# fundwotsai2001/AP-adapter

Hardware: AMD Instinct MI355X
Metric: 10s-clips/sec @200 DDIM steps, AudioLDM2-large+AP (higher is better)
Workload: dtype bf16; 1 GPU; AudioLDM2-large geometry + 32 AP processors, style_transfer preset (ap_scale 0.55, La=32, CFG 9.5), batch 32/GPU, 10 s clips (latents 8x250x16), 200-step DDIM, hipGraph-captured step; one bench step = one DDIM step; global_batch=32, parallelism=dp1 (independent clips, no collective in the loop), weights=random-init N(0,0.02^2), real shapes (no checkpoint offline)

## Files before the change

ap-adapter_amd/_lib.py:

```python
import ctypes as C
import os
import subprocess
import threading

import torch

_HERE = os.path.dirname(os.path.abspath(__file__))
LIB_PATH = os.environ.get("APAD_LIB_PATH") or os.path.join(_HERE, "libapadapter_hip.so")
CSRC = os.path.join(_HERE, "csrc")

BF16, F16, F32, F32_BF16X3 = 0, 1, 2, 3
A_PLAIN, A_CONV3X3, A_PATCH16, A_CONV1D = 0, 1, 2, 4
EPI_NONE, EPI_SILU, EPI_GELU, EPI_GEGLU, EPI_TANH, EPI_RELU, EPI_GELU_TANH, EPI_GEGLU_TANH = 0, 1, 2, 3, 4, 5, 6, 7
OUT_ROWMAJOR, OUT_VT, OUT_QKV = 0, 1, 2

_vp, _i64, _i32, _f32 = C.c_void_p, C.c_int64, C.c_int32, C.c_float


class GemmDesc(C.Structure):
    _fields_ = [(n, _vp) for n in ("a", "w", "out", "bias", "residual", "rowgroup_bias", "step_ptr")] + \
               [(n, _i64) for n in ("M", "N", "K", "lda", "ldw", "ldo", "ldr", "ld_rg", "rows_per_group")] + \
               [(n, _i32) for n in ("a_mode", "epilogue", "out_mode", "dtype", "Hin", "Win", "Cin", "Hout", "Wout",
                                    "stride", "Hup", "Wup", "src_batch_mod", "residual_row_mod", "heads", "head_dim", "L", "Lpad")] + \
               [("out2", _vp), ("out3", _vp)] + \
               [(n, _i32) for n in ("taps", "dilation", "pad", "transposed", "a_pre_act")] + [("a_pre_slope", _f32)] + \
               [("conv_asym_pad", _i32), ("reserved_conv", _i32)] + \
               [(n, _vp) for n in ("rowstat_out", "rowstat_in", "ln_colsum", "ln_bias")] + [("rowstat_in_tiles", _i32), ("ln_eps", _f32)] + \
               [("a2", _vp), ("lda2", _i64), ("k_split", _i32), ("a_row_mod", _i32), ("a2_row_mod", _i32), ("reserved_a2", _i32), ("out4", _vp),
                ("w_halo", _vp), ("workspace", _vp), ("workspace_bytes", _i64)]


class AttnDesc(C.Structure):
    _fields_ = [(n, _vp) for n in ("q", "k", "vt", "k2", "vt2", "out", "key_bias", "lse")] + \
               [(n, _i64) for n in ("q_stride_b", "q_stride_n", "k_stride_b", "k_stride_l", "vt_stride_b",
                                    "k2_stride_b", "k2_stride_l", "vt2_stride_b", "o_stride_b", "o_stride_n")] + \
               [(n, _i32) for n in ("B", "N", "H", "D", "L", "Lpad", "L2", "Lpad2", "kv_batch_div", "kv2_batch_div",
                                    "dtype")] + \
               [("softmax_scale", _f32), ("scale2", _f32), ("q_prescaled", _i32)]


class RpSegment(C.Structure):
    _fields_ = [("out", _vp), ("bias", _vp), ("ldo", _i64), ("n_cols", _i32), ("mode", _i32)]


class RpDesc(C.Structure):
    _fields_ = [(n, _vp) for n in ("x", "w", "ln_gamma", "ln_beta", "residual")] + \
               [(n, _i64) for n in ("M", "lda", "ldw", "ldr")] + \
               [(n, _i32) for n in ("K", "epilogue", "dtype", "n_segments")] + [("ln_eps", _f32)] + \
               [(n, _i32) for n in ("heads", "head_dim", "L", "Lpad")] + [("seg", RpSegment * 3)]


class MlpDesc(C.Structure):
    _fields_ = [(n, _vp) for n in ("x", "ln_gamma", "ln_beta", "w1", "b1", "w2", "b2", "out")] + \
               [("M", _i64), ("C", _i32), ("dtype", _i32), ("ln_eps", _f32), ("reserved", _i32)]


class XattnDesc(C.Structure):
    _fields_ = [(n, _vp) for n in ("x", "ln_gamma", "ln_beta", "wq_packed", "wo_packed", "bo", "kv1_packed", "key_bias", "kv2_packed", "out", "q_fold")] + \
               [(n, _i32) for n in ("B", "N", "C", "heads", "L1", "L2", "dtype", "reserved")] + \
               [(n, _f32) for n in ("ln_eps", "softmax_scale", "scale2", "reserved_f")]


class XrowsDesc(C.Structure):
    _fields_ = [(n, _vp) for n in ("x", "ln_gamma", "ln_beta", "wq_packed", "wo_packed", "bo", "k1", "vt1", "key_bias", "k2", "vt2", "out")] + \
               [(n, _i32) for n in ("B", "N", "C", "heads", "L1", "Lpad1", "L2", "Lpad2", "dtype", "reserved")] + \
               [(n, _f32) for n in ("ln_eps", "softmax_scale", "scale2", "reserved_f")]


class HsAttnDesc(C.Structure):
    _fields_ = [(n, _vp) for n in ("x", "w_packed", "w_bias", "k1", "vt1", "key_bias", "k2", "vt2", "out")] + \
               [(n, _i32) for n in ("B", "N", "C", "heads", "L1", "Lpad1", "L2", "Lpad2", "self_attention", "q_prescaled", "dtype", "normalize")] + \
               [(n, _f32) for n in ("ln_eps", "softmax_scale", "scale2", "reserved_f")]


class HsOutDesc(C.Structure):
    _fields_ = [(n, _vp) for n in ("o", "w_packed", "bias", "residual", "out", "rowstat_out")] + [(n, _i32) for n in ("B", "N", "C", "dtype")]


class AttnBwdDesc(C.Structure):
    _fields_ = [(n, _vp) for n in ("q", "k", "v", "qt", "kt", "out", "dout", "doutt", "lse", "key_bias", "delta", "dq", "dk", "dv")] + \
               [(n, _i32) for n in ("B", "N", "H", "D", "L", "Npad", "Lpad", "dtype")] + \
               [("softmax_scale", _f32), ("dout_scale", _f32), ("accumulate_dq", _i32), ("ld_grad", _i32)]


SYMBOLS = {
    "apad_last_error": (C.c_char_p, []),
    "apad_abi_version": (C.c_int, []),
    "apad_set_gemm_ring": (C.c_int, [_i32]),
    "apad_sizeof_gemm_desc": (C.c_int, []),
    "apad_sizeof_attn_desc": (C.c_int, []),
    "apad_echo_gemm_desc": (C.c_int, [C.POINTER(GemmDesc), C.POINTER(C.c_double), C.c_int]),
    "apad_echo_attn_desc": (C.c_int, [C.POINTER(AttnDesc), C.POINTER(C.c_double), C.c_int]),
    "apad_sizeof_rp_desc": (C.c_int, []),
    "apad_echo_rp_desc": (C.c_int, [C.POINTER(RpDesc), C.POINTER(C.c_double), C.c_int]),
    "apad_rowpanel_gemm": (C.c_int, [C.POINTER(RpDesc), _vp]),
    "apad_sizeof_mlp_desc": (C.c_int, []),
    "apad_echo_mlp_desc": (C.c_int, [C.POINTER(MlpDesc), C.POINTER(C.c_double), C.c_int]),
    "apad_geglu_mlp": (C.c_int, [C.POINTER(MlpDesc), _vp]),
    "apad_mlp_packed_bytes": (_i64, [_i32]),
    "apad_mlp_packed_bias_floats": (_i64, [_i32]),
    "apad_mlp_pack": (C.c_int, [_vp, _vp, _vp, _vp, _vp, _i32, _i32, _vp]),
    "apad_geglu_mlp_packed": (C.c_int, [C.POINTER(MlpDesc), _vp, _vp, _vp]),
    "apad_geglu_packed_bytes": (_i64, [_i32]),
    "apad_geglu_packed_bias_floats": (_i64, [_i32]),
    "apad_geglu_pack": (C.c_int, [_vp, _vp, _vp, _vp, _i32, _i32, _vp]),
    "apad_layernorm_geglu_packed": (C.c_int, [_vp, _vp, _vp, _vp, _vp, _vp, _i64, _i32, _f32, _i32, _vp]),
    "apad_sizeof_xattn_desc": (C.c_int, []),
    "apad_echo_xattn_desc": (C.c_int, [C.POINTER(XattnDesc), C.POINTER(C.c_double), C.c_int]),
    "apad_fused_cross_attention": (C.c_int, [C.POINTER(XattnDesc), _vp]),
    "apad_sizeof_xrows_desc": (C.c_int, []),
    "apad_cross_attention_rows": (C.c_int, [C.POINTER(XrowsDesc), _vp]),
    "apad_sizeof_hs_attn_desc": (C.c_int, []),
    "apad_hs_attention": (C.c_int, [C.POINTER(HsAttnDesc), _vp]),
    "apad_self_attention_fused": (C.c_int, [_vp, _vp, _vp, _vp, _i32, _i32, _i32, _i32, _f32, _i32, _vp]),
    "apad_hs_geglu": (C.c_int, [_vp, _vp, _vp, _vp, _i32, _i32, _i32, _i32, _f32, _i32, _vp]),
    "apad_sizeof_hs_out_desc": (C.c_int, []),
    "apad_hs_out": (C.c_int, [C.POINTER(HsOutDesc), _vp]),
    "apad_hs_ff2": (C.c_int, [C.POINTER(HsOutDesc), _vp]),
    "apad_xattn_pack_weight": (C.c_int, [_vp, _vp, _i64, _i32, _vp]),
    "apad_xattn_packed_kv_bytes": (_i64, [_i32, _i32]),
    "apad_xattn_pack_kv": (C.c_int, [_vp, _vp, _vp, _i32, _i32, _i32, _i64, _i64, _i64, _i32, _vp]),
    "apad_rows_packed_kv_bytes": (_i64, [_i32, _i32, _i32, _i32]),
    "apad_rows_pack_kv": (C.c_int, [_vp, _vp, _vp, _i32, _i32, _i32, _i32, _i32, _i32, _vp]),
    "apad_gemm": (C.c_int, [C.POINTER(GemmDesc), _vp]),
    "apad_conv_halo_pack": (C.c_int, [_vp, _vp, _i64, _i64, _i32, _vp]),
    "apad_hconv_launch_count": (_i64, []),
    "apad_f32_split_weight": (C.c_int, [_vp, _vp, _i64, _i64, _i64, _vp]),
    "apad_f32x3_launch_count": (_i64, []),
    "apad_probe_mfma": (C.c_int, [_vp, _i32, _i32, C.POINTER(C.c_double), _vp]),
    "apad_conv_halo_packed_bytes": (_i64, [_i64, _i64]),
    "apad_conv_halo_workspace_bytes": (_i64, [_i64, _i64, _i64, _i32]),
    "apad_attention": (C.c_int, [C.POINTER(AttnDesc), _vp]),
    "apad_layernorm": (C.c_int, [_vp, _vp, _vp, _vp, _i64, _i32, _i64, _i64, _f32, _i32, _vp]),
    "apad_groupnorm_workspace_bytes": (_i64, [_i32, _i32, _i32]),
    "apad_groupnorm": (C.c_int, [_vp, _vp, _vp, _vp, _vp, _i32, _i32, _i32, _i32, _f32, _i32, _i32, _vp]),
    "apad_groupnorm2": (C.c_int, [_vp, _vp, _vp, _vp, _vp, _vp, _i32, _i32, _i32, _i32, _i32, _i32, _i32, _f32, _i32, _i32, _vp]),
    "apad_audiomae_pool": (C.c_int, [_vp, _vp, _i32, _i32, _i32, _i32, _i32, _vp]),
    "apad_timestep_embedding": (C.c_int, [_vp, _vp, _i32, _i32, _i32, _f32, _i32, _vp]),
    "apad_cfg_ddim_step": (C.c_int, [_vp, _vp, _vp, _vp, _vp, _vp, _f32, _i32, _i64, _i32, _vp]),
    "apad_step_advance": (C.c_int, [_vp, _vp]),
    "apad_cfg_sampler_step": (C.c_int, [_vp, _vp, _vp, _vp, _vp, _vp, _vp, _vp, _i32, _f32, _i32, _i64, _i32, _vp]),
    "apad_cfg_edit_step": (C.c_int, [_vp, _vp, _vp, _vp, _vp, _vp, _vp, _vp, _vp, _vp, _vp, _i32, _i32, _vp, _i32, _f32, _i32, _i64, _i32, _vp]),
    "apad_cfg_dual_step": (C.c_int, [_vp, _vp, _vp, _vp, _vp, _vp, _vp, _vp, _vp, _vp, _vp, _vp, _i32, _i32, _vp, _i32, _i32, _i64, _i32, _vp]),
    "apad_cfg_shaped_step": (C.c_int, [_vp] * 15 + [_i32, _i32, _vp, _i32, _f32, _i32, _i32, _i64, _i32, _vp]),
    "apad_cfg_invert_step": (C.c_int, [_vp, _vp, _vp, _vp, _vp, _vp, _vp, _vp, _vp, _vp, _i32, _f32, _i32, _i32, _i64, _i32, _vp]),
    "apad_edit_start": (C.c_int, [_vp, _vp, _vp, _vp, _vp, _vp, _f32, _f32, _f32, _i64, _i32, _i32, _vp]),
    "apad_mix3": (C.c_int, [_vp, _vp, _vp, _vp, _i64, _f32, _i32, _vp]),
    "apad_softmax_rows": (C.c_int, [_vp, _vp, _vp, _i64, _i32, _i64, _i64, _i64, _f32, _i32, _vp]),
    "apad_rmsnorm": (C.c_int, [_vp, _vp, _vp, _i64, _i32, _i64, _i64, _f32, _i32, _i32, _vp]),
    "apad_gather_rows": (C.c_int, [_vp, _vp, _vp, _i64, _i64, _i32, _i32, _vp]),
    "apad_gaussian_sample": (C.c_int, [_vp, _vp, _vp, _i64, _i32, _f32, _i32, _vp]),
    "apad_sizeof_attn_bwd_desc": (C.c_int, []),
    "apad_echo_attn_bwd_desc": (C.c_int, [C.POINTER(AttnBwdDesc), C.POINTER(C.c_double), C.c_int]),
    "apad_attention_bwd": (C.c_int, [C.POINTER(AttnBwdDesc), _vp]),
    "apad_head_transpose": (C.c_int, [_vp, _vp, _i32, _i32, _i32, _i32, _i32, _i32, _vp]),
    "apad_head_transpose3": (C.c_int, [_vp, _vp, _vp, _vp, _vp, _vp, _i32, _i32, _i32, _i32, _i32, _i32, _vp]),
    "apad_layernorm_bwd": (C.c_int, [_vp, _vp, _vp, _vp, _i64, _i32, _f32, _i32, _vp]),
    "apad_layernorm_bwd_add": (C.c_int, [_vp, _vp, _vp, _vp, _vp, _i64, _i32, _f32, _i32, _vp]),
    "apad_groupnorm_bwd": (C.c_int, [_vp, _vp, _vp, _vp, _vp, _i32, _i32, _i32, _i32, _f32, _i32, _i32, _vp]),
    "apad_geglu": (C.c_int, [_vp, _vp, _i64, _i32, _i32, _vp]),
    "apad_geglu_bwd": (C.c_int, [_vp, _vp, _vp, _i64, _i32, _i32, _vp]),
    "apad_upsample_nearest_bwd": (C.c_int, [_vp, _vp, _i32, _i32, _i32, _i32, _i32, _i32, _i32, _vp]),
    "apad_zero_stuff2": (C.c_int, [_vp, _vp, _i32, _i32, _i32, _i32, _i32, _i32, _i32, _vp]),
    "apad_transpose_pad": (C.c_int, [_vp, _vp, _i32, _i32, _i32, _i32, _vp]),
    "apad_transpose_pad2": (C.c_int, [_vp, _vp, _i32, _vp, _vp, _i32, _i32, _i32, _i32, _i32, _vp]),
    "apad_reduce_workspace_bytes": (_i64, []),
    "apad_mse_loss_grad": (C.c_int, [_vp, _vp, _vp, _vp, _vp, _i64, _f32, _i32, _vp]),
    "apad_step_advance_if_finite": (C.c_int, [_vp, _vp, _vp]),
    "apad_grad_norm": (C.c_int, [_vp, _vp, _vp, _i64, _vp]),
    "apad_resample_fir": (C.c_int, [_vp, _vp, _vp, _i64, _i64, _i32, _i32, _i32, _vp]),
    "apad_kaldi_fbank": (C.c_int, [_vp, _i64, _f32, _vp, _vp, _vp, _vp, _i32, _i32, _f32, _f32, _f32, _vp]),
    "apad_wav_stats": (C.c_int, [_vp, _vp, _vp, _vp, _i32, _vp]),
    "apad_stft_logmel": (C.c_int, [_vp, _vp, _vp, _vp, _vp, _vp, _vp, _vp, _vp, _i32, _i64, _i32, _vp]),
    "apad_adamw_step": (C.c_int, [_vp, _vp, _vp, _vp, _vp, _vp, _vp, _i64, _f32, _f32, _f32, _f32, _f32, _f32, _i32, _vp]),
    "apad_window_attention": (C.c_int, [_vp, _vp, _vp, _i32, _i32, _i32, _i32, _i32, _i32, _i32, _i32, _vp]),
    "apad_clap_mel2img": (C.c_int, [_vp, _vp, _vp, _vp, _vp, _f32, _vp, _i32, _i32, _i32, _i32, _vp]),
    "apad_clap_logmel": (C.c_int, [_vp, _vp, _vp, _vp, _vp, _vp, _i32, _i32, _i32, _vp, _vp, _vp, _vp, _vp, _i32, _i64, _i32, _i32, _i32, _vp]),
    "apad_chroma": (C.c_int, [_vp, _vp, _vp, _vp, _vp, _vp, _vp, _i32, _i32, _vp]),
    "apad_chroma_similarity": (C.c_int, [_vp, _vp, _vp, _vp, _vp, _vp, _vp, _vp, _i32, _i32, _i32, _vp]),
    "apad_loudness": (C.c_int, [_vp, _vp, _vp, _vp, _vp, _vp, _vp, _i32, _i32, _i32, _vp]),
    "apad_loudness_gain": (C.c_int, [_vp, _vp, _vp, _vp, _vp, _vp, _vp, _vp, _vp, _vp, _i32, _i32, _f32, _vp]),
}

_lock = threading.Lock()
_lib = None


def build(verbose=False):
    r = subprocess.run(["make", "-C", CSRC, "-j4"], capture_output=True, text=True)
    if verbose or r.returncode != 0:
        print(r.stdout[-4000:])
        print(r.stderr[-4000:])
    if r.returncode != 0:
        raise RuntimeError("building libapadapter_hip.so failed:\n" + r.stderr[-2000:])
    return LIB_PATH


def lib():
    global _lib
    if _lib is not None:
        return _lib
    with _lock:
        if _lib is None:
            if not os.path.exists(LIB_PATH):
                raise RuntimeError(
                    f"{LIB_PATH} is missing: the HIP extension is the product path and has no fallback; "
                    "run `python -c 'import __graft_entry__ as g; g.build()'` (or `make -C ap-adapter_amd/csrc`).")
            h = C.CDLL(LIB_PATH)
            for name, (res, args) in SYMBOLS.items():
                fn = getattr(h, name)
                fn.restype = res
                fn.argtypes = args
            if h.apad_abi_version() != 12:
                raise RuntimeError("libapadapter_hip.so ABI version mismatch")
            if h.apad_sizeof_gemm_desc() != C.sizeof(GemmDesc) or h.apad_sizeof_attn_desc() != C.sizeof(AttnDesc) \
                    or h.apad_sizeof_rp_desc() != C.sizeof(RpDesc) \
                    or h.apad_sizeof_mlp_desc() != C.sizeof(MlpDesc) \
                    or h.apad_sizeof_attn_bwd_desc() != C.sizeof(AttnBwdDesc) \
                    or h.apad_sizeof_xattn_desc() != C.sizeof(XattnDesc) or h.apad_sizeof_xrows_desc() != C.sizeof(XrowsDesc) \
                    or h.apad_sizeof_hs_attn_desc() != C.sizeof(HsAttnDesc) or h.apad_sizeof_hs_out_desc() != C.sizeof(HsOutDesc):
                raise RuntimeError("descriptor layout mismatch between include/apadapter_hip.h and _lib.py")
            _lib = h
    return _lib


def check(rc, what):
    if rc != 0:
        raise RuntimeError(f"{what} failed (rc={rc}): {lib().apad_last_error().decode()}")
```

ap-adapter_amd/autograd.py:

```python
import os as _os

import torch

from . import ops
from .derived import derived


def on(*tensors):
    return torch.is_grad_enabled() and any(t is not None and t.requires_grad for t in tensors)


def _derived(w, tag, make, deps=()):
    return make() if w.requires_grad else derived(w, tag, make, deps)


def _wt(w):
    return _derived(w, "T", lambda: w.detach().reshape(w.shape[0], -1).t().contiguous())


def _conv_dgrad_w(w):
    return _derived(w, "dgrad", lambda: w.detach().flip(2, 3).permute(1, 2, 3, 0).reshape(w.shape[1], -1).contiguous())


def _conv_fwd_w(w):
    return ops.conv3x3_pack(w) if w.requires_grad else ops.conv3x3_weight(w)


def _c(t):
    return t if t.is_contiguous() else t.contiguous()


def _exact(backward):
    def run(ctx, *grads):
        with ops.exact_f32():
            return backward(ctx, *grads)
    return run


class _Linear(torch.autograd.Function):

    @staticmethod
    def forward(ctx, x, w, b, residual):
        ctx.save_for_backward(x if w.requires_grad else None, w)
        ctx.has_res = residual is not None
        ctx.sink = getattr(w, "_apad_grad_sink", None)
        w2 = w.reshape(w.shape[0], -1)
        with ops.recorded_forward():
            return ops.linear(_c(x), w2, b, residual=None if residual is None else _c(residual))

    @staticmethod
    @_exact
    def backward(ctx, dy):
        x, w = ctx.saved_tensors
        dy = _c(dy)
        dx = dw = None
        if ctx.needs_input_grad[0]:
            dx = ops.linear(dy, _wt(w))
        if ctx.needs_input_grad[1]:
            if ctx.sink is not None:
                acc, inv_scale = ctx.sink
                if inv_scale == 1.0 and acc.is_contiguous() and acc.dim() == 2:
                    ops.weight_grad(dy.reshape(-1, dy.shape[-1]), x.reshape(-1, x.shape[-1]), fp32=True, acc=acc)
                else:
                    acc.add_(ops.weight_grad(dy.reshape(-1, dy.shape[-1]), x.reshape(-1, x.shape[-1]), fp32=True).reshape(acc.shape),
                             alpha=inv_scale)
            else:
                dw = ops.weight_grad(dy.reshape(-1, dy.shape[-1]), x.reshape(-1, x.shape[-1])).reshape(w.shape)
        return dx, dw, None, (dy if ctx.has_res and ctx.needs_input_grad[3] else None)


def linear(x, w, b=None, residual=None):
    return _Linear.apply(x, w, b, residual)


_BWD_PACKED = True


def _packed_grads(dq, dk, dv):
    base = dq._base
    C_ = dq.shape[-1]
    if (base is not None and dk._base is base and dv._base is base and base.is_contiguous() and base.shape[-1] == 3 * C_
            and base.shape[:-1] == dq.shape[:-1] and dq.stride() == dk.stride() == dv.stride() == base.stride()
            and dq.storage_offset() == base.storage_offset() and dk.storage_offset() == base.storage_offset() + C_
            and dv.storage_offset() == base.storage_offset() + 2 * C_):
        return base
    return torch.cat([_c(dq), _c(dk), _c(dv)], dim=-1)


class _QKV(torch.autograd.Function):

    @staticmethod
    def forward(ctx, x, wq, wk, wv):
        x = _c(x)
        ctx.save_for_backward(wq, wk, wv)
        with ops.recorded_forward():
            return ops.linear(x, wq), ops.linear(x, wk), ops.linear(x, wv)

    @staticmethod
    @_exact
    def backward(ctx, dq, dk, dv):
        wq, wk, wv = ctx.saved_tensors
        wst = _derived(wq, "qkvT", lambda: torch.cat([wq.detach(), wk.detach(), wv.detach()], 0).t().contiguous(), (wk, wv))
        return ops.linear(_packed_grads(dq, dk, dv), wst), None, None, None


class _QKVT(_QKV):

    @staticmethod
    def forward(ctx, x, wq, wk, wv, heads):
        from .processors import vt_buffer
        x = _c(x)
        B, N, Cc = x.shape
        ctx.save_for_backward(wq, wk, wv)
        w = _derived(wq, "qkv_train", lambda: torch.cat([wq.detach(), wk.detach(), wv.detach()], 0).contiguous(), (wk, wv))
        q, k, v = torch.empty_like(x), torch.empty_like(x), torch.empty_like(x)
        vt = vt_buffer("train_self", B, heads, Cc // heads, N, x.dtype, x.device)
        ops.linear_qkv(x, w, B, N, heads, q, k, vt, v=v)
        ctx.mark_non_differentiable(vt)
        return q, k, v, vt

    @staticmethod
    @_exact
    def backward(ctx, dq, dk, dv, _dvt):
        return _QKV.backward(ctx, dq, dk, dv) + (None,)


_QKV_FUSED = True


def qkv(x, wq, wk, wv, heads=None):
    if wq.requires_grad or wk.requires_grad or wv.requires_grad:
        return linear(x, wq), linear(x, wk), linear(x, wv), None
    C_ = x.shape[-1]
    if (_QKV_FUSED and heads is not None and x.dtype in ops.FUSED_DTYPES and x.dim() == 3 and C_ % 128 == 0
            and tuple(wq.shape) == tuple(wk.shape) == tuple(wv.shape) == (C_, C_)):
        return _QKVT.apply(x, wq, wk, wv, heads)
    return _QKV.apply(x, wq, wk, wv) + (None,)


class _LayerNorm(torch.autograd.Function):
    @staticmethod
    def forward(ctx, x, g, b, eps):
        x = _c(x)
        ctx.save_for_backward(x, g)
        ctx.eps = eps
        return ops.layer_norm(x, g, b, eps)

    @staticmethod
    @_exact
    def backward(ctx, dy):
        x, g = ctx.saved_tensors
        return ops.layer_norm_bwd(x, g, _c(dy), ctx.eps), None, None, None


def layer_norm(x, g, b, eps):
    return _LayerNorm.apply(x, g, b, eps)


class _LayerNormRes(torch.autograd.Function):

    @staticmethod
    def forward(ctx, x, g, b, eps):
        x = _c(x)
        ctx.save_for_backward(x, g)
        ctx.eps = eps
        return ops.layer_norm(x, g, b, eps), x.view_as(x)

    @staticmethod
    @_exact
    def backward(ctx, dy, dres):
        x, g = ctx.saved_tensors
        if dy is None:
            return dres, None, None, None
        return ops.layer_norm_bwd(x, g, _c(dy), ctx.eps, dres=None if dres is None else _c(dres)), None, None, None


_LN_RES = True


def layer_norm_res(x, g, b, eps):
    if not _LN_RES:
        return _LayerNorm.apply(x, g, b, eps), x
    return _LayerNormRes.apply(x, g, b, eps)


class _GroupNorm(torch.autograd.Function):
    @staticmethod
    def forward(ctx, x, g, b, groups, eps, silu):
        x = _c(x)
        ctx.save_for_backward(x, g, b)
        ctx.cfg = (groups, eps, silu)
        return ops.group_norm(x, g, b, groups, eps, silu=silu)

    @staticmethod
    @_exact
    def backward(ctx, dy):
        x, g, b = ctx.saved_tensors
        groups, eps, silu = ctx.cfg
        return ops.group_norm_bwd(x, g, b, _c(dy), groups, eps, silu), None, None, None, None, None


def group_norm(x, g, b, groups, eps, silu):
    return _GroupNorm.apply(x, g, b, groups, eps, silu)


class _Conv3x3(torch.autograd.Function):

    @staticmethod
    def forward(ctx, x, w, b, residual, rowgroup_bias, geom):
        B, H, W, stride, up, rows_per_group = geom
        ctx.save_for_backward(w)
        ctx.geom = geom
        ctx.has_res = residual is not None
        out, Ho, Wo = ops.conv3x3(_c(x), _conv_fwd_w(w), b, B, H, W, stride=stride, up=up,
                                  residual=None if residual is None else _c(residual), rowgroup_bias=rowgroup_bias,
                                  rows_per_group=rows_per_group)
        ctx.out_hw = (Ho, Wo)
        return out

    @staticmethod
    @_exact
    def backward(ctx, dy):
        (w,) = ctx.saved_tensors
        B, H, W, stride, up, _ = ctx.geom
        Ho, Wo = ctx.out_hw
        dy = _c(dy)
        dx = None
        if ctx.needs_input_grad[0]:
            wd = _conv_dgrad_w(w)
            if stride == 2:
                z = ops.zero_stuff2(dy, B, H, W, Ho, Wo)
                dx, _, _ = ops.conv3x3(z, wd, None, B, H, W)
            elif up is not None:
                dup, _, _ = ops.conv3x3(dy, wd, None, B, up[0], up[1])
                dx = ops.upsample_nearest_bwd(dup, B, H, W, up[0], up[1])
            else:
                dx, _, _ = ops.conv3x3(dy, wd, None, B, H, W)
        return dx, None, None, (dy if ctx.has_res and ctx.needs_input_grad[3] else None), None, None


def conv3x3(x, w, b, B, H, W, stride=1, up=None, residual=None, rowgroup_bias=None, rows_per_group=0):
    Hs, Ws = up if up is not None else (H, W)
    Ho, Wo = (Hs + 2 - 3) // stride + 1, (Ws + 2 - 3) // stride + 1
    out = _Conv3x3.apply(x, w, b, residual, rowgroup_bias, (B, H, W, stride, up, rows_per_group))
    return out, Ho, Wo


class _Geglu(torch.autograd.Function):
    @staticmethod
    def forward(ctx, proj):
        proj = _c(proj)
        ctx.save_for_backward(proj)
        return ops.geglu(proj)

    @staticmethod
    @_exact
    def backward(ctx, dh):
        (proj,) = ctx.saved_tensors
        return ops.geglu_bwd(proj, _c(dh))


def geglu(proj):
    return _Geglu.apply(proj)


class _Attention(torch.autograd.Function):

    @staticmethod
    def forward(ctx, q, k, v, heads, key_bias, vt=None):
        q, k, v = _c(q), _c(k), _c(v)
        if vt is None:
            vt = ops.head_transpose(v, heads)
        o, lse = ops.attention_lse(q, k, vt, k.shape[1], heads, key_bias=key_bias)
        ctx.save_for_backward(q, k, v, o, lse, key_bias)
        ctx.heads = heads
        return o

    @staticmethod
    @_exact
    def backward(ctx, do):
        q, k, v, o, lse, key_bias = ctx.saved_tensors
        need_kv = ctx.needs_input_grad[1] or ctx.needs_input_grad[2]
        packed = _BWD_PACKED and all(ctx.needs_input_grad[:3]) and q.shape == k.shape
        dq, dk, dv = ops.attention_bwd(q, k, v, o, _c(do), lse, ctx.heads, key_bias=key_bias, need_dkv=need_kv, packed=packed)
        return dq, dk, dv, None, None, None


def attention(q, k, v, heads, key_bias=None, vt=None):
    return _Attention.apply(q, k, v, heads, key_bias, vt)


class _IPAttention(torch.autograd.Function):

    @staticmethod
    def forward(ctx, q, k_t, v_t, k_a, v_a, heads, key_bias, scale):
        q, k_t, v_t, k_a, v_a = _c(q), _c(k_t), _c(v_t), _c(k_a), _c(v_a)
        vt_t, vt_a = ops.head_transpose(v_t, heads), ops.head_transpose(v_a, heads)
        o_t, lse_t = ops.attention_lse(q, k_t, vt_t, k_t.shape[1], heads, key_bias=key_bias)
        o_a, lse_a = ops.attention_lse(q, k_a, vt_a, k_a.shape[1], heads)
        o = ops.attention(q, k_t, vt_t, k_t.shape[1], heads, key_bias=key_bias, k2=k_a, vt2=vt_a, L2=k_a.shape[1], scale2=scale)
        ctx.save_for_backward(q, k_t, v_t, k_a, v_a, o_t, o_a, lse_t, lse_a, key_bias)
        ctx.heads, ctx.scale = heads, scale
        return o

    @staticmethod
    @_exact
    def backward(ctx, do):
        q, k_t, v_t, k_a, v_a, o_t, o_a, lse_t, lse_a, key_bias = ctx.saved_tensors
        do = _c(do)
        need_t = ctx.needs_input_grad[1] or ctx.needs_input_grad[2]
        need_a = ctx.needs_input_grad[3] or ctx.needs_input_grad[4]
        dq, dk_t, dv_t = ops.attention_bwd(q, k_t, v_t, o_t, do, lse_t, ctx.heads, key_bias=key_bias, need_dkv=need_t)
        _, dk_a, dv_a = ops.attention_bwd(q, k_a, v_a, o_a, do, lse_a, ctx.heads, dout_scale=ctx.scale, need_dkv=need_a, dq=dq)
        return dq, dk_t, dv_t, dk_a, dv_a, None, None, None


def ip_attention(q, k_t, v_t, k_a, v_a, heads, key_bias, scale):
    return _IPAttention.apply(q, k_t, v_t, k_a, v_a, heads, key_bias, scale)


class _MSE(torch.autograd.Function):

    @staticmethod
    def forward(ctx, pred, target, grad_scale):
        loss, dpred = ops.mse_loss_grad(_c(pred), _c(target.float()), grad_scale)
        ctx.save_for_backward(dpred)
        return loss.reshape(())

    @staticmethod
    @_exact
    def backward(ctx, g):
        (dpred,) = ctx.saved_tensors
        return dpred * g.to(dpred.dtype), None, None


def mse_loss(pred, target, grad_scale=1.0):
    return _MSE.apply(pred, target, float(grad_scale))
```

ap-adapter_amd/csrc/capi.cpp:

```cpp
#include <hip/hip_runtime.h>
#include <stdarg.h>
#include <stdio.h>
#include <mutex>
#include "common.h"

static thread_local char g_err[512] = "";

void apad_set_error(const char* fmt, ...) {
    va_list ap;
    va_start(ap, fmt);
    vsnprintf(g_err, sizeof(g_err), fmt, ap);
    va_end(ap);
}

int apad_check_launch(const char* what) {
    hipError_t e = hipGetLastError();
    if (e != hipSuccess) {
        apad_set_error("%s: launch failed: %s", what, hipGetErrorString(e));
        return -2;
    }
    return 0;
}

extern "C" const char* apad_last_error(void) { return g_err; }
int apad_ensure_dyn_lds(const void* kern, int bytes, unsigned* devmask) {
    static std::mutex mu;
    int dev = 0;
    if (hipGetDevice(&dev) != hipSuccess || dev < 0 || dev > 31) dev = 0;
    std::lock_guard<std::mutex> g(mu);
    if (!((*devmask >> dev) & 1u)) {
        const hipError_t e = hipFuncSetAttribute(kern, hipFuncAttributeMaxDynamicSharedMemorySize, bytes);
        if (e != hipSuccess) {
            apad_set_error("hipFuncSetAttribute(MaxDynamicSharedMemorySize = %d) failed on device %d: %s", bytes, dev, hipGetErrorString(e));
            return -1;
        }
        *devmask |= 1u << dev;
    }
    return 0;
}

extern "C" int apad_abi_version(void) { return APAD_ABI_VERSION; }
extern "C" int apad_sizeof_gemm_desc(void) { return (int)sizeof(apad_gemm_desc); }
extern "C" int apad_sizeof_attn_desc(void) { return (int)sizeof(apad_attn_desc); }

#define PUT(x)                          \
    do {                                \
        if (n < cap) out[n] = (double)(x); \
        ++n;                            \
    } while (0)
#define PUTP(x) PUT((uintptr_t)(x))

extern "C" int apad_echo_gemm_desc(const apad_gemm_desc* d, double* out, int cap) {
    int n = 0;
    PUTP(d->a); PUTP(d->w); PUTP(d->out); PUTP(d->bias); PUTP(d->residual); PUTP(d->rowgroup_bias); PUTP(d->step_ptr);
    PUT(d->M); PUT(d->N); PUT(d->K); PUT(d->lda); PUT(d->ldw); PUT(d->ldo); PUT(d->ldr); PUT(d->ld_rg);
    PUT(d->rows_per_group);
    PUT(d->a_mode); PUT(d->epilogue); PUT(d->out_mode); PUT(d->dtype);
    PUT(d->Hin); PUT(d->Win); PUT(d->Cin); PUT(d->Hout); PUT(d->Wout); PUT(d->stride); PUT(d->Hup); PUT(d->Wup);
    PUT(d->src_batch_mod); PUT(d->residual_row_mod); PUT(d->heads); PUT(d->head_dim); PUT(d->L); PUT(d->Lpad);
    PUTP(d->out2); PUTP(d->out3);
    PUT(d->taps); PUT(d->dilation); PUT(d->pad); PUT(d->transposed); PUT(d->a_pre_act); PUT(d->a_pre_slope);
    PUT(d->conv_asym_pad); PUT(d->reserved_conv);
    PUTP(d->rowstat_out); PUTP(d->rowstat_in); PUTP(d->ln_colsum); PUTP(d->ln_bias); PUT(d->rowstat_in_tiles); PUT(d->ln_eps);
    PUTP(d->a2); PUT(d->lda2); PUT(d->k_split); PUT(d->a_row_mod); PUT(d->a2_row_mod); PUT(d->reserved_a2);
    PUTP(d->out4); PUTP(d->w_halo); PUTP(d->workspace); PUT(d->workspace_bytes);
    return n;
}

extern "C" int apad_echo_attn_desc(const apad_attn_desc* d, double* out, int cap) {
    int n = 0;
    PUTP(d->q); PUTP(d->k); PUTP(d->vt); PUTP(d->k2); PUTP(d->vt2); PUTP(d->out); PUTP(d->key_bias); PUTP(d->lse);
    PUT(d->q_stride_b); PUT(d->q_stride_n); PUT(d->k_stride_b); PUT(d->k_stride_l); PUT(d->vt_stride_b);
    PUT(d->k2_stride_b); PUT(d->k2_stride_l); PUT(d->vt2_stride_b); PUT(d->o_stride_b); PUT(d->o_stride_n);
    PUT(d->B); PUT(d->N); PUT(d->H); PUT(d->D); PUT(d->L); PUT(d->Lpad); PUT(d->L2); PUT(d->Lpad2);
    PUT(d->kv_batch_div); PUT(d->kv2_batch_div); PUT(d->dtype); PUT(d->softmax_scale); PUT(d->scale2); PUT(d->q_prescaled);
    return n;
}

extern "C" int apad_sizeof_rp_desc(void) { return (int)sizeof(apad_rp_desc); }
extern "C" int apad_echo_rp_desc(const apad_rp_desc* d, double* out, int cap) {
    int n = 0;
    PUTP(d->x); PUTP(d->w); PUTP(d->ln_gamma); PUTP(d->ln_beta); PUTP(d->residual);
    PUT(d->M); PUT(d->lda); PUT(d->ldw); PUT(d->ldr);
    PUT(d->K); PUT(d->epilogue); PUT(d->dtype); PUT(d->n_segments); PUT(d->ln_eps);
    PUT(d->heads); PUT(d->head_dim); PUT(d->L); PUT(d->Lpad);
    for (int i = 0; i < 3; ++i) {
        PUTP(d->seg[i].out); PUTP(d->seg[i].bias); PUT(d->seg[i].ldo); PUT(d->seg[i].n_cols); PUT(d->seg[i].mode);
    }
    return n;
}

extern "C" int apad_sizeof_mlp_desc(void) { return (int)sizeof(apad_mlp_desc); }
extern "C" int apad_echo_mlp_desc(const apad_mlp_desc* d, double* out, int cap) {
    int n = 0;
    PUTP(d->x); PUTP(d->ln_gamma); PUTP(d->ln_beta); PUTP(d->w1); PUTP(d->b1); PUTP(d->w2); PUTP(d->b2); PUTP(d->out);
    PUT(d->M); PUT(d->C); PUT(d->dtype); PUT(d->ln_eps); PUT(d->reserved);
    return n;
}

extern "C" int apad_sizeof_attn_bwd_desc(void) { return (int)sizeof(apad_attn_bwd_desc); }
extern "C" int apad_echo_attn_bwd_desc(const apad_attn_bwd_desc* d, double* out, int cap) {
    int n = 0;
    PUTP(d->q); PUTP(d->k); PUTP(d->v); PUTP(d->qt); PUTP(d->kt); PUTP(d->out); PUTP(d->dout); PUTP(d->doutt); PUTP(d->lse);
    PUTP(d->key_bias); PUTP(d->delta); PUTP(d->dq); PUTP(d->dk); PUTP(d->dv);
    PUT(d->B); PUT(d->N); PUT(d->H); PUT(d->D); PUT(d->L); PUT(d->Npad); PUT(d->Lpad); PUT(d->dtype);
    PUT(d->softmax_scale); PUT(d->dout_scale); PUT(d->accumulate_dq); PUT(d->ld_grad);
    return n;
}

extern "C" int apad_sizeof_xattn_desc(void) { return (int)sizeof(apad_xattn_desc); }
extern "C" int apad_sizeof_xrows_desc(void) { return (int)sizeof(apad_xrows_desc); }
extern "C" int apad_echo_xattn_desc(const apad_xattn_desc* d, double* out, int cap) {
    int n = 0;
    PUTP(d->x); PUTP(d->ln_gamma); PUTP(d->ln_beta); PUTP(d->wq_packed); PUTP(d->wo_packed); PUTP(d->bo); PUTP(d->kv1_packed);
    PUTP(d->key_bias); PUTP(d->kv2_packed); PUTP(d->out); PUTP(d->q_fold);
    PUT(d->B); PUT(d->N); PUT(d->C); PUT(d->heads); PUT(d->L1); PUT(d->L2);
    PUT(d->dtype); PUT(d->reserved); PUT(d->ln_eps); PUT(d->softmax_scale); PUT(d->scale2); PUT(d->reserved_f);
    return n;
}
```

ap-adapter_amd/csrc/hconv.hip:

```cpp
#include <type_traits>
#include <utility>
#include "gfx950_prims.h"
#include "gemm_shared.h"

namespace {

constexpr uint32_t H_OOB = 0x80000000u;

struct HcP {
    const uint8_t* a;
    const uint8_t* wp;
    uint8_t* out;
    const uint8_t* bias;
    const uint8_t* residual;
    const uint8_t* rg;
    const int32_t* step_ptr;
    int64_t ldo, ldr, ld_rg, rows_per_group;
    int32_t M, N, Cin;
    int32_t H, W, Wlog;
    int32_t Hs, Ws;
    int32_t Btot;
    int32_t m_tiles, n_tiles, nchunks;
    int32_t ksplit;
    float* partial;
    uint32_t a_bytes, w_bytes;
};

template <int... S, class F> __device__ __forceinline__ void h_for_each(std::integer_sequence<int, S...>, F&& f) {
    (f(std::integral_constant<int, S>{}), ...);
}

template <int WAVES_M_, int WAVES_N_, int MI_, int NJ_, int KS_> struct HcT {
    static constexpr int WAVES_M = WAVES_M_, WAVES_N = WAVES_N_, MI = MI_, NJ = NJ_, KS = KS_;
    static constexpr int NW = WAVES_M * WAVES_N, NT = NW * 64;
    static constexpr int BM = WAVES_M * MI * 32, BN = WAVES_N * NJ * 32;
    static constexpr int NLD = 5;
    static constexpr int NPX = NLD * NW * 8;
    static constexpr int ABUF = NPX * 128;
    static constexpr int SUBB = BN * 64;
    static constexpr int STAGE_B = SUBB * (KS / 2);
    static constexpr int NSTG = 4;
    static constexpr int PBW = STAGE_B / 1024 / NW;
    static constexpr int SPT = 4 / KS;
    static constexpr int SPC = 9 * SPT;
    static constexpr int OFF_B = ABUF, OFF_A1 = OFF_B + NSTG * STAGE_B, OFF_Z = OFF_A1 + ABUF, SMEM = OFF_Z + 256;
    static constexpr int OFF_STG = OFF_B + (NSTG - 1) * STAGE_B, STG_BYTES = STAGE_B + ABUF;
    static_assert(STAGE_B % (1024 * NW) == 0 && (KS == 2 || KS == 4) && SMEM <= 160 * 1024, "tile shape");
    static_assert(NJ * 2048 + SUBB < 65536, "immediate offsets of the weight fragment reads");
};

template <int DT, class T>
__global__ __launch_bounds__(T::NT) void hconv_kernel(HcP p) {
    constexpr int MI = T::MI, NJ = T::NJ, KS = T::KS, NW = T::NW, BM = T::BM, BN = T::BN, NLD = T::NLD, PBW = T::PBW, SPT = T::SPT, SPC = T::SPC;
    extern __shared__ __attribute__((aligned(16))) uint8_t smem[];
    using E = ET<DT>;
    const int tid = threadIdx.x, lane = tid & 63;
    const int wave = __builtin_amdgcn_readfirstlane(tid >> 6);
    const int wm = wave / T::WAVES_N, wn = wave % T::WAVES_N;
    const int half = lane >> 5, l31 = lane & 31;

    const int W = p.W, H = p.H, Wlog = p.Wlog;
    const int R = BM >> Wlog;
    const __amdgpu_buffer_rsrc_t ra = buf_rsrc(p.a, p.a_bytes), rw = buf_rsrc(p.wp, p.w_bytes);
    const uint32_t lds0 = (uint32_t)(size_t)(lds_ptr)smem;

    int m0 = 0, n0 = 0, c_begin = 0, c_end = 0, kslice = 0;
    uint32_t aoff[5];
    uint32_t pbase[4];
    auto setup_tile = [&](int tl_ks) {
        const int tl = tl_ks / p.ksplit;
        kslice = tl_ks - tl * p.ksplit;
        c_begin = kslice * p.nchunks / p.ksplit;
        c_end = (kslice + 1) * p.nchunks / p.ksplit;
        int mt, nt;
        xcd_tile_order(tl, p.m_tiles, p.n_tiles, mt, nt);
        m0 = mt * BM;
        n0 = nt * BN;
        const int g0 = mt * R;
        const int b0 = g0 / H, y0 = g0 - b0 * H;
#pragma unroll
        for (int l = 0; l < NLD; ++l) {
            const int pp = (l * NW + wave) * 8 + (lane >> 3);
            const int slot = lane & 7;
            const int j = pp >> Wlog, x = pp & (W - 1);
            const int v = y0 - 1 + j;
            const int q = v >= 0 ? v / (H + 1) : 0, r = v - q * (H + 1);
            const bool valid = v >= 0 && r != H && b0 + q < p.Btot;
            const int sy = p.Hs == H ? r : (r * p.Hs) / H, sx = p.Ws == W ? x : (x * p.Ws) / W;
            const uint32_t src = (uint32_t)(((b0 + q) * p.Hs + sy) * p.Ws + sx) * (uint32_t)(p.Cin * 2) + (uint32_t)((slot ^ ((pp >> 1) & 7)) << 4);
            aoff[l] = valid ? src : H_OOB;
        }
#pragma unroll
        for (int i = 0; i < MI; ++i) {
            const int ml = (wm * MI + i) * 32 + l31;
            const int ir = ml >> Wlog, x = ml & (W - 1);
            const int nsep = (y0 + ir) / H;
            pbase[i] = (uint32_t)(((1 + ir + nsep) << Wlog) + x);
        }
    };
    auto issue_a = [&](int l, int buf, int chunk) {
        __builtin_amdgcn_raw_ptr_buffer_load_lds(ra, (lds_ptr)(smem + buf * T::OFF_A1 + (l * NW + wave) * 1024), 16, aoff[l], chunk * 128, 0, 0);
    };
    const uint32_t lane16 = (uint32_t)(lane * 16);
    auto issue_b = [&](int c, int s, int slot, int i) {
        const int sub0 = (c * 9 + s / SPT) * 2 + (s % SPT) * (KS / 2);
        const int q = wave * PBW + i;
        const int sb = q / (T::SUBB / 1024), qq = q - sb * (T::SUBB / 1024);
        const int soff = ((sub0 + sb) * p.N + n0) * 64 + qq * 1024;
        __builtin_amdgcn_raw_ptr_buffer_load_lds(rw, (lds_ptr)(smem + T::OFF_B + slot * T::STAGE_B + q * 1024), 16, lane16, soff, 0, 0);
    };

    const bool x_first = (l31 & (W - 1)) == 0, x_last = (l31 & (W - 1)) == W - 1;
    const uint32_t zbase = lds0 + (uint32_t)T::OFF_Z;
    uint32_t bfo[2];
    {
        const int nl = wn * NJ * 32 + l31;
#pragma unroll
        for (int k2 = 0; k2 < 2; ++k2) bfo[k2] = lds0 + (uint32_t)T::OFF_B + (uint32_t)(nl * 64 + (((k2 * 2 + half) ^ ((nl >> 2) & 3)) << 4));
    }

    f32x16 acc[4][4];
    u32x4 fa[2][4] = {}, fb[2][4] = {};
    uint32_t a0[4], a0n[4];
    auto tap_address = [&](int i, int tap, int buf) -> uint32_t {
        const int dy = tap / 3 - 1, dx = tap - (tap / 3) * 3 - 1;
        const uint32_t ps = pbase[i] + (uint32_t)(dy * W + dx);
        uint32_t a = lds0 + (uint32_t)(buf * T::OFF_A1) + (ps << 7) + ((((ps >> 1) & 7) ^ (uint32_t)half) << 4);
        if (dx < 0) a = x_first ? (zbase | (a & 0xF0u)) : a;
        if (dx > 0) a = x_last ? (zbase | (a & 0xF0u)) : a;
        return a;
    };
    auto read_one = [&](auto set_tag, auto ks_tag, auto idx_tag, auto next_tag, uint32_t bb) {
        constexpr int SET = decltype(set_tag)::value, KSI = decltype(ks_tag)::value, IDX = decltype(idx_tag)::value;
        constexpr bool NEXT = decltype(next_tag)::value != 0;
        if constexpr (IDX < MI) {
            lds_read16<0, 'i'>(fa[SET][IDX], (NEXT ? a0n[IDX] : a0[IDX]) ^ (uint32_t)(KSI << 5));
        } else if constexpr (IDX < MI + NJ) {
            constexpr int J = IDX - MI, SB = (KSI % KS) >> 1;
            lds_read16<SB * T::SUBB + J * 2048, 'i'>(fb[SET][J], bb);
        }
    };
    using I0 = std::integral_constant<int, 0>;
    constexpr int NMF = MI * NJ, NRD = MI + NJ;
    constexpr int RSLOTS = (NRD + 1) / 2;
    constexpr int DSLOT0 = RSLOTS < NMF - 1 ? RSLOTS : NMF - 2;
    const int grp = wave >> 2;

    auto issue_prologue = [&]() {
#pragma unroll
        for (int l = 0; l < NLD; ++l) issue_a(l, 0, c_begin);
#pragma unroll
        for (int s = 0; s < 3; ++s)
#pragma unroll
            for (int i = 0; i < PBW; ++i) issue_b(c_begin, s, s, i);
    };
    if (tid < 16) *reinterpret_cast<uint4*>(smem + T::OFF_Z + tid * 16) = make_uint4(0, 0, 0, 0);
    const int ntiles = p.m_tiles * p.n_tiles * p.ksplit;
    setup_tile(blockIdx.x);
    issue_prologue();
#pragma unroll 1
    for (int tl = blockIdx.x; tl < ntiles; tl += gridDim.x) {
    const int cm0 = m0, cn0 = n0, cks = kslice, cb = c_begin, ce = c_end;
#pragma unroll
    for (int j = 0; j < NJ; ++j)
#pragma unroll
        for (int i = 0; i < MI; ++i)
#pragma unroll
            for (int r = 0; r < 16; ++r) acc[j][i][r] = 0.f;
    wait_vm<2 * PBW>();
    wait_lgkm<0>();
    RAW_BARRIER();
#pragma unroll
    for (int i = 0; i < MI; ++i) a0[i] = a0n[i] = tap_address(i, 0, 0);
    h_for_each(std::make_integer_sequence<int, NRD>{}, [&](auto idx_tag) { read_one(I0{}, I0{}, idx_tag, I0{}, bfo[0]); });

    int slot = 0;
#pragma unroll 1
    for (int c = cb; c < ce; ++c) {
        const bool last = c + 1 == ce;
        const int buf = (c - cb) & 1;
        auto stage = [&](auto s_tag) {
            constexpr int S = decltype(s_tag)::value;
            constexpr int TAP = S / SPT, KS0 = (S % SPT) * KS;
            constexpr bool prevA = S >= 1 && S - 1 < NLD;
            if (!last) wait_vm<PBW + (prevA ? 1 : 0)>();
            else if (S == 0 || S - 1 + 3 < SPC) wait_vm<PBW>();
            else wait_vm<0>();
            wait_lgkm<0>();
            RAW_BARRIER();
            const int nslot = (slot + 1) & 3;
            const bool dma_a = S < NLD && !last, dma_b = S + 3 < SPC || !last;
            h_for_each(std::make_integer_sequence<int, KS>{}, [&](auto kk_tag) {
                constexpr int KK = decltype(kk_tag)::value, SET = KK & 1;
                constexpr bool SAME = KK + 1 < KS;
                constexpr int NS = (S + 1) % SPC;
                constexpr bool NEWTAP = !SAME && NS % SPT == 0;
                constexpr int PKSI = SAME ? KS0 + KK + 1 : (NS % SPT) * KS;
                constexpr bool TAPCALC = S % SPT == SPT - 1 && KK == 0;
                constexpr int NTAP = (TAP + 1) % 9;
                const bool pf = SAME || S + 1 < SPC || !last;
                const uint32_t bb = bfo[PKSI & 1] + (uint32_t)((SAME ? slot : nslot) * T::STAGE_B);
                const bool dma_here = grp == (KK == 0 ? 0 : (KK == KS / 2 ? 1 : 2));
                h_for_each(std::make_integer_sequence<int, NMF>{}, [&](auto idx_tag) {
                    constexpr int IDX = decltype(idx_tag)::value;
                    acc[IDX / MI][IDX % MI] = E::mfma32(__builtin_bit_cast(typename E::v8, fb[SET][IDX / MI]),
                                                        __builtin_bit_cast(typename E::v8, fa[SET][IDX % MI]), acc[IDX / MI][IDX % MI]);
                    __builtin_amdgcn_sched_barrier(0);
                    if constexpr (IDX < RSLOTS) if (pf) {
                        read_one(std::integral_constant<int, SET ^ 1>{}, std::integral_constant<int, PKSI>{}, std::integral_constant<int, 2 * IDX>{},
                                 std::integral_constant<int, NEWTAP>{}, bb);
                        read_one(std::integral_constant<int, SET ^ 1>{}, std::integral_constant<int, PKSI>{}, std::integral_constant<int, 2 * IDX + 1>{},
                                 std::integral_constant<int, NEWTAP>{}, bb);
                    }
                    if constexpr (TAPCALC && IDX < MI) a0n[IDX] = tap_address(IDX, NTAP, TAP + 1 < 9 ? buf : buf ^ 1);
                    if (dma_here) {
                        if (IDX == DSLOT0 && dma_a) issue_a(S, buf ^ 1, c + 1);
                        if (IDX >= DSLOT0 && IDX - DSLOT0 < PBW && dma_b) {
                            if (S + 3 < SPC) issue_b(c, S + 3, (slot + 3) & 3, IDX - DSLOT0);
                            else issue_b(c + 1, S + 3 - SPC, (slot + 3) & 3, IDX - DSLOT0);
                        }
                    }
                    __builtin_amdgcn_sched_barrier(0);
                });
                if constexpr (SAME) {
                    wait_lgkm<0>(); SCHED_PIN();
                }
                if constexpr (NEWTAP) {
#pragma unroll
                    for (int i = 0; i < MI; ++i) a0[i] = a0n[i];
                }
            });
            slot = nslot;
        };
        h_for_each(std::make_integer_sequence<int, SPC>{}, stage);
    }

    const int64_t step = p.step_ptr ? (int64_t)*p.step_ptr : 0;
    using elem = typename E::elem;
    const bool rg_table = p.rg && p.rows_per_group >= p.M;
    const bool rg_rows = p.rg && !rg_table;
    constexpr int EROW = NJ * 64 + 16;
    constexpr int LPR = NJ * 4;
    constexpr int RPI = 64 / LPR;
    static_assert(32 * EROW * NW <= T::STG_BYTES, "the epilogue tiles of all waves fit ring slot 3 + halo buffer 1");
    const uint32_t stg = lds0 + (uint32_t)(T::OFF_STG + wave * (32 * EROW));
    const uint32_t stg_w = stg + (uint32_t)(l31 * EROW + 8 * half), stg_r = stg + (uint32_t)((lane / LPR) * EROW + (lane % LPR) * 16);
    const int cn_w = cn0 + wn * NJ * 32;
    uint2 braw[4][4], traw[4][4];
#pragma unroll
    for (int j = 0; j < NJ; ++j)
#pragma unroll
        for (int g = 0; g < 4; ++g) {
            const int n = cn_w + j * 32 + 8 * g + 4 * half;
            braw[j][g] = traw[j][g] = make_uint2(0, 0);
            if (p.bias && p.ksplit == 1) braw[j][g] = *reinterpret_cast<const uint2*>(p.bias + (int64_t)n * 2);
            if (rg_table && p.ksplit == 1) traw[j][g] = *reinterpret_cast<const uint2*>(p.rg + (step * p.ld_rg + n) * 2);
        }
    RAW_BARRIER();
    if (tl + (int)gridDim.x < ntiles) {
        setup_tile(tl + (int)gridDim.x);
        issue_prologue();
    }
    if (p.ksplit > 1) {
        float* slab = p.partial + (int64_t)cks * p.M * p.N;
#pragma unroll
        for (int i = 0; i < MI; ++i) {
            const int m = cm0 + (wm * MI + i) * 32 + l31;
            if (m < p.M) {
#pragma unroll
                for (int j = 0; j < NJ; ++j)
#pragma unroll
                    for (int g = 0; g < 4; ++g) {
                        const f32x4 v = {acc[j][i][4 * g], acc[j][i][4 * g + 1], acc[j][i][4 * g + 2], acc[j][i][4 * g + 3]};
                        *reinterpret_cast<f32x4*>(slab + (int64_t)m * p.N + cn_w + j * 32 + 8 * g + 4 * half) = v;
                    }
            }
        }
    } else {
#pragma unroll
    for (int i = 0; i < MI; ++i) {
        const int mrow0 = cm0 + (wm * MI + i) * 32;
        uint4 rres[32 / RPI] = {};
        if (p.residual) {
#pragma unroll
            for (int k = 0; k < 32 / RPI; ++k) {
                int m = mrow0 + lane / LPR + RPI * k;
                m = m < p.M ? m : p.M - 1;
                rres[k] = *reinterpret_cast<const uint4*>(p.residual + ((int64_t)m * p.ldr + cn_w + (lane % LPR) * 8) * 2);
            }
        }
        const int mp = mrow0 + l31 < p.M ? mrow0 + l31 : p.M - 1;
        const int64_t grp = rg_rows ? mp / p.rows_per_group + step : 0;
#pragma unroll
        for (int j = 0; j < NJ; ++j)
#pragma unroll
            for (int g = 0; g < 4; ++g) {
                uint2 tr = traw[j][g];
                if (rg_rows) tr = *reinterpret_cast<const uint2*>(p.rg + (grp * p.ld_rg + cn_w + j * 32 + 8 * g + 4 * half) * 2);
                const typename E::v4 b4 = __builtin_bit_cast(typename E::v4, braw[j][g]), t4 = __builtin_bit_cast(typename E::v4, tr);
                typename E::v4 h4;
#pragma unroll
                for (int e = 0; e < 4; ++e) h4[e] = (elem)((acc[j][i][4 * g + e] + (float)b4[e]) + (float)t4[e]);
                const uint2 u2 = __builtin_bit_cast(uint2, h4);
                asm volatile("ds_write_b64 %0, %1" ::"v"(stg_w + (uint32_t)((j * 32 + 8 * g) * 2)), "v"(u2) : "memory");
            }
        u32x4 orow[32 / RPI];
#pragma unroll
        for (int k = 0; k < 32 / RPI; ++k) asm volatile("ds_read_b128 %0, %1" : "=v"(orow[k]) : "v"(stg_r + (uint32_t)(RPI * k * EROW)));
        wait_lgkm<0>(); SCHED_PIN();
#pragma unroll
        for (int k = 0; k < 32 / RPI; ++k) {
            const int rl = lane / LPR + RPI * k, m = mrow0 + rl;
            uint4 o = __builtin_bit_cast(uint4, orow[k]);
            if (p.residual) {
                float f[8], rr[8];
                unpack8<DT>(o, f);
                unpack8<DT>(rres[k], rr);
#pragma unroll
                for (int e = 0; e < 8; ++e) f[e] += rr[e];
                o = pack8<DT>(f);
            }
            if (m < p.M)
                *reinterpret_cast<uint4*>(p.out + ((int64_t)m * p.ldo + cn_w + (lane % LPR) * 8) * 2) = o;
        }
    }
    }
    }
}

template <typename TE>
__global__ void hconv_pack_kernel(const TE* __restrict__ w, TE* __restrict__ out, int N, int Cin, int64_t total) {
    const int64_t idx = (int64_t)blockIdx.x * blockDim.x + threadIdx.x;
    if (idx >= total) return;
    const int s = (int)(idx & 3);
    int64_t r = idx >> 2;
    const int n = (int)(r % N);
    r /= N;
    const int h = (int)(r & 1);
    r >>= 1;
    const int tap = (int)(r % 9), c = (int)(r / 9);
    const int ch = c * 64 + h * 32 + ((s ^ ((n >> 2) & 3)) << 3);
    const uint4 v = *reinterpret_cast<const uint4*>(w + ((int64_t)n * 9 + tap) * Cin + ch);
    *reinterpret_cast<uint4*>(out + idx * 8) = v;
}

int64_t g_hconv_launches = 0;

struct HnP {
    const uint8_t* a;
    const uint8_t* wp;
    uint8_t* out;
    const uint8_t* bias;
    int64_t ldo;
    int32_t M, N, Cin, H, W, Wlog, Hs, Ws, Btot, m_tiles, nchunks;
    uint32_t a_bytes;
};

template <int DT> __device__ __forceinline__ f32x4 hn_mfma(u32x4 a, u32x4 b, f32x4 c) {
    if constexpr (DT == APAD_BF16) return __builtin_amdgcn_mfma_f32_16x16x32_bf16(__builtin_bit_cast(bf16x8_t, a), __builtin_bit_cast(bf16x8_t, b), c, 0, 0, 0);
    else return __builtin_amdgcn_mfma_f32_16x16x32_f16(__builtin_bit_cast(f16x8_t, a), __builtin_bit_cast(f16x8_t, b), c, 0, 0, 0);
}

template <int DT, int NCH>
__global__ __launch_bounds__(512) void hnarrow_kernel(HnP p) {
    constexpr int NW = 8, NLD = 5, NPX = NLD * NW * 8, ABUF = NPX * 128, NBUF = 3, OFF_Z = NBUF * ABUF, BM = 256;
    extern __shared__ __attribute__((aligned(16))) uint8_t smem[];
    using E = ET<DT>;
    const int tid = threadIdx.x, lane = tid & 63;
    const int wave = __builtin_amdgcn_readfirstlane(tid >> 6);
    const int l15 = lane & 15, kg = lane >> 4;
    const int W = p.W, H = p.H, Wlog = p.Wlog, R = BM >> Wlog;
    const __amdgpu_buffer_rsrc_t ra = buf_rsrc(p.a, p.a_bytes);
    const uint32_t lds0 = (uint32_t)(size_t)(lds_ptr)smem;

    u32x4 wf[NCH * 18];
#pragma unroll
    for (int i = 0; i < NCH * 18; ++i) wf[i] = *reinterpret_cast<const u32x4*>(p.wp + ((int64_t)i * 64 + lane) * 16);

    auto tile_sources = [&](int mt, uint32_t (&ao)[5]) {
        const int g0 = mt * R, b0 = g0 / H, y0 = g0 - b0 * H;
#pragma unroll
        for (int l = 0; l < NLD; ++l) {
            const int pp = (l * NW + wave) * 8 + (lane >> 3), slot = lane & 7;
            const int j = pp >> Wlog, x = pp & (W - 1), v = y0 - 1 + j;
            const int q = v >= 0 ? v / (H + 1) : 0, r = v - q * (H + 1);
            const bool valid = v >= 0 && r != H && b0 + q < p.Btot;
            const int sy = p.Hs == H ? r : (r * p.Hs) / H, sx = p.Ws == W ? x : (x * p.Ws) / W;
            const uint32_t src = (uint32_t)(((b0 + q) * p.Hs + sy) * p.Ws + sx) * (uint32_t)(p.Cin * 2) + (uint32_t)((slot ^ ((pp >> 1) & 7)) << 4);
            ao[l] = valid ? src : H_OOB;
        }
    };
    auto pixel_records = [&](int mt, uint32_t (&pb)[2]) {
        const int g0 = mt * R, b0 = g0 / H, y0 = g0 - b0 * H;
#pragma unroll
        for (int b = 0; b < 2; ++b) {
            const int ml = wave * 32 + b * 16 + l15, ir = ml >> Wlog, x = ml & (W - 1);
            pb[b] = (uint32_t)(((1 + ir + (y0 + ir) / H) << Wlog) + x);
        }
    };
    const bool x_first = (l15 & (W - 1)) == 0, x_last = (l15 & (W - 1)) == W - 1;
    const uint32_t zbase = lds0 + (uint32_t)OFF_Z;
    if (tid < 16) *reinterpret_cast<uint4*>(smem + OFF_Z + tid * 16) = make_uint4(0, 0, 0, 0);

    const int ntiles = p.m_tiles, tstride = (int)gridDim.x;
    uint32_t ao_cur[5], ao_next[5];
    auto request = [&](const uint32_t (&ao)[5], int chunk, int buf) {
#pragma unroll
        for (int l = 0; l < NLD; ++l)
            __builtin_amdgcn_raw_ptr_buffer_load_lds(ra, (lds_ptr)(smem + buf * ABUF + (l * NW + wave) * 1024), 16, ao[l], chunk * 128, 0, 0);
    };
    int tl = blockIdx.x;
    tile_sources(tl, ao_cur);
    if (tl + tstride < ntiles) tile_sources(tl + tstride, ao_next);
    int gc = 0;
    request(ao_cur, 0, 0);
    if (NCH == 2) request(ao_cur, 1, 1);
    else if (tl + tstride < ntiles) request(ao_next, 0, 1);
#pragma unroll 1
    for (; tl < ntiles; tl += tstride) {
        uint32_t pb[2];
        pixel_records(tl, pb);
        f32x4 acc[2] = {{0.f, 0.f, 0.f, 0.f}, {0.f, 0.f, 0.f, 0.f}};
        const bool more = tl + tstride < ntiles, more2 = tl + 2 * tstride < ntiles;
#pragma unroll
        for (int c = 0; c < NCH; ++c, ++gc) {
            const int buf = gc % NBUF;
            const bool has_next = c + 1 < NCH || more;
            if (has_next) wait_vm<NLD>();
            else wait_vm<0>();
            wait_lgkm<0>();
            RAW_BARRIER();
            {
                const int c2 = c + 2;
                const int nbuf = (gc + 2) % NBUF;
                if (c2 < NCH) request(ao_cur, c2, nbuf);
                else if (c2 - NCH < NCH) { if (more) request(ao_next, c2 - NCH, nbuf); }
                else if (more2) {
                    uint32_t ao2[5];
                    tile_sources(tl + 2 * tstride, ao2);
                    request(ao2, 0, nbuf);
                }
            }
#pragma unroll
            for (int tap = 0; tap < 9; ++tap) {
                const int dy = tap / 3 - 1, dx = tap - (tap / 3) * 3 - 1;
                uint32_t a0[2];
#pragma unroll
                for (int b = 0; b < 2; ++b) {
                    const uint32_t ps = pb[b] + (uint32_t)(dy * W + dx);
                    uint32_t a = lds0 + (uint32_t)(buf * ABUF) + (ps << 7) + ((((ps >> 1) & 7) ^ (uint32_t)kg) << 4);
                    if (dx < 0) a = x_first ? (zbase | (a & 0xF0u)) : a;
                    if (dx > 0) a = x_last ? (zbase | (a & 0xF0u)) : a;
                    a0[b] = a;
                }
                u32x4 fb[2][2];
#pragma unroll
                for (int kk = 0; kk < 2; ++kk)
#pragma unroll
                    for (int b = 0; b < 2; ++b) asm volatile("ds_read_b128 %0, %1" : "=v"(fb[kk][b]) : "v"(a0[b] ^ (uint32_t)(kk << 6)));
                wait_lgkm<0>(); SCHED_PIN();
#pragma unroll
                for (int kk = 0; kk < 2; ++kk)
#pragma unroll
                    for (int b = 0; b < 2; ++b) acc[b] = hn_mfma<DT>(wf[(c * 9 + tap) * 2 + kk], fb[kk][b], acc[b]);
            }
        }
        if (4 * kg < p.N) {
            float bv[4] = {0.f, 0.f, 0.f, 0.f};
            if (p.bias) {
#pragma unroll
                for (int e = 0; e < 4; ++e) bv[e] = ld_elem<DT>(p.bias, 4 * kg + e);
            }
#pragma unroll
            for (int b = 0; b < 2; ++b) {
                const int m = tl * BM + wave * 32 + b * 16 + l15;
                typename E::v4 h4;
#pragma unroll
                for (int e = 0; e < 4; ++e) h4[e] = (typename E::elem)(acc[b][e] + bv[e]);
                if (m < p.M) *reinterpret_cast<uint2*>(p.out + ((int64_t)m * p.ldo + 4 * kg) * 2) = __builtin_bit_cast(uint2, h4);
            }
        }
        if (more) {
#pragma unroll
            for (int l = 0; l < NLD; ++l) ao_cur[l] = ao_next[l];
            if (more2) tile_sources(tl + 2 * tstride, ao_next);
        }
    }
}

template <typename TE>
__global__ void hnarrow_pack_kernel(const TE* __restrict__ w, TE* __restrict__ out, int N, int Cin, int64_t total) {
    const int64_t idx = (int64_t)blockIdx.x * blockDim.x + threadIdx.x;
    if (idx >= total) return;
    const int lane = (int)(idx & 63);
    const int f = (int)(idx >> 6), kk = f & 1, tap = (f >> 1) % 9, c = (f >> 1) / 9;
    const int n = lane & 15, ch = c * 64 + kk * 32 + 8 * (lane >> 4);
    uint4 v = make_uint4(0, 0, 0, 0);
    if (n < N) v = *reinterpret_cast<const uint4*>(w + ((int64_t)n * 9 + tap) * Cin + ch);
    *reinterpret_cast<uint4*>(out + idx * 8) = v;
}

template <int DT, int NCH> int hn_launch(const HnP& p, hipStream_t s) {
    auto kern = hnarrow_kernel<DT, NCH>;
    constexpr int SMEM = 3 * 5 * 8 * 8 * 128 + 256;
    static unsigned devs = 0;
    if (apad_ensure_dyn_lds(reinterpret_cast<const void*>(kern), SMEM, &devs) != 0) return -1;
    ++g_hconv_launches;
    int dev = 0, cus = 256;
    if (hipGetDevice(&dev) == hipSuccess) (void)hipDeviceGetAttribute(&cus, hipDeviceAttributeMultiprocessorCount, dev);
    if (cus <= 0) cus = 256;
    hipLaunchKernelGGL(kern, dim3((unsigned)(p.m_tiles < cus ? p.m_tiles : cus)), dim3(512), SMEM, s, p);
    return apad_check_launch("apad_gemm(halo convolution, narrow form)");
}

template <int DT>
__global__ __launch_bounds__(256) void hconv_reduce_kernel(HcP p) {
    const int vpr = p.N >> 3;
    const int64_t idx = (int64_t)blockIdx.x * 256 + threadIdx.x;
    if (idx >= (int64_t)p.M * vpr) return;
    const int m = (int)(idx / vpr), n = (int)(idx - (int64_t)m * vpr) * 8;
    float a[8];
#pragma unroll
    for (int e = 0; e < 8; ++e) a[e] = 0.f;
    for (int ks = 0; ks < p.ksplit; ++ks) {
        const float* src = p.partial + ((int64_t)ks * p.M + m) * p.N + n;
        const f32x4 v0 = *reinterpret_cast<const f32x4*>(src), v1 = *reinterpret_cast<const f32x4*>(src + 4);
#pragma unroll
        for (int e = 0; e < 4; ++e) {
            a[e] += v0[e];
            a[e + 4] += v1[e];
        }
    }
    if (p.bias) {
        float b[8];
        unpack8<DT>(*reinterpret_cast<const uint4*>(p.bias + n * 2), b);
#pragma unroll
        for (int e = 0; e < 8; ++e) a[e] += b[e];
    }
    if (p.rg) {
        const int64_t step = p.step_ptr ? (int64_t)*p.step_ptr : 0;
        const int64_t grp = (p.rows_per_group >= p.M ? 0 : m / p.rows_per_group) + step;
        float t[8];
        unpack8<DT>(*reinterpret_cast<const uint4*>(p.rg + (grp * p.ld_rg + n) * 2), t);
#pragma unroll
        for (int e = 0; e < 8; ++e) a[e] += t[e];
    }
    uint4 o = pack8<DT>(a);
    if (p.residual) {
        float f[8], rr[8];
        unpack8<DT>(o, f);
        unpack8<DT>(*reinterpret_cast<const uint4*>(p.residual + ((int64_t)m * p.ldr + n) * 2), rr);
#pragma unroll
        for (int e = 0; e < 8; ++e) f[e] += rr[e];
        o = pack8<DT>(f);
    }
    *reinterpret_cast<uint4*>(p.out + ((int64_t)m * p.ldo + n) * 2) = o;
}

template <int DT, class T> int hc_launch(const HcP& p, hipStream_t s) {
    auto kern = hconv_kernel<DT, T>;
    ++g_hconv_launches;
    static unsigned devs = 0;
    if (apad_ensure_dyn_lds(reinterpret_cast<const void*>(kern), T::SMEM, &devs) != 0) return -1;
    static int cus[32] = {};
    int dev = 0;
    if (hipGetDevice(&dev) != hipSuccess || dev < 0 || dev > 31) dev = 0;
    if (cus[dev] == 0) {
        int n = 0;
        if (hipDeviceGetAttribute(&n, hipDeviceAttributeMultiprocessorCount, dev) != hipSuccess || n <= 0) n = 256;
        cus[dev] = n;
    }
    const int tiles = p.m_tiles * p.n_tiles * p.ksplit, cap = cus[dev];
    hipLaunchKernelGGL(kern, dim3((unsigned)(tiles < cap ? tiles : cap)), dim3(T::NT), T::SMEM, s, p);
    int rc = apad_check_launch("apad_gemm(halo convolution)");
    if (rc || p.ksplit == 1) return rc;
    const int64_t vecs = (int64_t)p.M * (p.N / 8);
    hipLaunchKernelGGL(hconv_reduce_kernel<DT>, dim3((unsigned)((vecs + 255) / 256)), dim3(256), 0, s, p);
    return apad_check_launch("apad_gemm(halo convolution, slice sum)");
}

using HcA = HcT<2, 4, 4, 2, 2>;
using HcB = HcT<4, 2, 2, 2, 4>;

}

static int hconv_ksplit(int W, int Cin) { return W == 2 && Cin / 64 >= 3 ? 3 : 1; }

extern "C" int64_t apad_conv_halo_workspace_bytes(int64_t M, int64_t N, int64_t Cin, int32_t Wout) {
    const int ks = hconv_ksplit(Wout, (int)Cin);
    return ks > 1 ? ks * M * N * (int64_t)sizeof(float) : 0;
}

extern "C" int64_t apad_hconv_launch_count(void) { return g_hconv_launches; }

extern "C" int64_t apad_conv_halo_packed_bytes(int64_t N, int64_t Cin) { return N <= 16 ? (Cin / 64) * 18 * 1024 : N * 9 * Cin * 2; }

extern "C" int apad_conv_halo_pack(const void* w, void* out, int64_t N, int64_t Cin, int32_t dtype, void* stream) {
    APAD_CHECK(w && out && N > 0 && Cin > 0 && Cin % 64 == 0, "apad_conv_halo_pack: needs Cin %% 64 == 0");
    APAD_CHECK(dtype == APAD_BF16 || dtype == APAD_F16, "apad_conv_halo_pack: 16-bit weights only");
    if (N <= 16) {
        const int64_t total = (Cin / 64) * 18 * 64;
        hipLaunchKernelGGL(hnarrow_pack_kernel<uint16_t>, dim3((unsigned)((total + 255) / 256)), dim3(256), 0, (hipStream_t)stream,
                           (const uint16_t*)w, (uint16_t*)out, (int)N, (int)Cin, total);
        return apad_check_launch("apad_conv_halo_pack(narrow)");
    }
    const int64_t total = N * 9 * Cin / 8;
    hipLaunchKernelGGL(hconv_pack_kernel<uint16_t>, dim3((unsigned)((total + 255) / 256)), dim3(256), 0, (hipStream_t)stream,
                       (const uint16_t*)w, (uint16_t*)out, (int)N, (int)Cin, total);
    return apad_check_launch("apad_conv_halo_pack");
}

int apad_hconv_try(const apad_gemm_desc* d, hipStream_t s) {
    if (!d->w_halo || d->a_mode != APAD_A_CONV3X3) return 1;
    if (d->dtype != APAD_BF16 && d->dtype != APAD_F16) return 1;
    if (d->epilogue != APAD_EPI_NONE || d->out_mode != APAD_OUT_ROWMAJOR || d->rowstat_out || d->rowstat_in) return 1;
    if (d->stride != 1 || d->src_batch_mod != 0 || d->conv_asym_pad || d->residual_row_mod != 0 || d->Cin % 64 != 0 || d->K != 9 * (int64_t)d->Cin) return 1;
    const int H = d->Hout, W = d->Wout;
    if (W < 2 || W > 16 || (W & (W - 1)) != 0 || H < 1) return 1;
    const int ksplit = hconv_ksplit(W, d->Cin);
    if (ksplit > 1 && (!d->workspace || d->workspace_bytes < ksplit * d->M * d->N * (int64_t)sizeof(float))) return 1;
    if (d->Hup == 0 && (d->Hin != H || d->Win != W)) return 1;
    if (d->Hup != 0 && (d->Hup != H || d->Wup != W)) return 1;
    if (d->M % ((int64_t)H * W) != 0 || d->M >= (1LL << 30)) return 1;
    if (d->N <= 16) {
        if (d->N % 8 != 0 || (d->Cin != 64 && d->Cin != 128) || W < 4 || d->residual || d->rowgroup_bias || d->ldo % 8 != 0) return 1;
        const int R = 256 / W, S = (R - 1) / H + 1;
        if ((R + 2 + S) * W > 320) return 1;
        const int64_t Btot = d->M / ((int64_t)H * W);
        const int64_t a_bytes = Btot * d->Hin * d->Win * (int64_t)d->Cin * 2;
        if (a_bytes >= (1LL << 31)) return 1;
        HnP q;
        q.a = (const uint8_t*)d->a; q.wp = (const uint8_t*)d->w_halo; q.out = (uint8_t*)d->out; q.bias = (const uint8_t*)d->bias; q.ldo = d->ldo;
        q.M = (int32_t)d->M; q.N = (int32_t)d->N; q.Cin = d->Cin; q.H = H; q.W = W; q.Wlog = __builtin_ctz((unsigned)W); q.Hs = d->Hin; q.Ws = d->Win;
        q.Btot = (int32_t)Btot; q.m_tiles = (int32_t)((d->M + 255) / 256); q.nchunks = d->Cin / 64; q.a_bytes = (uint32_t)a_bytes;
        if (d->dtype == APAD_BF16) return d->Cin == 64 ? hn_launch<APAD_BF16, 1>(q, s) : hn_launch<APAD_BF16, 2>(q, s);
        return d->Cin == 64 ? hn_launch<APAD_F16, 1>(q, s) : hn_launch<APAD_F16, 2>(q, s);
    }
    if (d->N % 128 != 0) return 1;
    if (d->ldo % 8 != 0 || (d->residual && d->ldr % 8 != 0)) return 1;
    const int cfg = d->N % 256 == 0 ? 0 : 1;
    constexpr int BM = 256;
    const int BNc = cfg == 0 ? HcA::BN : HcB::BN;
    const int R = BM / W, S = (R - 1) / H + 1;
    if ((R + 2 + S) * W > HcA::NPX) return 1;
    const int64_t Btot = d->M / ((int64_t)H * W);
    const int64_t a_bytes = Btot * d->Hin * d->Win * (int64_t)d->Cin * 2, w_bytes = d->N * 9 * (int64_t)d->Cin * 2;
    if (a_bytes >= (1LL << 31) || w_bytes >= (1LL << 31)) return 1;
    if (d->rowgroup_bias && d->rows_per_group <= 0) return 1;
    HcP p;
    p.a = (const uint8_t*)d->a; p.wp = (const uint8_t*)d->w_halo; p.out = (uint8_t*)d->out; p.bias = (const uint8_t*)d->bias;
    p.residual = (const uint8_t*)d->residual; p.rg = (const uint8_t*)d->rowgroup_bias; p.step_ptr = d->step_ptr;
    p.ldo = d->ldo; p.ldr = d->ldr; p.ld_rg = d->ld_rg; p.rows_per_group = d->rows_per_group;
    p.M = (int32_t)d->M; p.N = (int32_t)d->N; p.Cin = d->Cin;
    p.H = H; p.W = W; p.Wlog = __builtin_ctz((unsigned)W); p.Hs = d->Hin; p.Ws = d->Win; p.Btot = (int32_t)Btot;
    p.m_tiles = (int32_t)((d->M + BM - 1) / BM); p.n_tiles = (int32_t)(d->N / BNc); p.nchunks = d->Cin / 64;
    p.ksplit = ksplit; p.partial = (float*)d->workspace;
    p.a_bytes = (uint32_t)a_bytes; p.w_bytes = (uint32_t)w_bytes;
    if (d->dtype == APAD_BF16) return cfg == 0 ? hc_launch<APAD_BF16, HcA>(p, s) : hc_launch<APAD_BF16, HcB>(p, s);
    return cfg == 0 ? hc_launch<APAD_F16, HcA>(p, s) : hc_launch<APAD_F16, HcB>(p, s);
}
```

ap-adapter_amd/ops.py:

```python
import ctypes as C
import math

import torch

from . import _lib as L
from .derived import derived, is_derived

_DT = {torch.bfloat16: L.BF16, torch.float16: L.F16, torch.float32: L.F32}
_EPI = {None: L.EPI_NONE, "none": L.EPI_NONE, "silu": L.EPI_SILU, "gelu": L.EPI_GELU, "geglu": L.EPI_GEGLU, "tanh": L.EPI_TANH,
        "relu": L.EPI_RELU, "gelu_tanh": L.EPI_GELU_TANH, "geglu_tanh": L.EPI_GEGLU_TANH}


def _stream():
    return torch.cuda.current_stream().cuda_stream


def _ptr(t):
    return None if t is None else t.data_ptr()


def _req(t, name, dtype=None):
    if not t.is_cuda:
        raise RuntimeError(f"{name}: expected a GPU tensor; the HIP path has no CPU fallback")
    if dtype is not None and t.dtype != dtype:
        raise RuntimeError(f"{name}: dtype {t.dtype} != {dtype}")
    if t.stride(-1) != 1:
        raise RuntimeError(f"{name}: last dim must be contiguous")
    return t


def round_up(x, m):
    return (x + m - 1) // m * m


def set_gemm_ring(mode):
    return int(L.lib().apad_set_gemm_ring(int(mode)))


_F32_PRECISIONS = ("highest", "high")
_f32_precision = ["highest"]
_exact_depth = [0]


def set_float32_matmul_precision(precision):
    if precision not in _F32_PRECISIONS:
        raise ValueError(f"set_float32_matmul_precision: {precision!r} is not one of {_F32_PRECISIONS}")
    _f32_precision[0] = precision


def get_float32_matmul_precision():
    return _f32_precision[0]


class exact_f32:
    def __enter__(self):
        _exact_depth[0] += 1

    def __exit__(self, *exc):
        _exact_depth[0] -= 1


def _f32_dtype(dtype, exact=False):
    if dtype == torch.float32 and not exact and _exact_depth[0] == 0 and _f32_precision[0] == "high":
        return L.F32_BF16X3
    return _DT[dtype]


def f32_split_weight(w, rows, K, ldw):
    def make():
        wv = w.detach()
        out = torch.empty(2, rows, K, dtype=torch.bfloat16, device=w.device)
        L.check(L.lib().apad_f32_split_weight(wv.data_ptr(), out.data_ptr(), rows, K, ldw, _stream()), "apad_f32_split_weight")
        return out
    if not split_cacheable(w):
        return make()
    base = w if w._base is None else w._base
    off = w.storage_offset() - base.storage_offset()
    return derived(base, ("bf16x3", off, rows, K, ldw), make)


_in_recorded_forward = [0]


class recorded_forward:
    def __enter__(self):
        _in_recorded_forward[0] += 1

    def __exit__(self, *exc):
        _in_recorded_forward[0] -= 1


def split_cacheable(w):
    base = w if w._base is None else w._base
    recording = torch.is_grad_enabled() or _in_recorded_forward[0] > 0
    if recording and (w.requires_grad or base.requires_grad):
        return False
    return isinstance(base, torch.nn.Parameter) or is_derived(base)


def _set_w(d, w, rows, K, ldw, exact=False):
    d.dtype = _f32_dtype(w.dtype, exact)
    if d.dtype == L.F32_BF16X3:
        d.w, d.ldw = f32_split_weight(w, rows, K, ldw).data_ptr(), K
    else:
        d.w, d.ldw = w.data_ptr(), ldw


def gemm(a, w, *, M, N, K, lda, out, ldo, bias=None, residual=None, ldr=0, act=None, rowgroup_bias=None, ld_rg=0,
         rows_per_group=0, step_ptr=None, a_mode=L.A_PLAIN, out_mode=L.OUT_ROWMAJOR, conv=None, vt=None, ldw=None,
         residual_row_mod=0, asym_pad=False, rowstat_out=None, ln_fold=None, a2=None, lda2=0, k_split=0, a_row_mod=0, a2_row_mod=0,
         w_halo=None, workspace=None, exact=False):
    d = L.GemmDesc()
    if rowstat_out is not None:
        d.rowstat_out = rowstat_out.data_ptr()
    if ln_fold is not None:
        rs, cs, bb, eps = ln_fold
        d.rowstat_in, d.ln_colsum, d.ln_bias, d.rowstat_in_tiles, d.ln_eps = rs.data_ptr(), cs.data_ptr(), bb.data_ptr(), rs.shape[-2], float(eps)
    d.a, d.out = a.data_ptr(), out.data_ptr()
    d.bias, d.residual, d.rowgroup_bias, d.step_ptr = _ptr(bias), _ptr(residual), _ptr(rowgroup_bias), _ptr(step_ptr)
    d.M, d.N, d.K, d.lda, d.ldo, d.ldr, d.ld_rg = M, N, K, lda, ldo, ldr, ld_rg
    _set_w(d, w, 2 * N if act in ("geglu", "geglu_tanh") else N, K, K if ldw is None else ldw, exact)
    d.rows_per_group = rows_per_group
    d.residual_row_mod = residual_row_mod
    d.a_mode, d.epilogue, d.out_mode = a_mode, _EPI[act], out_mode
    if conv is not None:
        (d.Hin, d.Win, d.Cin, d.Hout, d.Wout, d.stride, d.Hup, d.Wup, d.src_batch_mod) = conv
    if vt is not None:
        d.heads, d.head_dim, d.L, d.Lpad = vt
    d.conv_asym_pad = 1 if asym_pad else 0
    if a2 is not None:
        d.a2, d.lda2, d.k_split = a2.data_ptr(), lda2, k_split
    d.a_row_mod, d.a2_row_mod = a_row_mod, a2_row_mod
    d.w_halo = _ptr(w_halo)
    if workspace is not None:
        d.workspace, d.workspace_bytes = workspace.data_ptr(), workspace.numel() * workspace.element_size()
    L.check(L.lib().apad_gemm(C.byref(d), _stream()), "apad_gemm")
    return out




def rowstat_of(x):
    return getattr(x, "_apad_rowstat", None)


def _ln_folded(w, bias, gamma, beta):
    def make():
        wf = w.detach().float()
        wg = (wf * gamma.detach().float()).to(w.dtype).contiguous()
        cs = wg.float().sum(1).contiguous()
        bb = wf @ beta.detach().float()
        if bias is not None:
            bb = bb + bias.detach().float()
        return wg, cs, bb.contiguous()
    return derived(w, "ln_fold", make, (bias, gamma, beta))


def linear(x, w, bias=None, residual=None, act=None, out=None, rowgroup_bias=None, rows_per_group=0, step_ptr=None,
           residual_row_mod=0, rowstat=False, ln=None):
    _req(x, "linear.x", w.dtype)
    _req(w, "linear.w")
    K = x.shape[-1]
    M = x.numel() // K
    N = w.shape[0] // 2 if act in ("geglu", "geglu_tanh") else w.shape[0]
    x2 = x.reshape(M, K)
    if out is None:
        out = torch.empty(*x.shape[:-1], N, dtype=w.dtype, device=x.device)
    r2 = None if residual is None else _req(residual, "linear.residual", w.dtype).reshape(-1, N)
    fold = rs_out = None
    if ln is not None:
        rs = rowstat_of(x)
        if rs is None:
            raise RuntimeError("linear(ln=...): no row statistics for x (use fused_linear, which falls back to apad_layernorm)")
        w, cs, bb = _ln_folded(w, bias, ln[0], ln[1])
        bias, fold = None, (rs, cs, bb, ln[2])
    if rowstat and N % 64 == 0 and N not in RP_K and act in (None, "none") and w.dtype in FUSED_DTYPES:
        rs_out = torch.empty(M, N // 64, 2, dtype=torch.float32, device=x.device)
    gemm(x2, w, M=M, N=N, K=K, lda=x2.stride(0), out=out, ldo=N, bias=bias, residual=r2, ldr=N, act=act,
         rowgroup_bias=rowgroup_bias, ld_rg=(rowgroup_bias.stride(0) if rowgroup_bias is not None else 0),
         rows_per_group=rows_per_group, step_ptr=step_ptr, ldw=w.stride(0), residual_row_mod=residual_row_mod,
         rowstat_out=rs_out, ln_fold=fold)
    if rs_out is not None:
        out._apad_rowstat = rs_out
    elif hasattr(out, "_apad_rowstat"):
        del out._apad_rowstat
    return out


def linear2(xa, xb, w, bias=None, out=None):
    _req(xa, "linear2.xa", w.dtype)
    _req(xb, "linear2.xb", w.dtype)
    Ba, T, Ca = xa.shape
    Bb, Tb, Cb = xb.shape
    B = max(Ba, Bb)
    if Tb != T or B % Ba or B % Bb or Ca % 64 or w.shape[1] != Ca + Cb or not (xa.is_contiguous() and xb.is_contiguous()):
        raise ValueError(f"linear2: xa {tuple(xa.shape)}, xb {tuple(xb.shape)}, w {tuple(w.shape)}")
    N = w.shape[0]
    if out is None:
        out = torch.empty(B, T, N, dtype=w.dtype, device=xa.device)
    gemm(xa, w, M=B * T, N=N, K=Ca + Cb, lda=Ca, out=out, ldo=N, bias=bias, ldw=w.stride(0), a2=xb, lda2=Cb, k_split=Ca,
         a_row_mod=(Ba * T if Ba != B else 0), a2_row_mod=(Bb * T if Bb != B else 0))
    return out


def ln_foldable(x, w):
    return x.dtype in FUSED_DTYPES and not rp_ok(x) and rowstat_of(x) is not None and w.shape[1] == x.shape[-1]


RP_K = (256, 384)
FUSED_DTYPES = (torch.bfloat16, torch.float16)


def rp_ok(x, K=None):
    return (x.shape[-1] if K is None else K) in RP_K and x.dtype in FUSED_DTYPES


def rowpanel(x, w, segs, ln=None, residual=None, act=None, vt_geom=None):
    _req(x, "rowpanel.x", w.dtype)
    K = x.shape[-1]
    M = x.numel() // K
    d = L.RpDesc()
    d.x, d.w = x.data_ptr(), w.data_ptr()
    if ln is not None:
        d.ln_gamma, d.ln_beta, d.ln_eps = ln[0].data_ptr(), ln[1].data_ptr(), float(ln[2])
    d.residual = _ptr(residual)
    d.M, d.lda, d.ldw, d.ldr = M, x.reshape(M, K).stride(0), w.stride(0), (residual.shape[-1] if residual is not None else 0)
    d.K, d.epilogue, d.dtype, d.n_segments = K, _EPI[act], _DT[w.dtype], len(segs)
    if vt_geom is not None:
        d.heads, d.head_dim, d.L, d.Lpad = vt_geom
    for i, (out, bias, n_cols, mode) in enumerate(segs):
        d.seg[i].out, d.seg[i].bias = out.data_ptr(), _ptr(bias)
        d.seg[i].ldo = out.shape[-1] if mode == "row" else 0
        d.seg[i].n_cols, d.seg[i].mode = n_cols, (L.OUT_ROWMAJOR if mode == "row" else L.OUT_VT)
    L.check(L.lib().apad_rowpanel_gemm(C.byref(d), _stream()), "apad_rowpanel_gemm")
    return [s[0] for s in segs]


def fused_linear(x, w, bias=None, ln=None, residual=None, act=None, out=None, rowstat=False):
    K = x.shape[-1]
    N = w.shape[0] // 2 if act == "geglu" else w.shape[0]
    if rp_ok(x, K) and N % 64 == 0:
        if out is None:
            out = torch.empty(*x.shape[:-1], N, dtype=w.dtype, device=x.device)
        rowpanel(x, w, [(out, bias, N, "row")], ln=ln, residual=residual, act=act)
        return out
    if ln is not None and ln_foldable(x, w):
        return linear(x, w, bias, residual=residual, act=act, out=out, rowstat=rowstat, ln=ln)
    if ln is not None:
        x = layer_norm(x, ln[0], ln[1], ln[2])
    return linear(x, w, bias, residual=residual, act=act, out=out, rowstat=rowstat)


XATTN_C, XATTN_HEADS, XATTN_MAXL = 256, 8, 64
XATTN_MAXL2 = 128
XATTN_LONG2 = 512


def xattn_lengths_ok(L1, L2=0, masked=False):
    return L1 <= XATTN_MAXL and (L2 <= XATTN_MAXL or (L1 == 8 and not masked and (L2 == XATTN_MAXL2 or (XATTN_MAXL2 < L2 <= XATTN_LONG2 and L2 % 64 == 0))))


def xattn_pack_weight(w, ln=None):
    _req(w, "xattn_pack_weight.w")
    if ln is not None:
        wf = w.detach().float()
        wg = (wf * ln[0].detach().float()).to(w.dtype).contiguous()
        q_fold = torch.stack([wg.float().sum(1), wf @ ln[1].detach().float()], 0).contiguous()
        return xattn_pack_weight(wg), q_fold
    if tuple(w.shape) != (XATTN_C, XATTN_C) or w.dtype not in FUSED_DTYPES:
        raise ValueError(f"xattn_pack_weight: weight {tuple(w.shape)} {w.dtype} outside the kernel envelope")
    out = torch.empty(XATTN_C * XATTN_C, dtype=w.dtype, device=w.device)
    L.check(L.lib().apad_xattn_pack_weight(w.data_ptr(), out.data_ptr(), w.stride(0), _DT[w.dtype], _stream()), "apad_xattn_pack_weight")
    return out


def xattn_pack_kv(k, vt, Lk):
    _req(k, "xattn_pack_kv.k")
    _req(vt, "xattn_pack_kv.vt", k.dtype)
    B = k.shape[0]
    if k.shape[-1] != XATTN_C or Lk > XATTN_LONG2 or tuple(vt.shape[:3]) != (B, XATTN_HEADS, XATTN_C // XATTN_HEADS) or not vt.is_contiguous():
        raise ValueError(f"xattn_pack_kv: k {tuple(k.shape)}, vt {tuple(vt.shape)}, Lk={Lk} outside the kernel envelope")
    nbytes = L.lib().apad_xattn_packed_kv_bytes(B, Lk)
    out = torch.empty(nbytes // k.element_size(), dtype=k.dtype, device=k.device)
    L.check(L.lib().apad_xattn_pack_kv(k.data_ptr(), vt.data_ptr(), out.data_ptr(), B, Lk, vt.shape[-1], k.stride(0), k.stride(1),
                                       vt.stride(0), _DT[k.dtype], _stream()), "apad_xattn_pack_kv")
    return out


def fused_cross_attention(x, wq_packed, wo_packed, bo, kv1_packed, L1, heads, ln=None, key_bias=None, kv2_packed=None, L2=0,
                          scale2=0.0, out=None, q_fold=None):
    _req(x, "fused_cross_attention.x", wq_packed.dtype)
    B, N, Cc = x.shape
    if Cc != XATTN_C or heads != XATTN_HEADS or not xattn_lengths_ok(L1, L2, key_bias is not None) or x.dtype not in FUSED_DTYPES:
        raise ValueError(f"fused_cross_attention: C={Cc} heads={heads} L1={L1} L2={L2} outside the kernel envelope")
    if not x.is_contiguous():
        raise ValueError("fused_cross_attention.x: must be contiguous")
    if out is None:
        out = torch.empty_like(x)
    d = L.XattnDesc()
    d.x, d.wq_packed, d.wo_packed, d.bo, d.kv1_packed, d.out = (x.data_ptr(), wq_packed.data_ptr(), wo_packed.data_ptr(), _ptr(bo),
                                                                 kv1_packed.data_ptr(), out.data_ptr())
    if ln is not None:
        if q_fold is None or q_fold.dtype != torch.float32 or tuple(q_fold.shape) != (2, Cc) or not q_fold.is_contiguous():
            raise ValueError("fused_cross_attention(ln=...): needs q_fold = the second result of xattn_pack_weight(to_q.weight, ln)")
        d.ln_gamma, d.ln_beta, d.ln_eps, d.q_fold = ln[0].data_ptr(), ln[1].data_ptr(), float(ln[2]), q_fold.data_ptr()
    d.key_bias = _ptr(key_bias)
    d.B, d.N, d.C, d.heads, d.L1 = B, N, Cc, heads, L1
    if L2 > 0:
        d.kv2_packed, d.L2 = kv2_packed.data_ptr(), L2
    d.dtype, d.softmax_scale, d.scale2 = _DT[x.dtype], 1.0 / math.sqrt(Cc // heads), float(scale2)
    L.check(L.lib().apad_fused_cross_attention(C.byref(d), _stream()), "apad_fused_cross_attention")
    return out


XROWS_C, XROWS_MAXL = (384,), 64
XROWS_MAXL2 = 512


def xrows_ok(C_, heads, L1, L2=0):
    return (C_ in XROWS_C and heads == XATTN_HEADS and 1 <= L1 <= XROWS_MAXL
            and (0 <= L2 <= XROWS_MAXL or (L2 <= XROWS_MAXL2 and L1 <= 32)))


def xrows_pack_weight(w):
    N, K = w.shape
    if N % 32 or K % 16:
        raise ValueError(f"xrows_pack_weight: {tuple(w.shape)}")
    return w.detach().reshape(N // 32, 32, K // 16, 2, 8).permute(0, 2, 3, 1, 4).contiguous().reshape(-1)


class RowsKV:
    __slots__ = ("data", "B", "L", "heads", "head_dim")

    def __init__(self, data, B, L, heads, head_dim):
        self.data, self.B, self.L, self.heads, self.head_dim = data, B, L, heads, head_dim

    @property
    def dtype(self):
        return self.data.dtype

    @property
    def shape(self):
        return (self.B, self.L, self.heads * self.head_dim)


def rows_pack_kv(k, vt):
    _req(k, "rows_pack_kv.k")
    _req(vt, "rows_pack_kv.vt", k.dtype)
    B, Lk, Cc = k.shape
    heads, hd = vt.shape[1], vt.shape[2]
    if k.dtype not in FUSED_DTYPES or not k.is_contiguous() or not vt.is_contiguous() or vt.shape[0] != B or heads * hd != Cc or hd % 16 or Lk < 1 \
            or vt.shape[3] < Lk or vt.shape[3] % 32:
        raise ValueError(f"rows_pack_kv: k {tuple(k.shape)} {k.dtype}, vt {tuple(vt.shape)} outside the packing's envelope")
    nbytes = L.lib().apad_rows_packed_kv_bytes(B, heads, hd, Lk)
    out = torch.empty(nbytes // k.element_size(), dtype=k.dtype, device=k.device)
    L.check(L.lib().apad_rows_pack_kv(k.data_ptr(), vt.data_ptr(), out.data_ptr(), B, heads, hd, Lk, vt.shape[3], _DT[k.dtype], _stream()), "apad_rows_pack_kv")
    return RowsKV(out, B, Lk, heads, hd)


def _rows_kv_args(k, vt, B, heads, hd, dtype, what):
    if isinstance(k, RowsKV):
        if vt is not None or (k.B, k.heads, k.head_dim) != (B, heads, hd) or k.dtype != dtype:
            raise ValueError(f"{what}: a RowsKV stands for the (k, vt) pair and must have the batch / heads / type of x")
        return k.data.data_ptr(), 0, k.L, 0
    for t in (k, vt):
        if t is None or not t.is_contiguous() or t.dtype != dtype:
            raise ValueError(f"{what}: must be contiguous {dtype}")
    if k.shape[0] != B or tuple(vt.shape[:3]) != (B, heads, hd):
        raise ValueError(f"{what}: key / value sets must have the batch of x")
    return k.data_ptr(), vt.data_ptr(), k.shape[1], vt.shape[-1]


def cross_attention_rows(x, wq_packed, wo_packed, bo, k1, vt1, heads, ln=None, key_bias=None, k2=None, vt2=None, scale2=0.0, out=None):
    _req(x, "cross_attention_rows.x", wq_packed.dtype)
    B, N, Cc = x.shape
    L1, L2 = k1.shape[1], (0 if k2 is None else k2.shape[1])
    if not xrows_ok(Cc, heads, L1, L2) or x.dtype not in FUSED_DTYPES:
        raise ValueError(f"cross_attention_rows: C={Cc} heads={heads} L1={L1} L2={L2} {x.dtype} outside the kernel envelope")
    if not x.is_contiguous():
        raise ValueError(f"cross_attention_rows.x: must be contiguous {x.dtype}")
    if out is None:
        out = torch.empty_like(x)
    d = L.XrowsDesc()
    d.x, d.wq_packed, d.wo_packed, d.bo, d.out = x.data_ptr(), wq_packed.data_ptr(), wo_packed.data_ptr(), _ptr(bo), out.data_ptr()
    d.k1, d.vt1, d.L1, d.Lpad1 = _rows_kv_args(k1, vt1, B, heads, Cc // heads, x.dtype, "cross_attention_rows.k1 / vt1")
    if ln is not None:
        d.ln_gamma, d.ln_beta, d.ln_eps = ln[0].data_ptr(), ln[1].data_ptr(), float(ln[2])
    d.key_bias = _ptr(key_bias)
    d.B, d.N, d.C, d.heads = B, N, Cc, heads
    if L2 > 0:
        d.k2, d.vt2, d.L2, d.Lpad2 = _rows_kv_args(k2, vt2, B, heads, Cc // heads, x.dtype, "cross_attention_rows.k2 / vt2")
    d.dtype, d.softmax_scale, d.scale2 = _DT[x.dtype], 1.0 / math.sqrt(Cc // heads), float(scale2)
    L.check(L.lib().apad_cross_attention_rows(C.byref(d), _stream()), "apad_cross_attention_rows")
    return out


SATTN_FUSED = True
SATTN_ENVELOPE = {256: (513, 1024), 384: (129, 256)}


def sattn_ok(x, heads):
    if not (SATTN_FUSED and x.dim() == 3 and x.dtype in FUSED_DTYPES and x.is_contiguous() and heads == 8):
        return False
    lo_hi = SATTN_ENVELOPE.get(x.shape[-1])
    return lo_hi is not None and lo_hi[0] <= x.shape[1] <= lo_hi[1]


def sattn_pack(wq, wk, wv, ln, heads):
    Cc = wq.shape[0]
    d = Cc // heads
    T3 = (3 * d + 31) // 32
    qs = LOG2E / math.sqrt(d)
    gamma, beta = ln[0].detach().float(), ln[1].detach().float()
    wf = torch.stack([wq.detach().float() * qs, wk.detach().float(), wv.detach().float()], 0)
    bb = wf @ beta
    wg = (wf * gamma).to(wq.dtype)
    cs = wg.float().sum(-1)
    per_head = lambda t: t.reshape(3, heads, d, *t.shape[2:]).transpose(0, 1).reshape(heads, 3 * d, *t.shape[2:])
    pad = T3 * 32 - 3 * d
    wh = torch.nn.functional.pad(per_head(wg), (0, 0, 0, pad))
    w = wh.reshape(heads, T3, 32, Cc // 16, 2, 8).permute(0, 1, 3, 4, 2, 5).contiguous().reshape(-1)
    csbb = torch.stack([torch.nn.functional.pad(per_head(cs), (0, pad)), torch.nn.functional.pad(per_head(bb), (0, pad))], 1).contiguous().reshape(-1)
    return w, csbb


def self_attention_fused(x, w_packed, csbb, heads, ln_eps, out=None):
    _req(x, "self_attention_fused.x", w_packed.dtype)
    B, N, Cc = x.shape
    if x.dtype not in FUSED_DTYPES or not x.is_contiguous() or csbb.dtype != torch.float32:
        raise ValueError("self_attention_fused: x must be contiguous 16-bit, colsum / bias fp32")
    if out is None:
        out = torch.empty_like(x)
    L.check(L.lib().apad_self_attention_fused(x.data_ptr(), w_packed.data_ptr(), csbb.data_ptr(), out.data_ptr(), B, N, Cc, heads, float(ln_eps),
                                              _DT[x.dtype], _stream()), "apad_self_attention_fused")
    return out


HS_C, HS_HEADS, HS_MAXN = 640, 8, 64
HS_ATTN = True


def hs_ok(x, heads, n_q_rows):
    return (HS_ATTN and x.dim() == 3 and x.shape[-1] == HS_C and x.shape[1] <= HS_MAXN and heads == HS_HEADS and n_q_rows == HS_C
            and x.dtype in FUSED_DTYPES and x.is_contiguous())


def hs_rows_ok(x):
    return x.dim() == 3 and x.shape[-1] == HS_C and x.shape[1] <= HS_MAXN and x.dtype in FUSED_DTYPES and x.is_contiguous()


def hs_cross_lengths_ok(L1, L2=0):
    return 1 <= L1 <= 64 and (0 <= L2 <= 64 or (L2 <= XROWS_MAXL2 and L1 <= 32))


def _hs_frag(w):
    lead = w.shape[:-2]
    n = len(lead)
    w = w.reshape(*lead, 5, 32, 40, 2, 8)
    return w.permute(*range(n), n, n + 2, n + 3, n + 1, n + 4)


def hs_pack_rows(w, ln=None, bias=None, scale=1.0):
    wf = w.detach().float()
    bb = None if bias is None else bias.detach().float()
    if ln is not None:
        bb = wf @ ln[1].detach().float() + (0.0 if bb is None else bb)
        wf = wf * ln[0].detach().float()
    if scale != 1.0:
        wf = wf * scale
        bb = None if bb is None else bb * scale
    pk = _hs_frag(wf.to(w.dtype).reshape(4, 160, HS_C)).contiguous().reshape(-1)
    return pk, (None if bb is None else bb.contiguous())


def hs_pack_qkv(wq, wk, wv, ln=None, q_scale=1.0):
    ws = [w.detach().float() for w in (wq, wk, wv)]
    bb = None
    if ln is not None:
        beta, gamma = ln[1].detach().float(), ln[0].detach().float()
        bb = [w @ beta for w in ws]
        ws = [w * gamma for w in ws]
    if q_scale != 1.0:
        ws[0] = ws[0] * q_scale
        if bb is not None:
            bb[0] = bb[0] * q_scale
    w = torch.stack(ws, 0).to(wq.dtype).reshape(3, 4, 160, HS_C).permute(1, 0, 2, 3)
    pk = _hs_frag(w).contiguous().reshape(-1)
    if bb is not None:
        bb = torch.stack(bb, 0).reshape(3, 4, 160).permute(1, 0, 2).contiguous().reshape(-1)
    return pk, bb


def hs_pack_geglu(w1, b1, ln=None):
    wf = w1.detach().float()
    bb = torch.zeros(wf.shape[0], device=wf.device) if b1 is None else b1.detach().float()
    if ln is not None:
        bb = wf @ ln[1].detach().float() + bb
        wf = wf * ln[0].detach().float()
    w = wf.to(w1.dtype).reshape(2, 4, 20, 32, 40, 2, 8).permute(1, 2, 0, 4, 5, 3, 6)
    return w.contiguous().reshape(-1), bb.reshape(2, 4, 20, 32).permute(1, 2, 0, 3).contiguous().reshape(-1)


def hs_geglu(x, w_packed, w_bias, normalize=True, ln_eps=1e-5, out=None):
    _req(x, "hs_geglu.x", w_packed.dtype)
    B, N, Cc = x.shape
    if Cc != HS_C or N > HS_MAXN or x.dtype not in FUSED_DTYPES or not x.is_contiguous():
        raise ValueError(f"hs_geglu: x {tuple(x.shape)} {x.dtype} outside the kernel envelope")
    if out is None:
        out = torch.empty(B, N, 4 * Cc, dtype=x.dtype, device=x.device)
    L.check(L.lib().apad_hs_geglu(x.data_ptr(), w_packed.data_ptr(), _ptr(w_bias), out.data_ptr(), B, N, Cc, int(bool(normalize)), float(ln_eps),
                                  _DT[x.dtype], _stream()), "apad_hs_geglu")
    return out


def hs_pack_ff2(w2):
    return w2.detach().reshape(4, 5, 32, 160, 2, 8).permute(0, 1, 3, 4, 2, 5).contiguous().reshape(-1)


def hs_ff2(h, w2_packed, bias, residual, rowstat=False, out=None):
    _req(h, "hs_ff2.h", w2_packed.dtype)
    B, N, K = h.shape
    if K != 4 * HS_C or N > HS_MAXN or h.dtype not in FUSED_DTYPES or not h.is_contiguous():
        raise ValueError(f"hs_ff2: h {tuple(h.shape)} outside the kernel envelope")
    if residual is not None:
        _req(residual, "hs_ff2.residual", h.dtype)
        if not residual.is_contiguous() or tuple(residual.shape) != (B, N, HS_C):
            raise ValueError(f"hs_ff2: residual {tuple(residual.shape)} must be contiguous [B, N, 640]")
    if out is None:
        out = torch.empty(B, N, HS_C, dtype=h.dtype, device=h.device)
    rs = torch.empty(B * N, 20, 2, dtype=torch.float32, device=h.device) if rowstat else None
    d = L.HsOutDesc()
    d.o, d.w_packed, d.bias, d.residual, d.out, d.rowstat_out = h.data_ptr(), w2_packed.data_ptr(), _ptr(bias), _ptr(residual), out.data_ptr(), _ptr(rs)
    d.B, d.N, d.C, d.dtype = B, N, HS_C, _DT[h.dtype]
    L.check(L.lib().apad_hs_ff2(C.byref(d), _stream()), "apad_hs_ff2")
    if rs is not None:
        out._apad_rowstat = rs
    elif hasattr(out, "_apad_rowstat"):
        del out._apad_rowstat
    return out


def hs_attention(x, w_packed, w_bias, *, self_attention, normalize=True, ln_eps=1e-5, k1=None, vt1=None, key_bias=None, k2=None, vt2=None,
                 scale2=0.0, q_prescaled=False, out=None):
    _req(x, "hs_attention.x", w_packed.dtype)
    B, N, Cc = x.shape
    if Cc != HS_C or N > HS_MAXN or x.dtype not in FUSED_DTYPES or not x.is_contiguous():
        raise ValueError(f"hs_attention: x {tuple(x.shape)} {x.dtype} outside the kernel envelope")
    d = L.HsAttnDesc()
    d.x, d.w_packed, d.w_bias = x.data_ptr(), w_packed.data_ptr(), _ptr(w_bias)
    if w_bias is not None and w_bias.dtype != torch.float32:
        raise ValueError("hs_attention.w_bias: must be fp32")
    if not self_attention:
        L1, L2 = k1.shape[1], (0 if k2 is None else k2.shape[1])
        if not hs_cross_lengths_ok(L1, L2):
            raise ValueError(f"hs_attention: segment lengths {L1} / {L2} outside the kernel envelope")
        d.k1, d.vt1, d.L1, d.Lpad1 = _rows_kv_args(k1, vt1, B, HS_HEADS, 80, x.dtype, "hs_attention.k1 / vt1")
        d.key_bias = _ptr(key_bias)
        if L2 > 0:
            d.k2, d.vt2, d.L2, d.Lpad2 = _rows_kv_args(k2, vt2, B, HS_HEADS, 80, x.dtype, "hs_attention.k2 / vt2")
    if out is None:
        out = torch.empty_like(x)
    d.out = out.data_ptr()
    d.B, d.N, d.C, d.heads = B, N, Cc, HS_HEADS
    d.self_attention, d.q_prescaled, d.dtype, d.normalize = int(bool(self_attention)), int(bool(q_prescaled)), _DT[x.dtype], int(bool(normalize))
    d.ln_eps, d.softmax_scale, d.scale2 = float(ln_eps), 1.0 / math.sqrt(80.0), float(scale2)
    L.check(L.lib().apad_hs_attention(C.byref(d), _stream()), "apad_hs_attention")
    return out


def hs_out(o, wo_packed, bias, residual, rowstat=False, out=None):
    _req(o, "hs_out.o", wo_packed.dtype)
    B, N, Cc = o.shape
    if Cc != HS_C or N > HS_MAXN or o.dtype not in FUSED_DTYPES or not o.is_contiguous():
        raise ValueError(f"hs_out: o {tuple(o.shape)} outside the kernel envelope")
    if residual is not None:
        _req(residual, "hs_out.residual", o.dtype)
        if not residual.is_contiguous() or residual.shape != o.shape:
            raise ValueError(f"hs_out: residual {tuple(residual.shape)} must be contiguous with the shape of o")
    if out is None:
        out = torch.empty_like(o)
    rs = torch.empty(B * N, 20, 2, dtype=torch.float32, device=o.device) if rowstat else None
    d = L.HsOutDesc()
    d.o, d.w_packed, d.bias, d.residual, d.out, d.rowstat_out = o.data_ptr(), wo_packed.data_ptr(), _ptr(bias), _ptr(residual), out.data_ptr(), _ptr(rs)
    d.B, d.N, d.C, d.dtype = B, N, Cc, _DT[o.dtype]
    L.check(L.lib().apad_hs_out(C.byref(d), _stream()), "apad_hs_out")
    if rs is not None:
        out._apad_rowstat = rs
    elif hasattr(out, "_apad_rowstat"):
        del out._apad_rowstat
    return out


MLP_C = (256,)
MLP_PACKED = True
MLP_PACKED_MIN_M = 48000


def mlp_pack(w1, b1, w2):
    _req(w1, "mlp_pack.w1")
    _req(w2, "mlp_pack.w2", w1.dtype)
    Cc = w2.shape[0]
    if Cc not in MLP_C or tuple(w1.shape) != (8 * Cc, Cc) or tuple(w2.shape) != (Cc, 4 * Cc) or w1.dtype not in FUSED_DTYPES or not (w1.is_contiguous() and w2.is_contiguous()):
        raise ValueError(f"mlp_pack: w1 {tuple(w1.shape)}, w2 {tuple(w2.shape)} {w1.dtype} outside the kernel envelope")
    if b1 is not None and (b1.dtype != w1.dtype or not b1.is_contiguous()):
        raise ValueError("mlp_pack.b1: must be contiguous and of the weights' dtype")
    wp = torch.empty(L.lib().apad_mlp_packed_bytes(Cc) // w1.element_size(), dtype=w1.dtype, device=w1.device)
    bp = torch.empty(L.lib().apad_mlp_packed_bias_floats(Cc), dtype=torch.float32, device=w1.device)
    L.check(L.lib().apad_mlp_pack(w1.data_ptr(), _ptr(b1), w2.data_ptr(), wp.data_ptr(), bp.data_ptr(), Cc, _DT[w1.dtype], _stream()), "apad_mlp_pack")
    return wp, bp


def geglu_mlp_packed(x, w_packed, b1_packed, b2, ln=None, out=None):
    _req(x, "geglu_mlp_packed.x", w_packed.dtype)
    Cc = x.shape[-1]
    if Cc not in MLP_C or x.dtype not in FUSED_DTYPES or not x.is_contiguous() or b1_packed.dtype != torch.float32:
        raise ValueError(f"geglu_mlp_packed: x {tuple(x.shape)} {x.dtype} outside the kernel envelope")
    if out is None:
        out = torch.empty_like(x)
    d = L.MlpDesc()
    d.x, d.b2, d.out = x.data_ptr(), _ptr(b2), out.data_ptr()
    if ln is not None:
        d.ln_gamma, d.ln_beta, d.ln_eps = ln[0].data_ptr(), ln[1].data_ptr(), float(ln[2])
    d.M, d.C, d.dtype = x.numel() // Cc, Cc, _DT[x.dtype]
    L.check(L.lib().apad_geglu_mlp_packed(C.byref(d), w_packed.data_ptr(), b1_packed.data_ptr(), _stream()), "apad_geglu_mlp_packed")
    return out


def geglu_mlp(x, w1, b1, w2, b2, ln=None, out=None):
    _req(x, "geglu_mlp.x", w1.dtype)
    Cc = x.shape[-1]
    if Cc not in MLP_C or w1.shape != (8 * Cc, Cc) or w2.shape != (Cc, 4 * Cc) or x.dtype not in FUSED_DTYPES:
        raise ValueError(f"geglu_mlp: C={Cc}, w1 {tuple(w1.shape)}, w2 {tuple(w2.shape)} outside the kernel envelope")
    if not (x.is_contiguous() and w1.is_contiguous() and w2.is_contiguous()):
        raise ValueError("geglu_mlp: operands must be contiguous")
    if out is None:
        out = torch.empty_like(x)
    d = L.MlpDesc()
    d.x, d.w1, d.b1, d.w2, d.b2, d.out = x.data_ptr(), w1.data_ptr(), _ptr(b1), w2.data_ptr(), _ptr(b2), out.data_ptr()
    if ln is not None:
        d.ln_gamma, d.ln_beta, d.ln_eps = ln[0].data_ptr(), ln[1].data_ptr(), float(ln[2])
    d.M, d.C, d.dtype = x.numel() // Cc, Cc, _DT[x.dtype]
    L.check(L.lib().apad_geglu_mlp(C.byref(d), _stream()), "apad_geglu_mlp")
    return out


GEGLU_PACKED_C = (384,)
GEGLU_PACKED_MIN_M = 12000


def geglu_pack(w1, b1):
    _req(w1, "geglu_pack.w1")
    Cc = w1.shape[1]
    if Cc not in GEGLU_PACKED_C or w1.shape[0] != 8 * Cc or w1.dtype not in FUSED_DTYPES or not w1.is_contiguous():
        raise ValueError(f"geglu_pack: w1 {tuple(w1.shape)} {w1.dtype} outside the kernel envelope")
    if b1 is not None and (b1.dtype != w1.dtype or not b1.is_contiguous()):
        raise ValueError("geglu_pack.b1: must be contiguous and of the weights' dtype")
    wp = torch.empty(L.lib().apad_geglu_packed_bytes(Cc) // w1.element_size(), dtype=w1.dtype, device=w1.device)
    bp = torch.empty(L.lib().apad_geglu_packed_bias_floats(Cc), dtype=torch.float32, device=w1.device)
    L.check(L.lib().apad_geglu_pack(w1.data_ptr(), _ptr(b1), wp.data_ptr(), bp.data_ptr(), Cc, _DT[w1.dtype], _stream()), "apad_geglu_pack")
    return wp, bp


def layernorm_geglu_packed(x, w_packed, b1_packed, ln=None, out=None):
    _req(x, "layernorm_geglu_packed.x", w_packed.dtype)
    Cc = x.shape[-1]
    if Cc not in GEGLU_PACKED_C or x.dtype not in FUSED_DTYPES or not x.is_contiguous() or b1_packed.dtype != torch.float32:
        raise ValueError(f"layernorm_geglu_packed: x {tuple(x.shape)} {x.dtype} outside the kernel envelope")
    if out is None:
        out = torch.empty(*x.shape[:-1], 4 * Cc, dtype=x.dtype, device=x.device)
    g, b, eps = (ln[0].data_ptr(), ln[1].data_ptr(), float(ln[2])) if ln is not None else (None, None, 0.0)
    L.check(L.lib().apad_layernorm_geglu_packed(x.data_ptr(), g, b, w_packed.data_ptr(), b1_packed.data_ptr(), out.data_ptr(), x.numel() // Cc, Cc, eps,
                                                _DT[x.dtype], _stream()), "apad_layernorm_geglu_packed")
    return out


def linear_vt(x, w, B, Lk, heads, out_vt, bias=None):
    _req(x, "linear_vt.x", w.dtype)
    K = x.shape[-1]
    Cc = w.shape[0]
    x2 = x.reshape(B * Lk, K)
    gemm(x2, w, M=B * Lk, N=Cc, K=K, lda=x2.stride(0), out=out_vt, ldo=0, out_mode=L.OUT_VT, bias=bias,
         vt=(heads, Cc // heads, Lk, out_vt.shape[-1]), ldw=w.stride(0))
    return out_vt


def linear_qkv(x, w_qkv, B, Lk, heads, q, k, vt, bias=None, ln=None, v=None):
    _req(x, "linear_qkv.x", w_qkv.dtype)
    fold = None
    if ln is not None:
        rs = rowstat_of(x)
        w_qkv, cs, bb = _ln_folded(w_qkv, bias, ln[0], ln[1])
        bias, fold = None, (rs, cs, bb, ln[2])
    K = x.shape[-1]
    C3 = w_qkv.shape[0]
    Cc = C3 // 3
    x2 = x.reshape(B * Lk, K)
    d = L.GemmDesc()
    d.a, d.out, d.out2, d.out3 = x2.data_ptr(), q.data_ptr(), k.data_ptr(), vt.data_ptr()
    d.out4 = _ptr(v)
    d.bias = _ptr(bias)
    d.M, d.N, d.K, d.lda, d.ldo = B * Lk, C3, K, x2.stride(0), Cc
    _set_w(d, w_qkv, C3, K, w_qkv.stride(0))
    d.a_mode, d.epilogue, d.out_mode = L.A_PLAIN, L.EPI_NONE, L.OUT_QKV
    d.heads, d.head_dim, d.L, d.Lpad = heads, Cc // heads, Lk, vt.shape[-1]
    if fold is not None:
        rs, cs, bb, eps = fold
        d.rowstat_in, d.ln_colsum, d.ln_bias, d.rowstat_in_tiles, d.ln_eps = rs.data_ptr(), cs.data_ptr(), bb.data_ptr(), rs.shape[-2], float(eps)
    L.check(L.lib().apad_gemm(C.byref(d), _stream()), "apad_gemm(qkv)")
    return q, k, vt


HCONV = True


def conv_halo_eligible(Cin, Cout, Wout, stride, dtype, src_batch_mod=0, asym_pad=False):
    wide = Cout % 128 == 0 and Wout in (2, 4, 8, 16)
    narrow = Cout in (8, 16) and Cin in (64, 128) and Wout in (4, 8, 16)
    return HCONV and stride == 1 and not asym_pad and src_batch_mod == 0 and dtype in FUSED_DTYPES and Cin % 64 == 0 and (wide or narrow)


def conv_halo_weight(w_packed):
    def make():
        wc = w_packed.detach().contiguous()
        Cout, K = wc.shape
        out = torch.empty(L.lib().apad_conv_halo_packed_bytes(Cout, K // 9) // 2, dtype=wc.dtype, device=wc.device)
        L.check(L.lib().apad_conv_halo_pack(wc.data_ptr(), out.data_ptr(), Cout, K // 9, _DT[wc.dtype], _stream()), "apad_conv_halo_pack")
        return out
    return derived(w_packed, "halo", make)


def conv3x3_pack(w):
    return w.detach().permute(0, 2, 3, 1).reshape(w.shape[0], -1).contiguous()


def conv3x3_weight(w):
    return derived(w, "conv3x3", lambda: conv3x3_pack(w))


def conv3x3(x, w_packed, bias, B, Hin, Win, stride=1, up=None, residual=None, rowgroup_bias=None, rows_per_group=0,
            step_ptr=None, src_batch_mod=0, out=None, asym_pad=False):
    _req(x, "conv3x3.x", w_packed.dtype)
    Cin = x.shape[-1]
    Cout = w_packed.shape[0]
    Hs, Ws = (up if up is not None else (Hin, Win))
    Hout = (Hs + (1 if asym_pad else 2) - 3) // stride + 1
    Wout = (Ws + (1 if asym_pad else 2) - 3) // stride + 1
    M = B * Hout * Wout
    if out is None:
        out = torch.empty(B, Hout * Wout, Cout, dtype=x.dtype, device=x.device)
    wh = ws = None
    if conv_halo_eligible(Cin, Cout, Wout, stride, w_packed.dtype, src_batch_mod, asym_pad):
        wh = conv_halo_weight(w_packed)
        nws = L.lib().apad_conv_halo_workspace_bytes(M, Cout, Cin, Wout)
        if nws:
            ws = torch.empty(nws // 4, dtype=torch.float32, device=x.device)
    gemm(x, w_packed, M=M, N=Cout, K=9 * Cin, lda=0, out=out, ldo=Cout, bias=bias, w_halo=wh, workspace=ws,
         residual=residual, ldr=Cout, rowgroup_bias=rowgroup_bias,
         ld_rg=(rowgroup_bias.stride(0) if rowgroup_bias is not None else 0), rows_per_group=rows_per_group,
         step_ptr=step_ptr, a_mode=L.A_CONV3X3, asym_pad=asym_pad,
         conv=(Hin, Win, Cin, Hout, Wout, stride, (up[0] if up else 0), (up[1] if up else 0), src_batch_mod))
    return out, Hout, Wout


def conv1d(x, w_packed, bias, taps, dilation=1, transposed_stride=0, pad=None, pre_slope=None, residual=None, act=None, out=None):
    _req(x, "conv1d.x", w_packed.dtype)
    B, T, Cin = x.shape
    Cout = w_packed.shape[0]
    s_ = int(transposed_stride)
    if pad is None:
        pad = (taps - s_) // 2 if s_ else (taps * dilation - dilation) // 2
    Tout = (T - 1) * s_ - 2 * pad + taps if s_ else T + 2 * pad - dilation * (taps - 1)
    if out is None:
        out = torch.empty(B, Tout, Cout, dtype=x.dtype, device=x.device)
    d = L.GemmDesc()
    d.a, d.out, d.bias, d.residual = x.data_ptr(), out.data_ptr(), _ptr(bias), _ptr(residual)
    d.M, d.N, d.K, d.lda, d.ldo, d.ldr = B * Tout, Cout, taps * Cin, 0, Cout, Cout
    _set_w(d, w_packed, Cout, taps * Cin, w_packed.stride(0))
    d.a_mode, d.epilogue, d.out_mode = L.A_CONV1D, _EPI[act], L.OUT_ROWMAJOR
    d.Hin, d.Hout, d.Cin, d.stride = T, Tout, Cin, max(s_, 1)
    d.taps, d.dilation, d.pad, d.transposed = taps, dilation, pad, 1 if s_ else 0
    if pre_slope is not None:
        d.a_pre_act, d.a_pre_slope = 1, float(pre_slope)
    d.rows_per_group = 1
    L.check(L.lib().apad_gemm(C.byref(d), _stream()), "apad_gemm(conv1d)")
    return out


def mix3(a, b, c, scale, out=None):
    _req(a, "mix3.a")
    if out is None:
        out = torch.empty_like(a)
    L.check(L.lib().apad_mix3(a.data_ptr(), b.data_ptr(), c.data_ptr(), out.data_ptr(), a.numel(), float(scale), _DT[a.dtype], _stream()),
            "apad_mix3")
    return out


def softmax_rows(x, scale=1.0, out=None, bias=None):
    _req(x, "softmax_rows.x")
    N = x.shape[-1]
    x2 = x.reshape(-1, N)
    if out is None:
        out = torch.empty_like(x2)
    b2 = None
    if bias is not None:
        b2 = _req(bias, "softmax_rows.bias", torch.float32).reshape(-1, N)
        if b2.shape[0] != x2.shape[0]:
            raise ValueError(f"softmax_rows: bias {tuple(bias.shape)} does not match x {tuple(x.shape)}")
    L.check(L.lib().apad_softmax_rows(x2.data_ptr(), _ptr(b2), out.data_ptr(), x2.shape[0], N, x2.stride(0), b2.stride(0) if b2 is not None else 0,
                                      out.stride(0), float(scale), _DT[x.dtype], _stream()), "apad_softmax_rows")
    return out.view(x.shape)


def rms_norm(x, gamma, eps):
    _req(x, "rms_norm.x", gamma.dtype)
    Cc = x.shape[-1]
    x2 = x.reshape(-1, Cc)
    out = torch.empty_like(x2)
    L.check(L.lib().apad_rmsnorm(x2.data_ptr(), gamma.data_ptr(), out.data_ptr(), x2.shape[0], Cc, x2.stride(0), Cc, float(eps), 0, _DT[x.dtype],
                                 _stream()), "apad_rmsnorm")
    return out.view(x.shape)


def l2_normalize(x, eps=1e-12):
    _req(x, "l2_normalize.x")
    Cc = x.shape[-1]
    x2 = x.reshape(-1, Cc)
    out = torch.empty_like(x2)
    L.check(L.lib().apad_rmsnorm(x2.data_ptr(), None, out.data_ptr(), x2.shape[0], Cc, x2.stride(0), Cc, float(eps), 1, _DT[x.dtype], _stream()),
            "apad_rmsnorm")
    return out.view(x.shape)


def embedding(table, ids):
    _req(table, "embedding.table")
    if ids.dtype != torch.int64 or not ids.is_cuda:
        raise RuntimeError("embedding.ids: expected an int64 GPU tensor")
    ids = ids.contiguous()
    out = torch.empty(*ids.shape, table.shape[1], dtype=table.dtype, device=table.device)
    L.check(L.lib().apad_gather_rows(table.data_ptr(), ids.data_ptr(), out.data_ptr(), ids.numel(), table.shape[0], table.shape[1],
                                     _DT[table.dtype], _stream()), "apad_gather_rows")
    return out


def gather_rows(table, ids):
    return embedding(table, ids)


def window_attention(qkv, bias, B, H, W, heads, shift, out=None):
    _req(qkv, "window_attention.qkv", torch.float32)
    _req(bias, "window_attention.bias", torch.float32)
    C3 = qkv.shape[-1]
    if C3 % (3 * heads) != 0:
        raise ValueError(f"window_attention: qkv width {C3} is not 3 * heads ({heads}) * head size")
    if not (qkv.is_contiguous() and bias.is_contiguous()) or qkv.numel() != B * H * W * C3 or tuple(bias.shape) != (heads, 64, 64):
        raise ValueError(f"window_attention: qkv {tuple(qkv.shape)} / bias {tuple(bias.shape)} do not match B={B} H={H} W={W} heads={heads}")
    if out is None:
        out = torch.empty(B * H * W, C3 // 3, dtype=torch.float32, device=qkv.device)
    L.check(L.lib().apad_window_attention(qkv.data_ptr(), bias.data_ptr(), out.data_ptr(), B, H, W, heads, C3 // (3 * heads), 8, int(shift),
                                          L.F32, _stream()), "apad_window_attention")
    return out


def clap_mel2img(x, bn_weight, bn_bias, bn_mean, bn_var, bn_eps, spec_size):
    _req(x, "clap_mel2img.x", torch.float32)
    if x.dim() != 4 or x.shape[1] != 1 or not x.is_contiguous():
        raise ValueError(f"clap_mel2img: input_features {tuple(x.shape)}: expected contiguous [B, 1, T, F]")
    B, _, T, F = x.shape
    for n, t in (("weight", bn_weight), ("bias", bn_bias), ("running_mean", bn_mean), ("running_var", bn_var)):
        if tuple(_req(t, f"clap_mel2img.{n}", torch.float32).shape) != (F,):
            raise ValueError(f"clap_mel2img: batch_norm {n} {tuple(t.shape)} does not match {F} mel bins")
    if spec_size % 4 or spec_size % F or T > spec_size * (spec_size // F):
        raise ValueError("the wav size should be less than or equal to the swin input size")
    out = torch.empty(B * (spec_size // 4) ** 2, 16, dtype=torch.float32, device=x.device)
    L.check(L.lib().apad_clap_mel2img(x.data_ptr(), bn_weight.data_ptr(), bn_bias.data_ptr(), bn_mean.data_ptr(), bn_var.data_ptr(),
                                      float(bn_eps), out.data_ptr(), B, T, F, spec_size, _stream()), "apad_clap_mel2img")
    return out


def chroma(x, offsets, offsets_host, window, twiddle, fb, out):
    for t, name in ((x, "x"), (window, "window"), (twiddle, "twiddle"), (fb, "fb"), (out, "out")):
        if not _req(t, "chroma." + name, torch.float32).is_contiguous():
            raise RuntimeError(f"chroma.{name}: must be contiguous")
    _req(offsets, "chroma.offsets", torch.int64)
    if offsets_host.is_cuda or offsets_host.dtype != torch.int64 or not offsets_host.is_contiguous():
        raise RuntimeError("chroma.offsets_host: expected a contiguous int64 host tensor")
    B = offsets_host.numel() - 1
    if offsets.numel() != B + 1 or out.dim() != 3 or out.shape[0] != B or out.shape[2] != 12:
        raise RuntimeError(f"chroma: offsets {tuple(offsets.shape)} / out {tuple(out.shape)} do not describe {B} clips as [B + 1] / [B, frames, 12]")
    if tuple(window.shape) != (2048,) or tuple(twiddle.shape) != (1024, 2) or tuple(fb.shape) != (12, 1025):
        raise RuntimeError("chroma: expected window [2048], twiddle [1024, 2] and fb [12, 1025]")
    if B and x.numel() < int(offsets_host[-1]):
        raise RuntimeError(f"chroma.x: {x.numel()} samples, the offsets end at {int(offsets_host[-1])}")
    L.check(L.lib().apad_chroma(x.data_ptr(), offsets.data_ptr(), offsets_host.data_ptr(), window.data_ptr(), twiddle.data_ptr(), fb.data_ptr(),
                                out.data_ptr(), B, out.shape[1], _stream()), "apad_chroma")
    return out


def chroma_similarity(a, b, ref_index, ref_index_host, frames, frames_host, out=None, per_frame=None):
    for t, name in ((a, "a"), (b, "b")):
        if not _req(t, "chroma_similarity." + name, torch.float32).is_contiguous() or t.dim() != 3 or t.shape[2] != 12:
            raise RuntimeError(f"chroma_similarity.{name}: expected a contiguous fp32 [clips, frames, 12] tensor, got {tuple(t.shape)}")
    n, T = a.shape[0], a.shape[1]
    if b.shape[1] != T:
        raise RuntimeError(f"chroma_similarity: a has {T} frames per clip, b has {b.shape[1]}")
    for d, h, name in ((ref_index, ref_index_host, "ref_index"), (frames, frames_host, "frames")):
        if _req(d, "chroma_similarity." + name, torch.int32).numel() != n or not d.is_contiguous():
            raise RuntimeError(f"chroma_similarity.{name}: expected {n} contiguous int32 values")
        if h.is_cuda or h.dtype != torch.int32 or h.numel() != n or not h.is_contiguous():
            raise RuntimeError(f"chroma_similarity.{name}_host: expected {n} contiguous int32 values on the host")
    if out is None:
        out = torch.empty(n, dtype=torch.float32, device=a.device)
    if _req(out, "chroma_similarity.out", torch.float32).numel() != n or not out.is_contiguous():
        raise RuntimeError(f"chroma_similarity.out: expected {n} contiguous fp32 values")
    if per_frame is not None and (tuple(_req(per_frame, "chroma_similarity.per_frame", torch.float32).shape) != (n, T) or not per_frame.is_contiguous()):
        raise RuntimeError(f"chroma_similarity.per_frame: expected a contiguous fp32 [{n}, {T}] tensor")
    L.check(L.lib().apad_chroma_similarity(a.data_ptr(), b.data_ptr(), ref_index.data_ptr(), ref_index_host.data_ptr(), frames.data_ptr(),
                                           frames_host.data_ptr(), out.data_ptr(), _ptr(per_frame), n, b.shape[0], T, _stream()),
            "apad_chroma_similarity")
    return out


def _host_table(t, name, dtype, n):
    if t.is_cuda or t.dtype != dtype or t.numel() != n or not t.is_contiguous():
        raise RuntimeError(f"{name}: expected {n} contiguous {dtype} values on the host")
    return t


def loudness(x, offsets, offsets_host, coef, powers, stats, hop, hop_energy=None):
    for t, name in ((x, "x"), (coef, "coef"), (powers, "powers"), (stats, "stats")) + (((hop_energy, "hop_energy"),) if hop_energy is not None else ()):
        if not _req(t, "loudness." + name, torch.float32).is_contiguous():
            raise RuntimeError(f"loudness.{name}: must be contiguous")
    _req(offsets, "loudness.offsets", torch.int64)
    B = offsets_host.numel() - 1
    _host_table(offsets_host, "loudness.offsets_host", torch.int64, B + 1)
    if B < 1 or offsets.numel() != B + 1 or not offsets.is_contiguous() or tuple(stats.shape) != (B, 4):
        raise RuntimeError(f"loudness: offsets {tuple(offsets.shape)} / stats {tuple(stats.shape)} do not describe {B} clips as [B + 1] / [B, 4]")
    if coef.numel() != 10 or tuple(powers.shape) != (2, 65, 2, 2, 2):
        raise RuntimeError("loudness: expected coef [10] and powers [2, 65, 2, 2, 2]")
    if hop_energy is not None and (hop_energy.dim() != 2 or hop_energy.shape[0] != B or hop_energy.shape[1] < 1):
        raise RuntimeError(f"loudness.hop_energy: expected [{B}, target_hops], got {tuple(hop_energy.shape)}")
    if x.numel() < int(offsets_host[-1]):
        raise RuntimeError(f"loudness.x: {x.numel()} samples, the offsets end at {int(offsets_host[-1])}")
    L.check(L.lib().apad_loudness(x.data_ptr(), offsets.data_ptr(), offsets_host.data_ptr(), coef.data_ptr(), powers.data_ptr(), stats.data_ptr(),
                                  _ptr(hop_energy), B, int(hop), 0 if hop_energy is None else hop_energy.shape[1], _stream()), "apad_loudness")
    return stats


def loudness_gain(x, offsets, offsets_host, stats, out, gains, peak_limit, target=None, ref_stats=None, ref_index=None, ref_index_host=None):
    by_ref = ref_stats is not None or ref_index is not None or ref_index_host is not None
    if by_ref == (target is not None) or (by_ref and (ref_stats is None or ref_index is None or ref_index_host is None)):
        raise RuntimeError("loudness_gain: give either target, or ref_stats with ref_index and ref_index_host")
    for t, name in ((x, "x"), (stats, "stats"), (out, "out"), (gains, "gains")) + (((ref_stats, "ref_stats"),) if by_ref else ((target, "target"),)):
        if not _req(t, "loudness_gain." + name, torch.float32).is_contiguous():
            raise RuntimeError(f"loudness_gain.{name}: must be contiguous")
    _req(offsets, "loudness_gain.offsets", torch.int64)
    B = offsets_host.numel() - 1
    _host_table(offsets_host, "loudness_gain.offsets_host", torch.int64, B + 1)
    if B < 1 or offsets.numel() != B + 1 or not offsets.is_contiguous() or tuple(stats.shape) != (B, 4) or gains.numel() != B:
        raise RuntimeError(f"loudness_gain: offsets {tuple(offsets.shape)} / stats {tuple(stats.shape)} / gains {tuple(gains.shape)} do not describe "
                           f"{B} clips")
    if x.numel() < int(offsets_host[-1]) or out.numel() < int(offsets_host[-1]):
        raise RuntimeError(f"loudness_gain: x {x.numel()} / out {out.numel()} samples, the offsets end at {int(offsets_host[-1])}")
    m = 0
    if by_ref:
        if ref_stats.dim() != 2 or ref_stats.shape[1] != 4 or ref_stats.shape[0] < 1:
            raise RuntimeError(f"loudness_gain.ref_stats: expected [m, 4], got {tuple(ref_stats.shape)}")
        m = ref_stats.shape[0]
        if _req(ref_index, "loudness_gain.ref_index", torch.int32).numel() != B or not ref_index.is_contiguous():
            raise RuntimeError(f"loudness_gain.ref_index: expected {B} contiguous int32 values")
        _host_table(ref_index_host, "loudness_gain.ref_index_host", torch.int32, B)
    elif target.numel() != B:
        raise RuntimeError(f"loudness_gain.target: expected {B} values")
    L.check(L.lib().apad_loudness_gain(x.data_ptr(), offsets.data_ptr(), offsets_host.data_ptr(), stats.data_ptr(), _ptr(target), _ptr(ref_stats),
                                       _ptr(ref_index), _ptr(ref_index_host), out.data_ptr(), gains.data_ptr(), B, m, float(peak_limit), _stream()),
            "apad_loudness_gain")
    return out


def gaussian_sample(moments, noise, scale=1.0):
    _req(moments, "gaussian_sample.moments")
    _req(noise, "gaussian_sample.noise", moments.dtype)
    rows, L2 = moments.shape
    if not (moments.is_contiguous() and noise.is_contiguous() and tuple(noise.shape) == (rows, L2 // 2)):
        raise ValueError(f"gaussian_sample: moments {tuple(moments.shape)} / noise {tuple(noise.shape)} must be contiguous [rows, 2L] / [rows, L]")
    out = torch.empty_like(noise)
    L.check(L.lib().apad_gaussian_sample(moments.data_ptr(), noise.data_ptr(), out.data_ptr(), rows, L2 // 2, float(scale), _DT[moments.dtype],
                                         _stream()), "apad_gaussian_sample")
    return out


def patch_embed(mel, w, bias, dtype):
    _req(mel, "patch_embed.mel", torch.float32)
    B, H, W = mel.shape
    n_tok = (H // 16) * (W // 16)
    out = torch.empty(B, n_tok, w.shape[0], dtype=dtype, device=mel.device)
    gemm(mel, w, M=B * n_tok, N=w.shape[0], K=256, lda=0, out=out, ldo=w.shape[0], bias=bias, a_mode=L.A_PATCH16,
         conv=(H, W, 1, H // 16, W // 16, 1, 0, 0, 0))
    return out


LOG2E = 1.4426950408889634


def attention(q, k, vt, Lk, heads, key_bias=None, k2=None, vt2=None, L2=0, scale2=0.0, kv_batch_div=1,
              kv2_batch_div=1, out=None, q_prescaled=False):
    _req(q, "attention.q")
    _req(k, "attention.k", q.dtype)
    _req(vt, "attention.vt", q.dtype)
    B, N, Cc = q.shape
    d_head = Cc // heads
    if out is None:
        out = torch.empty(B, N, Cc, dtype=q.dtype, device=q.device)
    d = L.AttnDesc()
    d.q, d.k, d.vt, d.out = q.data_ptr(), k.data_ptr(), vt.data_ptr(), out.data_ptr()
    d.key_bias = _ptr(key_bias)
    d.q_stride_b, d.q_stride_n = q.stride(0), q.stride(1)
    d.k_stride_b, d.k_stride_l, d.vt_stride_b = k.stride(0), k.stride(1), vt.stride(0)
    d.o_stride_b, d.o_stride_n = out.stride(0), out.stride(1)
    d.B, d.N, d.H, d.D, d.L, d.Lpad = B, N, heads, d_head, Lk, vt.shape[-1]
    d.kv_batch_div, d.kv2_batch_div = kv_batch_div, kv2_batch_div
    d.dtype = _f32_dtype(q.dtype)
    d.softmax_scale = 1.0 / math.sqrt(d_head)
    d.scale2 = float(scale2)
    d.q_prescaled = 1 if q_prescaled else 0
    if L2 > 0:
        d.k2, d.vt2 = k2.data_ptr(), vt2.data_ptr()
        d.k2_stride_b, d.k2_stride_l, d.vt2_stride_b = k2.stride(0), k2.stride(1), vt2.stride(0)
        d.L2, d.Lpad2 = L2, vt2.shape[-1]
    L.check(L.lib().apad_attention(C.byref(d), _stream()), "apad_attention")
    return out


def layer_norm(x, gamma, beta, eps, out=None):
    _req(x, "layer_norm.x", gamma.dtype)
    Cc = x.shape[-1]
    M = x.numel() // Cc
    if out is None:
        out = torch.empty_like(x)
    L.check(L.lib().apad_layernorm(x.data_ptr(), gamma.data_ptr(), beta.data_ptr(), out.data_ptr(), M, Cc, Cc, Cc,
                                   eps, _DT[x.dtype], _stream()), "apad_layernorm")
    return out


_gn_ws = {}


def _gn_workspace(dev, B, HW, groups):
    key = (dev, B, HW, groups, torch.cuda.current_stream().cuda_stream)
    ws = _gn_ws.get(key)
    if ws is None:
        ws = torch.empty(L.lib().apad_groupnorm_workspace_bytes(B, HW, groups) // 4, dtype=torch.float32, device=dev)
        _gn_ws[key] = ws
    return ws


def group_norm(x, gamma, beta, groups, eps, silu=False, out=None):
    _req(x, "group_norm.x", gamma.dtype)
    B, HW, Cc = x.shape
    ws = _gn_workspace(x.device, B, HW, groups)
    if out is None:
        out = torch.empty_like(x)
    L.check(L.lib().apad_groupnorm(x.data_ptr(), gamma.data_ptr(), beta.data_ptr(), out.data_ptr(), ws.data_ptr(), B, HW,
                                   Cc, groups, eps, 1 if silu else 0, _DT[x.dtype], _stream()), "apad_groupnorm")
    return out


def group_norm2(xa, xb, gamma, beta, groups, eps, silu=False):
    _req(xa, "group_norm2.xa", gamma.dtype)
    _req(xb, "group_norm2.xb", gamma.dtype)
    Ba, HW, Ca = xa.shape
    Bb, HWb, Cb = xb.shape
    B = max(Ba, Bb)
    if HWb != HW or B % Ba or B % Bb or not (xa.is_contiguous() and xb.is_contiguous()) or xa.dtype not in FUSED_DTYPES:
        raise ValueError(f"group_norm2: xa {tuple(xa.shape)}, xb {tuple(xb.shape)} {xa.dtype}")
    ws = _gn_workspace(xa.device, B, HW, groups)
    out = torch.empty(B, HW, Ca + Cb, dtype=xa.dtype, device=xa.device)
    L.check(L.lib().apad_groupnorm2(xa.data_ptr(), xb.data_ptr(), gamma.data_ptr(), beta.data_ptr(), out.data_ptr(), ws.data_ptr(), B, Ba, Bb,
                                    HW, Ca, Cb, groups, eps, 1 if silu else 0, _DT[xa.dtype], _stream()), "apad_groupnorm2")
    return out


def audiomae_pool(rep, tp, fp, out_dtype=None):
    _req(rep, "audiomae_pool.rep")
    B = rep.shape[0]
    out_dtype = out_dtype or rep.dtype
    out = torch.empty(B, (64 // tp) * (8 // fp), 768, dtype=out_dtype, device=rep.device)
    L.check(L.lib().apad_audiomae_pool(rep.data_ptr(), out.data_ptr(), B, tp, fp, _DT[rep.dtype], _DT[out_dtype],
                                       _stream()), "apad_audiomae_pool")
    return out


def timestep_embedding(t, dim, flip_sin_to_cos, freq_shift, dtype):
    _req(t, "timestep_embedding.t", torch.float32)
    out = torch.empty(t.numel(), dim, dtype=dtype, device=t.device)
    L.check(L.lib().apad_timestep_embedding(t.data_ptr(), out.data_ptr(), t.numel(), dim, 1 if flip_sin_to_cos else 0,
                                            float(freq_shift), _DT[dtype], _stream()), "apad_timestep_embedding")
    return out


def cfg_ddim_step(eps2, latents, unet_in, coef, step_ptr, guidance_scale, eps_out=None):
    _req(latents, "cfg_ddim_step.latents", torch.float32)
    B = latents.shape[0]
    n = latents.numel() // B
    L.check(L.lib().apad_cfg_ddim_step(eps2.data_ptr(), latents.data_ptr(), unet_in.data_ptr(), _ptr(eps_out),
                                       coef.data_ptr(), _ptr(step_ptr), float(guidance_scale), B, n, _DT[eps2.dtype],
                                       _stream()), "apad_cfg_ddim_step")


def _cfg_step(fn, branches, eps, latents, unet_in, coef, step_ptr, eps_out, history, noise, keep=None, x0=None, z0=None, mask=None, channels=8):
    _req(latents, fn + ".latents", torch.float32)
    if branches == 3 and (eps.numel() != 3 * latents.numel() or (eps.dim() > 1 and eps.shape[0] != 3 * latents.shape[0])):
        raise RuntimeError(f"{fn}: eps3 must hold three branches [3B, n] of latents [B, n] = {tuple(latents.shape)}, got {tuple(eps.shape)}")
    _req(coef, fn + ".coef", torch.float32)
    if coef.dim() != 2 or coef.shape[1] != 6 or not coef.is_contiguous():
        raise RuntimeError(f"{fn}.coef: expected a contiguous [steps, 6] table, got {tuple(coef.shape)}")
    steps = coef.shape[0]
    B = latents.shape[0]
    n = latents.numel() // B
    if eps.dtype != unet_in.dtype or eps.numel() != branches * latents.numel() or unet_in.numel() != latents.numel():
        raise RuntimeError(f"{fn}: eps{branches} [{branches}B, n] and unet_in [B, n] must share the model dtype and match latents [B, n]")
    numel = latents.numel()
    for t, name, want in ((eps_out, "eps_out", numel), (history, "history", numel), (noise, "noise", steps * numel), (x0, "x0", numel),
                          (z0, "z0", numel), (keep, "keep", 2 * steps)):
        if t is not None and (_req(t, f"{fn}.{name}", torch.float32).numel() != want or not t.is_contiguous()):
            raise RuntimeError(f"{fn}.{name}: expected {want} contiguous fp32 values, got {tuple(t.shape)}")
    mask_batch = 0
    if mask is not None:
        _req(mask, fn + ".mask", torch.float32)
        channels = int(channels)
        if mask.dim() != 2 or not mask.is_contiguous() or (channels > 0 and n % channels == 0 and mask.shape[1] != n // channels):
            raise RuntimeError(f"{fn}.mask: expected a contiguous [1 or B, n / channels] table with n = {n}, channels = {channels}, "
                               f"got {tuple(mask.shape)}")
        mask_batch = mask.shape[0]
    return ((eps.data_ptr(), latents.data_ptr(), unet_in.data_ptr(), _ptr(eps_out), _ptr(history), _ptr(noise), coef.data_ptr()),
            (_ptr(keep), _ptr(x0), _ptr(z0), _ptr(mask), mask_batch, int(channels)), (_ptr(step_ptr), steps), (B, n, _DT[eps.dtype], _stream()))


def cfg_sampler_step(eps2, latents, unet_in, coef, step_ptr, guidance_scale, eps_out=None, history=None, noise=None):
    bufs, _, step, geom = _cfg_step("cfg_sampler_step", 2, eps2, latents, unet_in, coef, step_ptr, eps_out, history, noise)
    L.check(L.lib().apad_cfg_sampler_step(*bufs, *step, float(guidance_scale), *geom), "apad_cfg_sampler_step")


def cfg_edit_step(eps2, latents, unet_in, coef, keep, step_ptr, guidance_scale, x0, z0, mask, channels=8, eps_out=None, history=None, noise=None):
    bufs, edit, step, geom = _cfg_step("cfg_edit_step", 2, eps2, latents, unet_in, coef, step_ptr, eps_out, history, noise, keep, x0, z0, mask, channels)
    L.check(L.lib().apad_cfg_edit_step(*bufs, *edit, *step, float(guidance_scale), *geom), "apad_cfg_edit_step")


def cfg_dual_step(eps3, latents, unet_in, coef, guidance, step_ptr, eps_out=None, history=None, noise=None, keep=None, x0=None, z0=None, mask=None,
                  channels=8):
    fn = "cfg_dual_step"
    bufs, edit, step, geom = _cfg_step(fn, 3, eps3, latents, unet_in, coef, step_ptr, eps_out, history, noise, keep, x0, z0, mask, channels)
    _req(guidance, fn + ".guidance", torch.float32)
    if guidance.dim() != 2 or tuple(guidance.shape) != (step[1], 2) or not guidance.is_contiguous():
        raise RuntimeError(f"{fn}.guidance: expected a contiguous fp32 [{step[1]}, 2] table of (s_A, s_T), got {tuple(guidance.shape)}")
    if not eps3.is_contiguous():
        raise RuntimeError(f"{fn}: eps3 must be contiguous")
    L.check(L.lib().apad_cfg_dual_step(*bufs, guidance.data_ptr(), *edit, *step, *geom), "apad_cfg_dual_step")


def cfg_shaped_step(eps, latents, unet_in, coef, shape, step_ptr, guidance_scale=None, guidance=None, momentum=None, stats=None, eps_out=None,
                    history=None, noise=None, keep=None, x0=None, z0=None, mask=None, channels=8):
    fn = "cfg_shaped_step"
    if (guidance is None) == (guidance_scale is None):
        raise RuntimeError(f"{fn}: pass guidance_scale (two branches) or the guidance table (three branches), not both or neither")
    branches = 2 if guidance is None else 3
    if branches == 2 and eps.dim() > 1 and eps.shape[0] != 2 * latents.shape[0]:
        raise RuntimeError(f"{fn}: eps2 must hold two branches [2B, n] of latents [B, n] = {tuple(latents.shape)}, got {tuple(eps.shape)}")
    bufs, edit, step, geom = _cfg_step(fn, branches, eps, latents, unet_in, coef, step_ptr, eps_out, history, noise, keep, x0, z0, mask, channels)
    for t, name, want in ((guidance, "guidance", (step[1], 2)), (shape, "shape", (step[1], 4)), (stats, "stats", (geom[0], 8))):
        if t is not None and (_req(t, f"{fn}.{name}", torch.float32).dim() != 2 or tuple(t.shape) != want or not t.is_contiguous()):
            raise RuntimeError(f"{fn}.{name}: expected a contiguous fp32 {list(want)} table, got {tuple(t.shape)}")
    if shape is None:
        raise RuntimeError(f"{fn}.shape: required")
    if momentum is not None and (_req(momentum, fn + ".momentum", torch.float32).numel() != (branches - 1) * latents.numel()
                                 or not momentum.is_contiguous()):
        raise RuntimeError(f"{fn}.momentum: expected {(branches - 1) * latents.numel()} contiguous fp32 values [{branches - 1}, B, n], got "
                           f"{tuple(momentum.shape)}")
    for t, name in ((eps, "eps"), (unet_in, "unet_in"), (latents, "latents")):
        if not t.is_contiguous():
            raise RuntimeError(f"{fn}.{name}: must be contiguous")
    for t in (eps, unet_in, coef, shape, guidance, momentum, stats, step_ptr, eps_out, history, noise, keep, x0, z0, mask):
        if t is not None and t.device != latents.device:
            raise RuntimeError(f"{fn}: every operand must live on latents' device {latents.device}, got {t.device}")
    L.check(L.lib().apad_cfg_shaped_step(*bufs, _ptr(guidance), shape.data_ptr(), _ptr(momentum), _ptr(stats), *edit, *step,
                                         0.0 if guidance_scale is None else float(guidance_scale), branches, *geom), "apad_cfg_shaped_step")


def cfg_invert_step(eps, latents, unet_in, coef, keep, x0, noise, step_ptr, guidance_scale=None, guidance=None, eps_out=None):
    fn = "cfg_invert_step"
    if (guidance is None) == (guidance_scale is None):
        raise RuntimeError(f"{fn}: pass guidance_scale (two branches) or the guidance table (three branches), not both or neither")
    branches = 2 if guidance is None else 3
    if branches == 2 and (eps.dim() > 1 and latents.dim() > 0 and eps.shape[0] != 2 * latents.shape[0]):
        raise RuntimeError(f"{fn}: eps2 must hold two branches [2B, n] of latents [B, n] = {tuple(latents.shape)}, got {tuple(eps.shape)}")
    for t, name in ((keep, "keep"), (x0, "x0"), (noise, "noise")):
        if t is None:
            raise RuntimeError(f"{fn}.{name}: required")
    for t, name in ((eps, "eps"), (unet_in, "unet_in")):
        if not _req(t, f"{fn}.{name}").is_contiguous():
            raise RuntimeError(f"{fn}.{name}: must be contiguous")
    if not latents.is_contiguous():
        raise RuntimeError(f"{fn}.latents: must be contiguous")
    bufs, edit, step, geom = _cfg_step(fn, branches, eps, latents, unet_in, coef, step_ptr, eps_out, None, noise, keep, x0)
    if noise.shape[0] != step[1] or keep.shape[0] != step[1]:
        raise RuntimeError(f"{fn}: noise {tuple(noise.shape)}, coef {tuple(coef.shape)} and keep {tuple(keep.shape)} must have one row per step")
    if guidance is not None:
        _req(guidance, fn + ".guidance", torch.float32)
        if tuple(guidance.shape) != (step[1], 2) or not guidance.is_contiguous():
            raise RuntimeError(f"{fn}.guidance: expected a contiguous fp32 [{step[1]}, 2] table of (s_A, s_T), got {tuple(guidance.shape)}")
    for t in (eps, unet_in, coef, keep, x0, noise, step_ptr, guidance, eps_out):
        if t is not None and t.device != latents.device:
            raise RuntimeError(f"{fn}: every operand must live on latents' device {latents.device}, got {t.device}")
    eps_p, lat_p, unet_p, eps_out_p, _, noise_p, coef_p = bufs
    L.check(L.lib().apad_cfg_invert_step(eps_p, lat_p, unet_p, eps_out_p, noise_p, coef_p, _ptr(guidance), edit[0], edit[1], *step,
                                         0.0 if guidance_scale is None else float(guidance_scale), branches, *geom), "apad_cfg_invert_step")


def edit_start(z0, x0, latents, unet_in, a, s, moments=None, post_noise=None, scale=1.0):
    _req(z0, "edit_start.z0", torch.float32)
    numel = z0.numel()
    for t, name in ((x0, "x0"), (latents, "latents")):
        if _req(t, "edit_start." + name, torch.float32).numel() != numel or not t.is_contiguous():
            raise RuntimeError(f"edit_start.{name}: expected {numel} contiguous fp32 values, got {tuple(t.shape)}")
    _req(unet_in, "edit_start.unet_in")
    if unet_in.numel() != numel or not unet_in.is_contiguous() or not z0.is_contiguous():
        raise RuntimeError(f"edit_start: z0 and unet_in must be contiguous with {numel} values")
    if moments is None:
        Lc = z0.shape[-1]
        if post_noise is not None:
            raise RuntimeError("edit_start.post_noise: given without moments")
    else:
        _req(moments, "edit_start.moments", unet_in.dtype)
        if moments.dim() != 2 or not moments.is_contiguous() or moments.numel() != 2 * numel:
            raise RuntimeError(f"edit_start.moments: expected a contiguous [rows, 2L] tensor of {2 * numel} values, got {tuple(moments.shape)}")
        Lc = moments.shape[1] // 2
        if post_noise is None or _req(post_noise, "edit_start.post_noise", torch.float32).numel() != numel or not post_noise.is_contiguous():
            raise RuntimeError(f"edit_start.post_noise: expected {numel} contiguous fp32 values")
    L.check(L.lib().apad_edit_start(_ptr(moments), _ptr(post_noise), z0.data_ptr(), x0.data_ptr(), latents.data_ptr(), unet_in.data_ptr(), float(a),
                                    float(s), float(scale), numel // Lc, Lc, _DT[unet_in.dtype], _stream()), "apad_edit_start")


def step_advance(step_ptr):
    L.check(L.lib().apad_step_advance(step_ptr.data_ptr(), _stream()), "apad_step_advance")


def attention_lse(q, k, vt, Lk, heads, key_bias=None):
    _req(q, "attention_lse.q")
    B, N, Cc = q.shape
    out = torch.empty_like(q)
    lse = torch.empty(B, heads, round_up(N, 32), dtype=torch.float32, device=q.device)
    d = L.AttnDesc()
    d.q, d.k, d.vt, d.out, d.key_bias, d.lse = q.data_ptr(), k.data_ptr(), vt.data_ptr(), out.data_ptr(), _ptr(key_bias), lse.data_ptr()
    d.q_stride_b, d.q_stride_n = q.stride(0), q.stride(1)
    d.k_stride_b, d.k_stride_l, d.vt_stride_b = k.stride(0), k.stride(1), vt.stride(0)
    d.o_stride_b, d.o_stride_n = out.stride(0), out.stride(1)
    d.B, d.N, d.H, d.D = B, N, heads, Cc // heads
    d.L, d.Lpad, d.L2, d.Lpad2 = Lk, vt.shape[-1], 0, 0
    d.kv_batch_div, d.kv2_batch_div, d.dtype = 1, 1, _f32_dtype(q.dtype)
    d.softmax_scale, d.scale2 = 1.0 / math.sqrt(Cc // heads), 0.0
    L.check(L.lib().apad_attention(C.byref(d), _stream()), "apad_attention")
    return out, lse


def head_transpose(x, heads, pad=None):
    _req(x, "head_transpose.x")
    B, N, Cc = x.shape
    pad = pad or round_up(N, 32)
    xt = torch.empty(B, heads, Cc // heads, pad, dtype=x.dtype, device=x.device)
    L.check(L.lib().apad_head_transpose(x.data_ptr(), xt.data_ptr(), B, N, heads, Cc // heads, pad, _DT[x.dtype], _stream()),
            "apad_head_transpose")
    return xt


def head_transpose_many(xs, heads, pad):
    B, N, Cc = xs[0].shape
    outs = [torch.empty(B, heads, Cc // heads, pad, dtype=x.dtype, device=x.device) for x in xs]
    for i in range(0, len(xs), 3):
        a = [(_req(x, "head_transpose.x").data_ptr(), y.data_ptr()) for x, y in zip(xs[i:i + 3], outs[i:i + 3])]
        a += [(None, None)] * (3 - len(a))
        L.check(L.lib().apad_head_transpose3(a[0][0], a[0][1], a[1][0], a[1][1], a[2][0], a[2][1], B, N, heads, Cc // heads, pad,
                                             _DT[xs[0].dtype], _stream()), "apad_head_transpose3")
    return outs


def attention_bwd(q, k, v, out, dout, lse, heads, key_bias=None, dout_scale=1.0, need_dkv=True, dq=None, packed=False):
    for t, n in ((q, "q"), (k, "k"), (v, "v"), (out, "out"), (dout, "dout")):
        _req(t, "attention_bwd." + n, q.dtype)
        if not t.is_contiguous():
            raise RuntimeError(f"attention_bwd.{n}: must be contiguous")
    B, N, Cc = q.shape
    Lk = k.shape[1]
    Npad, Lpad = round_up(N, 32), round_up(Lk, 32)
    d = L.AttnBwdDesc()
    f32 = q.dtype == torch.float32
    same = need_dkv and not f32 and N == Lk
    if same:
        kt, qt, dot = head_transpose_many([k, q, dout], heads, Lpad)
    else:
        kt = None if f32 else head_transpose(k, heads, Lpad)
    keep = [kt]
    d.q, d.k, d.v, d.kt, d.out, d.dout, d.lse = (q.data_ptr(), k.data_ptr(), v.data_ptr(), _ptr(kt), out.data_ptr(),
                                                 dout.data_ptr(), lse.data_ptr())
    d.key_bias = _ptr(key_bias)
    delta = torch.empty(B, heads, Npad, dtype=torch.float32, device=q.device)
    d.delta = delta.data_ptr()
    acc = dq is not None
    packed = packed and need_dkv and not f32 and dq is None and N == Lk
    dk = dv = None
    if packed:
        buf = torch.empty(B, N, 3 * Cc, dtype=q.dtype, device=q.device)
        dq, dk, dv = buf[..., :Cc], buf[..., Cc:2 * Cc], buf[..., 2 * Cc:]
        d.ld_grad = 3 * Cc
    elif dq is None:
        dq = torch.empty_like(q)
    d.dq = dq.data_ptr()
    if need_dkv:
        if not packed:
            dk, dv = torch.empty_like(k), torch.empty_like(v)
        d.dk, d.dv = dk.data_ptr(), dv.data_ptr()
        if not f32:
            if not same:
                qt, dot = head_transpose_many([q, dout], heads, Npad)
            keep += [qt, dot]
            d.qt, d.doutt = qt.data_ptr(), dot.data_ptr()
    d.B, d.N, d.H, d.D, d.L, d.Npad, d.Lpad, d.dtype = B, N, heads, Cc // heads, Lk, Npad, Lpad, _DT[q.dtype]
    d.softmax_scale, d.dout_scale, d.accumulate_dq = 1.0 / math.sqrt(Cc // heads), float(dout_scale), 1 if acc else 0
    L.check(L.lib().apad_attention_bwd(C.byref(d), _stream()), "apad_attention_bwd")
    return dq, dk, dv


def layer_norm_bwd(x, gamma, dy, eps, dres=None):
    _req(x, "layer_norm_bwd.x", gamma.dtype)
    Cc = x.shape[-1]
    dx = torch.empty_like(x)
    if dres is not None:
        _req(dres, "layer_norm_bwd.dres", x.dtype)
        if not dres.is_contiguous() or dres.shape != x.shape:
            raise ValueError("layer_norm_bwd.dres: must be contiguous and shaped like x")
    L.check(L.lib().apad_layernorm_bwd_add(x.data_ptr(), gamma.data_ptr(), dy.data_ptr(), _ptr(dres), dx.data_ptr(), x.numel() // Cc, Cc,
                                           eps, _DT[x.dtype], _stream()), "apad_layernorm_bwd")
    return dx


def group_norm_bwd(x, gamma, beta, dy, groups, eps, silu):
    _req(x, "group_norm_bwd.x", gamma.dtype)
    B, HW, Cc = x.shape
    dx = torch.empty_like(x)
    L.check(L.lib().apad_groupnorm_bwd(x.data_ptr(), gamma.data_ptr(), beta.data_ptr(), dy.data_ptr(), dx.data_ptr(), B, HW,
                                       Cc, groups, eps, 1 if silu else 0, _DT[x.dtype], _stream()), "apad_groupnorm_bwd")
    return dx


def geglu(proj):
    _req(proj, "geglu.proj")
    N = proj.shape[-1] // 2
    h = torch.empty(*proj.shape[:-1], N, dtype=proj.dtype, device=proj.device)
    L.check(L.lib().apad_geglu(proj.data_ptr(), h.data_ptr(), proj.numel() // (2 * N), N, _DT[proj.dtype], _stream()), "apad_geglu")
    return h


def geglu_bwd(proj, dh):
    N = proj.shape[-1] // 2
    dproj = torch.empty_like(proj)
    L.check(L.lib().apad_geglu_bwd(proj.data_ptr(), dh.data_ptr(), dproj.data_ptr(), proj.numel() // (2 * N), N,
                                   _DT[proj.dtype], _stream()), "apad_geglu_bwd")
    return dproj


def upsample_nearest_bwd(dup, B, H, W, Hup, Wup):
    Cc = dup.shape[-1]
    dx = torch.empty(B, H * W, Cc, dtype=dup.dtype, device=dup.device)
    L.check(L.lib().apad_upsample_nearest_bwd(dup.data_ptr(), dx.data_ptr(), B, H, W, Hup, Wup, Cc, _DT[dup.dtype], _stream()),
            "apad_upsample_nearest_bwd")
    return dx


def zero_stuff2(dy, B, H, W, Ho, Wo):
    Cc = dy.shape[-1]
    z = torch.empty(B, H * W, Cc, dtype=dy.dtype, device=dy.device)
    L.check(L.lib().apad_zero_stuff2(dy.data_ptr(), z.data_ptr(), B, H, W, Ho, Wo, Cc, _DT[dy.dtype], _stream()), "apad_zero_stuff2")
    return z


def transpose_pad(x, Mpad):
    M, Cc = x.shape
    xt = torch.empty(Cc, Mpad, dtype=x.dtype, device=x.device)
    L.check(L.lib().apad_transpose_pad(x.data_ptr(), xt.data_ptr(), M, Cc, Mpad, _DT[x.dtype], _stream()), "apad_transpose_pad")
    return xt


def weight_grad(dy, x, fp32=False, acc=None):
    M, N = dy.shape
    K = x.shape[-1]
    Mpad = round_up(M, 64)
    dy, x = dy.contiguous(), x.contiguous()
    if fp32 and dy.dtype in FUSED_DTYPES:
        dyt = torch.empty(N, Mpad, dtype=torch.float32, device=dy.device)
        xt = torch.empty(K, Mpad, dtype=torch.float32, device=dy.device)
        L.check(L.lib().apad_transpose_pad2(dy.data_ptr(), dyt.data_ptr(), N, x.data_ptr(), xt.data_ptr(), K, M, Mpad, _DT[dy.dtype], 1, _stream()),
                "apad_transpose_pad2")
    else:
        dyt, xt = transpose_pad(dy, Mpad), transpose_pad(x, Mpad)
        if fp32:
            dyt, xt = dyt.float(), xt.float()
    if acc is not None:
        if not (fp32 and acc.dtype == torch.float32 and acc.is_contiguous() and tuple(acc.shape) == (N, K)):
            raise ValueError("weight_grad(acc=...): needs fp32=True and a contiguous fp32 [N, K] accumulator")
        gemm(dyt, xt, M=N, N=K, K=Mpad, lda=Mpad, out=acc, ldo=K, ldw=Mpad, residual=acc, ldr=K, exact=True)
        return None
    out = torch.empty(N, K, dtype=dyt.dtype, device=dy.device)
    gemm(dyt, xt, M=N, N=K, K=Mpad, lda=Mpad, out=out, ldo=K, ldw=Mpad, exact=True)
    return out


def _reduce_ws(dev):
    return torch.empty(L.lib().apad_reduce_workspace_bytes() // 4, dtype=torch.float32, device=dev)


def mse_loss_grad(pred, target, grad_scale=1.0):
    _req(pred, "mse_loss_grad.pred")
    _req(target, "mse_loss_grad.target", torch.float32)
    loss = torch.empty(1, dtype=torch.float32, device=pred.device)
    dpred = torch.empty_like(pred)
    ws = _reduce_ws(pred.device)
    L.check(L.lib().apad_mse_loss_grad(pred.data_ptr(), target.data_ptr(), dpred.data_ptr(), loss.data_ptr(), ws.data_ptr(),
                                       pred.numel(), float(grad_scale), _DT[pred.dtype], _stream()), "apad_mse_loss_grad")
    return loss, dpred


def step_advance_if_finite(step_ptr, grad_norm_t):
    L.check(L.lib().apad_step_advance_if_finite(step_ptr.data_ptr(), _ptr(grad_norm_t), _stream()), "apad_step_advance_if_finite")


def grad_norm(grad, out=None, ws=None):
    _req(grad, "grad_norm.grad", torch.float32)
    out = out if out is not None else torch.empty(1, dtype=torch.float32, device=grad.device)
    ws = ws if ws is not None else _reduce_ws(grad.device)
    L.check(L.lib().apad_grad_norm(grad.data_ptr(), out.data_ptr(), ws.data_ptr(), grad.numel(), _stream()), "apad_grad_norm")
    return out


def adamw_step(param, work, grad, exp_avg, exp_avg_sq, grad_norm_t, step_t, lr, betas, eps, weight_decay, max_grad_norm):
    for t, n in ((param, "param"), (grad, "grad"), (exp_avg, "exp_avg"), (exp_avg_sq, "exp_avg_sq")):
        _req(t, "adamw_step." + n, torch.float32)
    L.check(L.lib().apad_adamw_step(param.data_ptr(), _ptr(work), grad.data_ptr(), exp_avg.data_ptr(), exp_avg_sq.data_ptr(),
                                    _ptr(grad_norm_t), step_t.data_ptr(), param.numel(), lr, betas[0], betas[1], eps,
                                    weight_decay, max_grad_norm if max_grad_norm else 0.0,
                                    _DT[work.dtype] if work is not None else L.BF16, _stream()), "apad_adamw_step")
```

include/apadapter_hip.h:

```cpp
#ifndef APADAPTER_HIP_H
#define APADAPTER_HIP_H

#include <stdint.h>

#ifdef __cplusplus
extern "C" {
#endif

#define APAD_ABI_VERSION 12

enum { APAD_BF16 = 0, APAD_F16 = 1, APAD_F32 = 2, APAD_F32_BF16X3 = 3 };

enum {
    APAD_A_PLAIN = 0,
    APAD_A_CONV3X3 = 1,
    APAD_A_PATCH16 = 2,
    APAD_A_CONV1D = 4
};

enum {
    APAD_EPI_NONE = 0, APAD_EPI_SILU = 1, APAD_EPI_GELU = 2, APAD_EPI_GEGLU = 3, APAD_EPI_TANH = 4,
    APAD_EPI_RELU = 5,
    APAD_EPI_GELU_TANH = 6,
    APAD_EPI_GEGLU_TANH = 7
};

enum {
    APAD_OUT_ROWMAJOR = 0,
    APAD_OUT_VT = 1,
    APAD_OUT_QKV = 2
};

typedef struct apad_gemm_desc {
    const void* a;
    const void* w;
    void* out;
    const void* bias;
    const void* residual;
    const void* rowgroup_bias;
    const int32_t* step_ptr;
    int64_t M, N, K;
    int64_t lda, ldw, ldo, ldr, ld_rg;
    int64_t rows_per_group;
    int32_t a_mode, epilogue, out_mode, dtype;
    int32_t Hin, Win, Cin;
    int32_t Hout, Wout;
    int32_t stride;
    int32_t Hup, Wup;
    int32_t src_batch_mod;
    int32_t residual_row_mod;
    int32_t heads, head_dim, L, Lpad;
    void* out2;
    void* out3;
    int32_t taps, dilation, pad, transposed;
    int32_t a_pre_act;
    float a_pre_slope;
    int32_t conv_asym_pad;
    int32_t reserved_conv;
    float* rowstat_out;
    const float* rowstat_in;
    const float* ln_colsum;
    const float* ln_bias;
    int32_t rowstat_in_tiles;
    float ln_eps;
    const void* a2;
    int64_t lda2;
    int32_t k_split;
    int32_t a_row_mod, a2_row_mod;
    int32_t reserved_a2;
    void* out4;
    const void* w_halo;
    void* workspace;
    int64_t workspace_bytes;
} apad_gemm_desc;

typedef struct apad_attn_desc {
    const void* q;
    const void* k;
    const void* vt;
    const void* k2;
    const void* vt2;
    void* out;
    const float* key_bias;
    float* lse;
    int64_t q_stride_b, q_stride_n;
    int64_t k_stride_b, k_stride_l, vt_stride_b;
    int64_t k2_stride_b, k2_stride_l, vt2_stride_b;
    int64_t o_stride_b, o_stride_n;
    int32_t B, N, H, D;
    int32_t L, Lpad, L2, Lpad2;
    int32_t kv_batch_div;
    int32_t kv2_batch_div;
    int32_t dtype;
    float softmax_scale;
    float scale2;
    int32_t q_prescaled;
} apad_attn_desc;

typedef struct apad_rp_segment {
    void* out;
    const void* bias;
    int64_t ldo;
    int32_t n_cols;
    int32_t mode;
} apad_rp_segment;

typedef struct apad_rp_desc {
    const void* x;
    const void* w;
    const void* ln_gamma;
    const void* ln_beta;
    const void* residual;
    int64_t M, lda, ldw, ldr;
    int32_t K;
    int32_t epilogue;
    int32_t dtype, n_segments;
    float ln_eps;
    int32_t heads, head_dim, L, Lpad;
    apad_rp_segment seg[3];
} apad_rp_desc;

typedef struct apad_mlp_desc {
    const void* x;
    const void* ln_gamma;
    const void* ln_beta;
    const void* w1;
    const void* b1;
    const void* w2;
    const void* b2;
    void* out;
    int64_t M;
    int32_t C, dtype;
    float ln_eps;
    int32_t reserved;
} apad_mlp_desc;

typedef struct apad_xattn_desc {
    const void* x;
    const void* ln_gamma;
    const void* ln_beta;
    const void* wq_packed;
    const void* wo_packed;
    const void* bo;
    const void* kv1_packed;
    const float* key_bias;
    const void* kv2_packed;
    void* out;
    const float* q_fold;
    int32_t B, N, C, heads;
    int32_t L1, L2;
    int32_t dtype, reserved;
    float ln_eps, softmax_scale, scale2, reserved_f;
} apad_xattn_desc;
int apad_sizeof_xattn_desc(void);
int apad_echo_xattn_desc(const apad_xattn_desc* d, double* out, int cap);
int apad_fused_cross_attention(const apad_xattn_desc* d, void* stream);

typedef struct apad_xrows_desc {
    const void* x;
    const void* ln_gamma;
    const void* ln_beta;
    const void* wq_packed;
    const void* wo_packed;
    const void* bo;
    const void* k1;
    const void* vt1;
    const float* key_bias;
    const void* k2;
    const void* vt2;
    void* out;
    int32_t B, N, C, heads;
    int32_t L1, Lpad1, L2, Lpad2;
    int32_t dtype, reserved;
    float ln_eps, softmax_scale, scale2, reserved_f;
} apad_xrows_desc;
int apad_sizeof_xrows_desc(void);
int apad_cross_attention_rows(const apad_xrows_desc* d, void* stream);
int64_t apad_rows_packed_kv_bytes(int32_t B, int32_t heads, int32_t head_dim, int32_t L);
int apad_rows_pack_kv(const void* k, const void* vt, void* out, int32_t B, int32_t heads, int32_t head_dim, int32_t L, int32_t Lpad, int32_t dtype, void* stream);
typedef struct apad_hs_attn_desc {
    const void* x;
    const void* w_packed;
    const float* w_bias;
    const void* k1;
    const void* vt1;
    const float* key_bias;
    const void* k2;
    const void* vt2;
    void* out;
    int32_t B, N, C, heads;
    int32_t L1, Lpad1, L2, Lpad2;
    int32_t self_attention, q_prescaled, dtype;
    int32_t normalize;
    float ln_eps, softmax_scale, scale2, reserved_f;
} apad_hs_attn_desc;
int apad_sizeof_hs_attn_desc(void);
int apad_hs_attention(const apad_hs_attn_desc* d, void* stream);
typedef struct apad_hs_out_desc {
    const void* o;
    const void* w_packed;
    const void* bias;
    const void* residual;
    void* out;
    float* rowstat_out;
    int32_t B, N, C, dtype;
} apad_hs_out_desc;
int apad_sizeof_hs_out_desc(void);
int apad_hs_out(const apad_hs_out_desc* d, void* stream);
int apad_hs_ff2(const apad_hs_out_desc* d, void* stream);
int apad_self_attention_fused(const void* x, const void* w_packed, const float* colsum_bias, void* out, int32_t B, int32_t N, int32_t C, int32_t heads,
                              float ln_eps, int32_t dtype, void* stream);
int apad_hs_geglu(const void* x, const void* w_packed, const float* w_bias, void* out, int32_t B, int32_t N, int32_t C, int32_t normalize, float ln_eps,
                  int32_t dtype, void* stream);
int64_t apad_mlp_packed_bytes(int32_t C);
int64_t apad_mlp_packed_bias_floats(int32_t C);
int apad_mlp_pack(const void* w1, const void* b1, const void* w2, void* w_packed, float* b1_packed, int32_t C, int32_t dtype, void* stream);
int apad_geglu_mlp_packed(const apad_mlp_desc* d, const void* w_packed, const float* b1_packed, void* stream);
int64_t apad_geglu_packed_bytes(int32_t C);
int64_t apad_geglu_packed_bias_floats(int32_t C);
int apad_geglu_pack(const void* w1, const void* b1, void* w_packed, float* b1_packed, int32_t C, int32_t dtype, void* stream);
int apad_layernorm_geglu_packed(const void* x, const void* ln_gamma, const void* ln_beta, const void* w_packed, const float* b1_packed, void* out, int64_t M,
                                int32_t C, float ln_eps, int32_t dtype, void* stream);
int apad_xattn_pack_weight(const void* w, void* packed, int64_t ldw, int32_t dtype, void* stream);
int64_t apad_xattn_packed_kv_bytes(int32_t B, int32_t L);
int apad_xattn_pack_kv(const void* k, const void* vt, void* packed, int32_t B, int32_t L, int32_t Lpad, int64_t k_stride_b,
                       int64_t k_stride_l, int64_t vt_stride_b, int32_t dtype, void* stream);

const char* apad_last_error(void);
int apad_abi_version(void);
int apad_set_gemm_ring(int32_t mode);
int apad_sizeof_gemm_desc(void);
int apad_sizeof_attn_desc(void);
int apad_echo_gemm_desc(const apad_gemm_desc* d, double* out, int cap);
int apad_echo_attn_desc(const apad_attn_desc* d, double* out, int cap);
int apad_sizeof_rp_desc(void);
int apad_echo_rp_desc(const apad_rp_desc* d, double* out, int cap);
int apad_sizeof_mlp_desc(void);
int apad_echo_mlp_desc(const apad_mlp_desc* d, double* out, int cap);

int apad_gemm(const apad_gemm_desc* d, void* stream);
int apad_conv_halo_pack(const void* w, void* out, int64_t N, int64_t Cin, int32_t dtype, void* stream);
int64_t apad_conv_halo_packed_bytes(int64_t N, int64_t Cin);
int64_t apad_conv_halo_workspace_bytes(int64_t M, int64_t N, int64_t Cin, int32_t Wout);
int apad_probe_mfma(void* sink, int32_t mode, int32_t iters, double* flops, void* stream);
int64_t apad_hconv_launch_count(void);
int apad_f32_split_weight(const void* w, void* out, int64_t N, int64_t K, int64_t ldw, void* stream);
int64_t apad_f32x3_launch_count(void);
int apad_attention(const apad_attn_desc* d, void* stream);
int apad_rowpanel_gemm(const apad_rp_desc* d, void* stream);
int apad_geglu_mlp(const apad_mlp_desc* d, void* stream);

int apad_layernorm(const void* x, const void* gamma, const void* beta, void* out, int64_t M, int32_t C,
                   int64_t ldx, int64_t ldo, float eps, int32_t dtype, void* stream);

int64_t apad_groupnorm_workspace_bytes(int32_t B, int32_t HW, int32_t G);
int apad_groupnorm(const void* x, const void* gamma, const void* beta, void* out, void* workspace, int32_t B,
                   int32_t HW, int32_t C, int32_t G, float eps, int32_t silu, int32_t dtype, void* stream);
int apad_groupnorm2(const void* xa, const void* xb, const void* gamma, const void* beta, void* out, void* workspace, int32_t B,
                    int32_t Ba, int32_t Bb, int32_t HW, int32_t Ca, int32_t Cb, int32_t G, float eps, int32_t silu, int32_t dtype,
                    void* stream);

int apad_audiomae_pool(const void* rep, void* out, int32_t B, int32_t tp, int32_t fp, int32_t dtype,
                       int32_t out_dtype, void* stream);

int apad_timestep_embedding(const float* t, void* out, int32_t n, int32_t dim, int32_t flip_sin_to_cos,
                            float freq_shift, int32_t dtype, void* stream);

int apad_cfg_ddim_step(const void* eps2, float* latents, void* unet_in, float* eps_out, const float* coef,
                       const int32_t* step_ptr, float guidance_scale, int32_t B, int64_t n, int32_t dtype,
                       void* stream);
int apad_step_advance(int32_t* step_ptr, void* stream);
int apad_cfg_sampler_step(const void* eps2, float* latents, void* unet_in, float* eps_out, float* history, const float* noise,
                          const float* coef, const int32_t* step_ptr, int32_t n_steps, float guidance_scale, int32_t B, int64_t n,
                          int32_t dtype, void* stream);
int apad_cfg_edit_step(const void* eps2, float* latents, void* unet_in, float* eps_out, float* history, const float* noise,
                       const float* coef, const float* keep, const float* x0, const float* z0, const float* mask, int32_t mask_batch,
                       int32_t C, const int32_t* step_ptr, int32_t n_steps, float guidance_scale, int32_t B, int64_t n, int32_t dtype,
                       void* stream);
int apad_cfg_dual_step(const void* eps3, float* latents, void* unet_in, float* eps_out, float* history, const float* noise,
                       const float* coef, const float* guidance, const float* keep, const float* x0, const float* z0, const float* mask,
                       int32_t mask_batch, int32_t C, const int32_t* step_ptr, int32_t n_steps, int32_t B, int64_t n, int32_t dtype,
                       void* stream);
int apad_cfg_shaped_step(const void* eps, float* latents, void* unet_in, float* eps_out, float* history, const float* noise, const float* coef,
                         const float* guidance, const float* shape, float* momentum, float* stats, const float* keep, const float* x0,
                         const float* z0, const float* mask, int32_t mask_batch, int32_t C, const int32_t* step_ptr, int32_t n_steps,
                         float guidance_scale, int32_t branches, int32_t B, int64_t n, int32_t dtype, void* stream);
int apad_cfg_invert_step(const void* eps, float* latents, void* unet_in, float* eps_out, float* noise, const float* coef, const float* guidance,
                         const float* keep, const float* x0, const int32_t* step_ptr, int32_t n_steps, float guidance_scale, int32_t branches,
                         int32_t B, int64_t n, int32_t dtype, void* stream);
int apad_edit_start(const void* moments, const float* post_noise, const float* z0, float* x0_out, float* latents, void* unet_in, float a,
                    float s, float scale, int64_t rows, int32_t Lc, int32_t dtype, void* stream);
int apad_mix3(const void* a, const void* b, const void* c, void* out, int64_t n, float scale, int32_t dtype, void* stream);

int apad_softmax_rows(const void* x, const float* bias, void* out, int64_t M, int32_t N, int64_t ldx, int64_t ldb, int64_t ldo,
                      float scale, int32_t dtype, void* stream);

int apad_rmsnorm(const void* x, const void* gamma, void* out, int64_t M, int32_t C, int64_t ldx, int64_t ldo, float eps,
                 int32_t mode, int32_t dtype, void* stream);

int apad_gather_rows(const void* table, const int64_t* ids, void* out, int64_t n, int64_t rows, int32_t C, int32_t dtype,
                     void* stream);

int apad_gaussian_sample(const void* moments, const void* noise, void* out, int64_t rows, int32_t latent, float scale,
                         int32_t dtype, void* stream);

typedef struct apad_attn_bwd_desc {
    const void* q;
    const void* k;
    const void* v;
    const void* qt;
    const void* kt;
    const void* out;
    const void* dout;
    const void* doutt;
    const float* lse;
    const float* key_bias;
    float* delta;
    void* dq;
    void* dk;
    void* dv;
    int32_t B, N, H, D, L, Npad, Lpad, dtype;
    float softmax_scale;
    float dout_scale;
    int32_t accumulate_dq;
    int32_t ld_grad;
} apad_attn_bwd_desc;
int apad_sizeof_attn_bwd_desc(void);
int apad_echo_attn_bwd_desc(const apad_attn_bwd_desc* d, double* out, int cap);
int apad_attention_bwd(const apad_attn_bwd_desc* d, void* stream);
int apad_head_transpose(const void* x, void* xt, int32_t B, int32_t N, int32_t H, int32_t D, int32_t pad, int32_t dtype,
                        void* stream);
int apad_head_transpose3(const void* x0, void* xt0, const void* x1, void* xt1, const void* x2, void* xt2, int32_t B, int32_t N,
                         int32_t H, int32_t D, int32_t pad, int32_t dtype, void* stream);

int apad_layernorm_bwd(const void* x, const void* gamma, const void* dy, void* dx, int64_t M, int32_t C, float eps,
                       int32_t dtype, void* stream);
int apad_layernorm_bwd_add(const void* x, const void* gamma, const void* dy, const void* dres, void* dx, int64_t M, int32_t C, float eps,
                           int32_t dtype, void* stream);
int apad_groupnorm_bwd(const void* x, const void* gamma, const void* beta, const void* dy, void* dx, int32_t B, int32_t HW,
                       int32_t C, int32_t G, float eps, int32_t silu, int32_t dtype, void* stream);
int apad_geglu(const void* proj, void* h, int64_t M, int32_t N, int32_t dtype, void* stream);
int apad_geglu_bwd(const void* proj, const void* dh, void* dproj, int64_t M, int32_t N, int32_t dtype, void* stream);
int apad_upsample_nearest_bwd(const void* dup, void* dx, int32_t B, int32_t H, int32_t W, int32_t Hup, int32_t Wup,
                              int32_t C, int32_t dtype, void* stream);
int apad_zero_stuff2(const void* dy, void* z, int32_t B, int32_t H, int32_t W, int32_t Ho, int32_t Wo, int32_t C,
                     int32_t dtype, void* stream);
int apad_transpose_pad(const void* x, void* xt, int32_t M, int32_t C, int32_t Mpad, int32_t dtype, void* stream);
int apad_transpose_pad2(const void* x0, void* xt0, int32_t C0, const void* x1, void* xt1, int32_t C1, int32_t M, int32_t Mpad,
                        int32_t dtype, int32_t out_f32, void* stream);

int64_t apad_reduce_workspace_bytes(void);
int apad_mse_loss_grad(const void* pred, const float* target, void* dpred, float* loss, float* workspace, int64_t n,
                       float grad_scale, int32_t dtype, void* stream);
int apad_grad_norm(const float* grad, float* norm, float* workspace, int64_t n, void* stream);
int apad_step_advance_if_finite(int32_t* step, const float* grad_norm, void* stream);
int apad_adamw_step(float* param, void* work, const float* grad, float* exp_avg, float* exp_avg_sq, const float* grad_norm,
                    const int32_t* step, int64_t n, float lr, float beta1, float beta2, float eps, float weight_decay,
                    float max_grad_norm, int32_t dtype, void* stream);

int apad_resample_fir(const float* x, const float* kernel, float* out, int64_t n_in, int64_t n_out, int32_t orig,
                      int32_t newf, int32_t width, void* stream);
int apad_kaldi_fbank(const float* x, int64_t n_samples, float dc, const float* window, const float* twiddle,
                     const float* mel, float* out, int32_t target_frames, int32_t num_mel_bins, float preemphasis,
                     float norm_mean, float norm_std, void* stream);

int apad_wav_stats(const float* x, const int64_t* offsets, const int64_t* offsets_host, float* stats, int32_t batch,
                   void* stream);
int apad_stft_logmel(const float* x, const int64_t* offsets, const int64_t* offsets_host, const float* stats,
                     const float* window, const float* twiddle, const float* mel, const int32_t* mel_range, float* out,
                     int32_t batch, int64_t segment, int32_t target_frames, void* stream);

int apad_window_attention(const void* qkv, const float* bias, void* out, int32_t B, int32_t H, int32_t W, int32_t heads,
                          int32_t head_dim, int32_t window, int32_t shift, int32_t dtype, void* stream);
int apad_clap_mel2img(const float* x, const float* bn_weight, const float* bn_bias, const float* bn_mean, const float* bn_var,
                      float bn_eps, float* out, int32_t B, int32_t T, int32_t F, int32_t spec_size, void* stream);

int apad_clap_logmel(const float* x, const int64_t* offsets, const int64_t* offsets_host, const int64_t* starts,
                     const int64_t* starts_host, const float* kernel, int32_t orig, int32_t newf, int32_t width,
                     const float* window, const float* twiddle, const float* mel, const int32_t* mel_range, float* out,
                     int32_t batch, int64_t max_length, int32_t hop, int32_t n_mels, int32_t padding, void* stream);

int apad_chroma(const float* x, const int64_t* offsets, const int64_t* offsets_host, const float* window, const float* twiddle,
                const float* fb, float* out, int32_t batch, int32_t target_frames, void* stream);
int apad_chroma_similarity(const float* a, const float* b, const int32_t* ref_index, const int32_t* ref_index_host,
                           const int32_t* frames, const int32_t* frames_host, float* out, float* per_frame, int32_t n, int32_t m,
                           int32_t T, void* stream);

int apad_loudness(const float* x, const int64_t* offsets, const int64_t* offsets_host, const float* coef, const float* powers,
                  float* stats, float* hop_energy, int32_t batch, int32_t hop, int32_t target_hops, void* stream);
int apad_loudness_gain(const float* x, const int64_t* offsets, const int64_t* offsets_host, const float* stats, const float* target,
                       const float* ref_stats, const int32_t* ref_index, const int32_t* ref_index_host, float* out, float* gains,
                       int32_t batch, int32_t n_ref, float peak_limit, void* stream);

#ifdef __cplusplus
}
#endif
#endif
```

Baseline: 4.651 clips/s.

## Fold nearest-x2 upsample into halo conv3x3 via per-phase 2x2 collapsed weights

Adds an upsample-folded path to the halo conv3x3 kernel. Each of the four output parity classes (plus bottom-row classes for odd heights) reads the low-resolution source directly and runs a 2x2 tap conv with pre-summed weights, so the upsampled activation is never materialised. This cuts MACs per output from 9 taps to 4 and shrinks the A-tile load. The cost is a new weight-packing kernel, a scattered output and residual row mapping in the epilogue, and more template code paths. It applies only to source widths 2, 4 or 8 with Cout divisible by 128, and the autograd forward keeps the old path.

Result: no change. 4.672 clips/s, median of 6 (+0.4%).

```diff
diff --git a/ap-adapter_amd/_lib.py b/ap-adapter_amd/_lib.py
--- a/ap-adapter_amd/_lib.py
+++ b/ap-adapter_amd/_lib.py
@@ -24,7 +24,7 @@
                                     "stride", "Hup", "Wup", "src_batch_mod", "residual_row_mod", "heads", "head_dim", "L", "Lpad")] + \
                [("out2", _vp), ("out3", _vp)] + \
                [(n, _i32) for n in ("taps", "dilation", "pad", "transposed", "a_pre_act")] + [("a_pre_slope", _f32)] + \
-               [("conv_asym_pad", _i32), ("reserved_conv", _i32)] + \
+               [("conv_asym_pad", _i32), ("halo_up2", _i32)] + \
                [(n, _vp) for n in ("rowstat_out", "rowstat_in", "ln_colsum", "ln_bias")] + [("rowstat_in_tiles", _i32), ("ln_eps", _f32)] + \
                [("a2", _vp), ("lda2", _i64), ("k_split", _i32), ("a_row_mod", _i32), ("a2_row_mod", _i32), ("reserved_a2", _i32), ("out4", _vp),
                 ("w_halo", _vp), ("workspace", _vp), ("workspace_bytes", _i64)]
@@ -129,6 +129,8 @@
     "apad_f32x3_launch_count": (_i64, []),
     "apad_probe_mfma": (C.c_int, [_vp, _i32, _i32, C.POINTER(C.c_double), _vp]),
     "apad_conv_halo_packed_bytes": (_i64, [_i64, _i64]),
+    "apad_conv_halo_pack_up2": (C.c_int, [_vp, _vp, _i64, _i64, _i32, _vp]),
+    "apad_conv_halo_up2_packed_bytes": (_i64, [_i64, _i64]),
     "apad_conv_halo_workspace_bytes": (_i64, [_i64, _i64, _i64, _i32]),
     "apad_attention": (C.c_int, [C.POINTER(AttnDesc), _vp]),
     "apad_layernorm": (C.c_int, [_vp, _vp, _vp, _vp, _i64, _i32, _i64, _i64, _f32, _i32, _vp]),
diff --git a/ap-adapter_amd/autograd.py b/ap-adapter_amd/autograd.py
--- a/ap-adapter_amd/autograd.py
+++ b/ap-adapter_amd/autograd.py
@@ -214,7 +214,7 @@
         ctx.has_res = residual is not None
         out, Ho, Wo = ops.conv3x3(_c(x), _conv_fwd_w(w), b, B, H, W, stride=stride, up=up,
                                   residual=None if residual is None else _c(residual), rowgroup_bias=rowgroup_bias,
-                                  rows_per_group=rows_per_group)
+                                  rows_per_group=rows_per_group, up_fold=False)
         ctx.out_hw = (Ho, Wo)
         return out
 
diff --git a/ap-adapter_amd/csrc/capi.cpp b/ap-adapter_amd/csrc/capi.cpp
--- a/ap-adapter_amd/csrc/capi.cpp
+++ b/ap-adapter_amd/csrc/capi.cpp
@@ -60,7 +60,7 @@
     PUT(d->src_batch_mod); PUT(d->residual_row_mod); PUT(d->heads); PUT(d->head_dim); PUT(d->L); PUT(d->Lpad);
     PUTP(d->out2); PUTP(d->out3);
     PUT(d->taps); PUT(d->dilation); PUT(d->pad); PUT(d->transposed); PUT(d->a_pre_act); PUT(d->a_pre_slope);
-    PUT(d->conv_asym_pad); PUT(d->reserved_conv);
+    PUT(d->conv_asym_pad); PUT(d->halo_up2);
     PUTP(d->rowstat_out); PUTP(d->rowstat_in); PUTP(d->ln_colsum); PUTP(d->ln_bias); PUT(d->rowstat_in_tiles); PUT(d->ln_eps);
     PUTP(d->a2); PUT(d->lda2); PUT(d->k_split); PUT(d->a_row_mod); PUT(d->a2_row_mod); PUT(d->reserved_a2);
     PUTP(d->out4); PUTP(d->w_halo); PUTP(d->workspace); PUT(d->workspace_bytes);
diff --git a/ap-adapter_amd/csrc/hconv.hip b/ap-adapter_amd/csrc/hconv.hip
--- a/ap-adapter_amd/csrc/hconv.hip
+++ b/ap-adapter_amd/csrc/hconv.hip
@@ -24,6 +24,10 @@
     int32_t ksplit;
     float* partial;
     uint32_t a_bytes, w_bytes;
+    int32_t Ho, Wo;
+    int32_t mt_n, mt_b;
+    int32_t Rn, Rb;
+    int32_t Hb;
 };
 
 template <int... S, class F> __device__ __forceinline__ void h_for_each(std::integer_sequence<int, S...>, F&& f) {
@@ -42,16 +46,18 @@
     static constexpr int NSTG = 4;
     static constexpr int PBW = STAGE_B / 1024 / NW;
     static constexpr int SPT = 4 / KS;
-    static constexpr int SPC = 9 * SPT;
     static constexpr int OFF_B = ABUF, OFF_A1 = OFF_B + NSTG * STAGE_B, OFF_Z = OFF_A1 + ABUF, SMEM = OFF_Z + 256;
     static constexpr int OFF_STG = OFF_B + (NSTG - 1) * STAGE_B, STG_BYTES = STAGE_B + ABUF;
     static_assert(STAGE_B % (1024 * NW) == 0 && (KS == 2 || KS == 4) && SMEM <= 160 * 1024, "tile shape");
     static_assert(NJ * 2048 + SUBB < 65536, "immediate offsets of the weight fragment reads");
 };
 
-template <int DT, class T>
+template <int DT, class T, bool UP>
 __global__ __launch_bounds__(T::NT) void hconv_kernel(HcP p) {
-    constexpr int MI = T::MI, NJ = T::NJ, KS = T::KS, NW = T::NW, BM = T::BM, BN = T::BN, NLD = T::NLD, PBW = T::PBW, SPT = T::SPT, SPC = T::SPC;
+    constexpr int MI = T::MI, NJ = T::NJ, KS = T::KS, NW = T::NW, BM = T::BM, BN = T::BN, NLD = T::NLD, PBW = T::PBW, SPT = T::SPT;
+    constexpr int NTAPS = UP ? 4 : 9, SPC = NTAPS * SPT;
+    constexpr int PPS = (NLD + SPC - 3) / (SPC - 2);
+    static_assert(SPC >= 3 && PPS * (SPC - 2) >= NLD, "halo pieces per chunk");
     extern __shared__ __attribute__((aligned(16))) uint8_t smem[];
     using E = ET<DT>;
     const int tid = threadIdx.x, lane = tid & 63;
@@ -65,9 +71,49 @@
     const uint32_t lds0 = (uint32_t)(size_t)(lds_ptr)smem;
 
     int m0 = 0, n0 = 0, c_begin = 0, c_end = 0, kslice = 0;
+    int t_cls = 0, t_H = H, t_row0 = 0, t_sep = 1, t_b0 = 0, t_y0 = 0, t_pix = BM;
     uint32_t aoff[5];
     uint32_t pbase[4];
     auto setup_tile = [&](int tl_ks) {
+        if constexpr (UP) {
+            c_begin = 0;
+            c_end = p.nchunks;
+            int mj, nt;
+            xcd_tile_order(tl_ks, p.m_tiles, p.n_tiles, mj, nt);
+            n0 = nt * BN;
+            const int nn = 4 * p.mt_n;
+            const bool bot = mj >= nn;
+            t_cls = bot ? 4 + ((mj - nn) & 1) : (mj & 3);
+            const int mt = bot ? (mj - nn) >> 1 : mj >> 2;
+            t_H = bot ? p.Hb : H;
+            t_row0 = bot ? H - p.Hb : 0;
+            t_sep = bot && p.Hb > 1 ? 0 : 1;
+            const int Rt = bot ? p.Rb : p.Rn;
+            t_pix = Rt << Wlog;
+            const int g0 = mt * Rt;
+            t_b0 = g0 / t_H;
+            t_y0 = g0 - t_b0 * t_H;
+            const int per = t_H + t_sep;
+#pragma unroll
+            for (int l = 0; l < NLD; ++l) {
+                const int pp = (l * NW + wave) * 8 + (lane >> 3);
+                const int slot = lane & 7;
+                const int j = pp >> Wlog, x = pp & (W - 1);
+                const int v = t_y0 - 1 + j;
+                const int q = v >= 0 ? v / per : 0, r = v - q * per;
+                const bool valid = v >= 0 && r < t_H && t_b0 + q < p.Btot;
+                const uint32_t src = (uint32_t)(((t_b0 + q) * H + t_row0 + r) * W + x) * (uint32_t)(p.Cin * 2) + (uint32_t)((slot ^ ((pp >> 1) & 7)) << 4);
+                aoff[l] = valid ? src : H_OOB;
+            }
+#pragma unroll
+            for (int i = 0; i < MI; ++i) {
+                int ml = (wm * MI + i) * 32 + l31;
+                ml = ml < t_pix ? ml : 0;
+                const int ir = ml >> Wlog, x = ml & (W - 1);
+                const int nsep = t_sep ? (t_y0 + ir) / t_H : 0;
+                pbase[i] = (uint32_t)(((1 + ir + nsep) << Wlog) + x);
+            }
+        } else {
         const int tl = tl_ks / p.ksplit;
         kslice = tl_ks - tl * p.ksplit;
         c_begin = kslice * p.nchunks / p.ksplit;
@@ -97,13 +143,14 @@
             const int nsep = (y0 + ir) / H;
             pbase[i] = (uint32_t)(((1 + ir + nsep) << Wlog) + x);
         }
+        }
     };
     auto issue_a = [&](int l, int buf, int chunk) {
         __builtin_amdgcn_raw_ptr_buffer_load_lds(ra, (lds_ptr)(smem + buf * T::OFF_A1 + (l * NW + wave) * 1024), 16, aoff[l], chunk * 128, 0, 0);
     };
     const uint32_t lane16 = (uint32_t)(lane * 16);
     auto issue_b = [&](int c, int s, int slot, int i) {
-        const int sub0 = (c * 9 + s / SPT) * 2 + (s % SPT) * (KS / 2);
+        const int sub0 = ((UP ? t_cls * p.nchunks : 0) + c) * (NTAPS * 2) + (s / SPT) * 2 + (s % SPT) * (KS / 2);
         const int q = wave * PBW + i;
         const int sb = q / (T::SUBB / 1024), qq = q - sb * (T::SUBB / 1024);
         const int soff = ((sub0 + sb) * p.N + n0) * 64 + qq * 1024;
@@ -123,12 +170,21 @@
     u32x4 fa[2][4] = {}, fb[2][4] = {};
     uint32_t a0[4], a0n[4];
     auto tap_address = [&](int i, int tap, int buf) -> uint32_t {
+        if constexpr (UP) {
+            const int ca = t_cls >= 4 ? 0 : t_cls >> 1, cb = t_cls & 1;
+            const int dy = (tap >> 1) - 1 + ca, dx = (tap & 1) - 1 + cb;
+            const uint32_t ps = pbase[i] + (uint32_t)(dy * W + dx);
+            const uint32_t a = lds0 + (uint32_t)(buf * T::OFF_A1) + (ps << 7) + ((((ps >> 1) & 7) ^ (uint32_t)half) << 4);
+            const bool border = (tap & 1) == 0 ? (cb == 0 && x_first) : (cb == 1 && x_last);
+            return border ? (zbase | (a & 0xF0u)) : a;
+        } else {
         const int dy = tap / 3 - 1, dx = tap - (tap / 3) * 3 - 1;
         const uint32_t ps = pbase[i] + (uint32_t)(dy * W + dx);
         uint32_t a = lds0 + (uint32_t)(buf * T::OFF_A1) + (ps << 7) + ((((ps >> 1) & 7) ^ (uint32_t)half) << 4);
         if (dx < 0) a = x_first ? (zbase | (a & 0xF0u)) : a;
         if (dx > 0) a = x_last ? (zbase | (a & 0xF0u)) : a;
         return a;
+        }
     };
     auto read_one = [&](auto set_tag, auto ks_tag, auto idx_tag, auto next_tag, uint32_t bb) {
         constexpr int SET = decltype(set_tag)::value, KSI = decltype(ks_tag)::value, IDX = decltype(idx_tag)::value;
@@ -161,6 +217,7 @@
 #pragma unroll 1
     for (int tl = blockIdx.x; tl < ntiles; tl += gridDim.x) {
     const int cm0 = m0, cn0 = n0, cks = kslice, cb = c_begin, ce = c_end;
+    const int e_cls = t_cls, e_H = t_H, e_row0 = t_row0, e_b0 = t_b0, e_y0 = t_y0, e_pix = t_pix;
 #pragma unroll
     for (int j = 0; j < NJ; ++j)
 #pragma unroll
@@ -182,14 +239,15 @@
         auto stage = [&](auto s_tag) {
             constexpr int S = decltype(s_tag)::value;
             constexpr int TAP = S / SPT, KS0 = (S % SPT) * KS;
-            constexpr bool prevA = S >= 1 && S - 1 < NLD;
-            if (!last) wait_vm<PBW + (prevA ? 1 : 0)>();
+            constexpr int NA = NLD - S * PPS < 0 ? 0 : (NLD - S * PPS < PPS ? NLD - S * PPS : PPS);
+            constexpr int prevA = S == 0 ? 0 : (NLD - (S - 1) * PPS < 0 ? 0 : (NLD - (S - 1) * PPS < PPS ? NLD - (S - 1) * PPS : PPS));
+            if (!last) wait_vm<PBW + prevA>();
             else if (S == 0 || S - 1 + 3 < SPC) wait_vm<PBW>();
             else wait_vm<0>();
             wait_lgkm<0>();
             RAW_BARRIER();
             const int nslot = (slot + 1) & 3;
-            const bool dma_a = S < NLD && !last, dma_b = S + 3 < SPC || !last;
+            const bool dma_a = NA > 0 && !last, dma_b = S + 3 < SPC || !last;
             h_for_each(std::make_integer_sequence<int, KS>{}, [&](auto kk_tag) {
                 constexpr int KK = decltype(kk_tag)::value, SET = KK & 1;
                 constexpr bool SAME = KK + 1 < KS;
@@ -197,7 +255,7 @@
                 constexpr bool NEWTAP = !SAME && NS % SPT == 0;
                 constexpr int PKSI = SAME ? KS0 + KK + 1 : (NS % SPT) * KS;
                 constexpr bool TAPCALC = S % SPT == SPT - 1 && KK == 0;
-                constexpr int NTAP = (TAP + 1) % 9;
+                constexpr int NTAP = (TAP + 1) % NTAPS;
                 const bool pf = SAME || S + 1 < SPC || !last;
                 const uint32_t bb = bfo[PKSI & 1] + (uint32_t)((SAME ? slot : nslot) * T::STAGE_B);
                 const bool dma_here = grp == (KK == 0 ? 0 : (KK == KS / 2 ? 1 : 2));
@@ -212,9 +270,12 @@
                         read_one(std::integral_constant<int, SET ^ 1>{}, std::integral_constant<int, PKSI>{}, std::integral_constant<int, 2 * IDX + 1>{},
                                  std::integral_constant<int, NEWTAP>{}, bb);
                     }
-                    if constexpr (TAPCALC && IDX < MI) a0n[IDX] = tap_address(IDX, NTAP, TAP + 1 < 9 ? buf : buf ^ 1);
+                    if constexpr (TAPCALC && IDX < MI) a0n[IDX] = tap_address(IDX, NTAP, TAP + 1 < NTAPS ? buf : buf ^ 1);
                     if (dma_here) {
-                        if (IDX == DSLOT0 && dma_a) issue_a(S, buf ^ 1, c + 1);
+                        if (IDX == DSLOT0 && dma_a) {
+#pragma unroll
+                            for (int q = 0; q < NA; ++q) issue_a(S * PPS + q, buf ^ 1, c + 1);
+                        }
                         if (IDX >= DSLOT0 && IDX - DSLOT0 < PBW && dma_b) {
                             if (S + 3 < SPC) issue_b(c, S + 3, (slot + 3) & 3, IDX - DSLOT0);
                             else issue_b(c + 1, S + 3 - SPC, (slot + 3) & 3, IDX - DSLOT0);
@@ -253,15 +314,24 @@
         for (int g = 0; g < 4; ++g) {
             const int n = cn_w + j * 32 + 8 * g + 4 * half;
             braw[j][g] = traw[j][g] = make_uint2(0, 0);
-            if (p.bias && p.ksplit == 1) braw[j][g] = *reinterpret_cast<const uint2*>(p.bias + (int64_t)n * 2);
-            if (rg_table && p.ksplit == 1) traw[j][g] = *reinterpret_cast<const uint2*>(p.rg + (step * p.ld_rg + n) * 2);
+            if (p.bias && (UP || p.ksplit == 1)) braw[j][g] = *reinterpret_cast<const uint2*>(p.bias + (int64_t)n * 2);
+            if (rg_table && (UP || p.ksplit == 1)) traw[j][g] = *reinterpret_cast<const uint2*>(p.rg + (step * p.ld_rg + n) * 2);
         }
     RAW_BARRIER();
     if (tl + (int)gridDim.x < ntiles) {
         setup_tile(tl + (int)gridDim.x);
         issue_prologue();
     }
-    if (p.ksplit > 1) {
+    auto up_row = [&](int ml) -> int64_t {
+        const int ir = ml >> Wlog, x = ml & (W - 1);
+        const int gy = e_y0 + ir, q = gy / e_H, isrc = e_row0 + gy - q * e_H, smp = e_b0 + q;
+        const int ca = e_cls >= 4 ? 0 : e_cls >> 1, oy = 2 * isrc + ca;
+        bool ok = ml < e_pix && smp < p.Btot && oy < p.Ho;
+        if (e_cls >= 4) ok = ok && isrc == H - 1;
+        else if (p.mt_b > 0 && ca == 0) ok = ok && isrc != H - 1;
+        return ok ? ((int64_t)smp * p.Ho + oy) * p.Wo + 2 * x + (e_cls & 1) : (int64_t)-1;
+    };
+    if (!UP && p.ksplit > 1) {
         float* slab = p.partial + (int64_t)cks * p.M * p.N;
 #pragma unroll
         for (int i = 0; i < MI; ++i) {
@@ -281,15 +351,25 @@
     for (int i = 0; i < MI; ++i) {
         const int mrow0 = cm0 + (wm * MI + i) * 32;
         uint4 rres[32 / RPI] = {};
+        int64_t urow[32 / RPI] = {};
+        if constexpr (UP) {
+#pragma unroll
+            for (int k = 0; k < 32 / RPI; ++k) urow[k] = up_row((wm * MI + i) * 32 + lane / LPR + RPI * k);
+        }
         if (p.residual) {
 #pragma unroll
             for (int k = 0; k < 32 / RPI; ++k) {
-                int m = mrow0 + lane / LPR + RPI * k;
+                int64_t m = mrow0 + lane / LPR + RPI * k;
                 m = m < p.M ? m : p.M - 1;
-                rres[k] = *reinterpret_cast<const uint4*>(p.residual + ((int64_t)m * p.ldr + cn_w + (lane % LPR) * 8) * 2);
-            }
-        }
-        const int mp = mrow0 + l31 < p.M ? mrow0 + l31 : p.M - 1;
+                if constexpr (UP) m = urow[k] >= 0 ? urow[k] : 0;
+                rres[k] = *reinterpret_cast<const uint4*>(p.residual + (m * p.ldr + cn_w + (lane % LPR) * 8) * 2);
+            }
+        }
+        int64_t mp = mrow0 + l31 < p.M ? mrow0 + l31 : p.M - 1;
+        if constexpr (UP) {
+            mp = rg_rows ? up_row((wm * MI + i) * 32 + l31) : 0;
+            mp = mp >= 0 ? mp : 0;
+        }
         const int64_t grp = rg_rows ? mp / p.rows_per_group + step : 0;
 #pragma unroll
         for (int j = 0; j < NJ; ++j)
@@ -320,7 +400,9 @@
                 for (int e = 0; e < 8; ++e) f[e] += rr[e];
                 o = pack8<DT>(f);
             }
-            if (m < p.M)
+            if constexpr (UP) {
+                if (urow[k] >= 0) *reinterpret_cast<uint4*>(p.out + (urow[k] * p.ldo + cn_w + (lane % LPR) * 8) * 2) = o;
+            } else if (m < p.M)
                 *reinterpret_cast<uint4*>(p.out + ((int64_t)m * p.ldo + cn_w + (lane % LPR) * 8) * 2) = o;
         }
     }
@@ -342,6 +424,36 @@
     const int ch = c * 64 + h * 32 + ((s ^ ((n >> 2) & 3)) << 3);
     const uint4 v = *reinterpret_cast<const uint4*>(w + ((int64_t)n * 9 + tap) * Cin + ch);
     *reinterpret_cast<uint4*>(out + idx * 8) = v;
+}
+
+template <int DT>
+__global__ void hconv_pack_up2_kernel(const uint8_t* __restrict__ w, uint8_t* __restrict__ out, int N, int Cin, int64_t total) {
+    const int64_t idx = (int64_t)blockIdx.x * blockDim.x + threadIdx.x;
+    if (idx >= total) return;
+    const int s = (int)(idx & 3);
+    int64_t r = idx >> 2;
+    const int n = (int)(r % N);
+    r /= N;
+    const int h = (int)(r & 1);
+    r >>= 1;
+    const int tap = (int)(r & 3);
+    r >>= 2;
+    const int nch = Cin / 64, c = (int)(r % nch), cls = (int)(r / nch);
+    const int ch = c * 64 + h * 32 + ((s ^ ((n >> 2) & 3)) << 3);
+    const int ca = cls >= 4 ? 0 : cls >> 1, cb = cls & 1, ty = tap >> 1, tx = tap & 1;
+    const int ky0 = ty == 0 ? 0 : (ca == 0 ? 1 : 2), ky1 = cls >= 4 ? ky0 : (ty == 0 ? ca : 2);
+    const int kx0 = tx == 0 ? 0 : (cb == 0 ? 1 : 2), kx1 = tx == 0 ? cb : 2;
+    float acc[8];
+#pragma unroll
+    for (int e = 0; e < 8; ++e) acc[e] = 0.f;
+    for (int ky = ky0; ky <= ky1; ++ky)
+        for (int kx = kx0; kx <= kx1; ++kx) {
+            float f[8];
+            unpack8<DT>(*reinterpret_cast<const uint4*>(w + (((int64_t)n * 9 + ky * 3 + kx) * Cin + ch) * 2), f);
+#pragma unroll
+            for (int e = 0; e < 8; ++e) acc[e] += f[e];
+        }
+    *reinterpret_cast<uint4*>(out + idx * 16) = pack8<DT>(acc);
 }
 
 int64_t g_hconv_launches = 0;
@@ -557,8 +669,8 @@
     *reinterpret_cast<uint4*>(p.out + ((int64_t)m * p.ldo + n) * 2) = o;
 }
 
-template <int DT, class T> int hc_launch(const HcP& p, hipStream_t s) {
-    auto kern = hconv_kernel<DT, T>;
+template <int DT, class T, bool UP = false> int hc_launch(const HcP& p, hipStream_t s) {
+    auto kern = hconv_kernel<DT, T, UP>;
     ++g_hconv_launches;
     static unsigned devs = 0;
     if (apad_ensure_dyn_lds(reinterpret_cast<const void*>(kern), T::SMEM, &devs) != 0) return -1;
@@ -573,7 +685,7 @@
     const int tiles = p.m_tiles * p.n_tiles * p.ksplit, cap = cus[dev];
     hipLaunchKernelGGL(kern, dim3((unsigned)(tiles < cap ? tiles : cap)), dim3(T::NT), T::SMEM, s, p);
     int rc = apad_check_launch("apad_gemm(halo convolution)");
-    if (rc || p.ksplit == 1) return rc;
+    if (rc || UP || p.ksplit == 1) return rc;
     const int64_t vecs = (int64_t)p.M * (p.N / 8);
     hipLaunchKernelGGL(hconv_reduce_kernel<DT>, dim3((unsigned)((vecs + 255) / 256)), dim3(256), 0, s, p);
     return apad_check_launch("apad_gemm(halo convolution, slice sum)");
@@ -594,6 +706,30 @@
 extern "C" int64_t apad_hconv_launch_count(void) { return g_hconv_launches; }
 
 extern "C" int64_t apad_conv_halo_packed_bytes(int64_t N, int64_t Cin) { return N <= 16 ? (Cin / 64) * 18 * 1024 : N * 9 * Cin * 2; }
+
+extern "C" int64_t apad_conv_halo_up2_packed_bytes(int64_t N, int64_t Cin) { return 24 * N * Cin * 2; }
+
+extern "C" int apad_conv_halo_pack_up2(const void* w, void* out, int64_t N, int64_t Cin, int32_t dtype, void* stream) {
+    APAD_CHECK(w && out && N > 0 && Cin > 0 && Cin % 64 == 0, "apad_conv_halo_pack_up2: needs Cin %% 64 == 0");
+    APAD_CHECK(dtype == APAD_BF16 || dtype == APAD_F16, "apad_conv_halo_pack_up2: 16-bit weights only");
+    const int64_t total = 24 * N * Cin / 8;
+    const dim3 grid((unsigned)((total + 255) / 256));
+    if (dtype == APAD_BF16)
+        hipLaunchKernelGGL(hconv_pack_up2_kernel<APAD_BF16>, grid, dim3(256), 0, (hipStream_t)stream, (const uint8_t*)w, (uint8_t*)out, (int)N, (int)Cin, total);
+    else
+        hipLaunchKernelGGL(hconv_pack_up2_kernel<APAD_F16>, grid, dim3(256), 0, (hipStream_t)stream, (const uint8_t*)w, (uint8_t*)out, (int)N, (int)Cin, total);
+    return apad_check_launch("apad_conv_halo_pack_up2");
+}
+
+static bool hconv_up2_geometry(int Hin, int Win, int Hup, int Wup) {
+    return Hup > 0 && Wup == 2 * Win && (Hup == 2 * Hin || Hup == 2 * Hin - 1) && Win >= 2 && Win <= 8 && (Win & (Win - 1)) == 0;
+}
+
+static int hconv_up2_tile_rows(int W, int Hv, bool sep, int npx) {
+    int R = 256 / W;
+    while (R > 1 && (R + 2 + (sep ? (R - 1) / Hv + 1 : 0)) * W > npx) --R;
+    return R;
+}
 
 extern "C" int apad_conv_halo_pack(const void* w, void* out, int64_t N, int64_t Cin, int32_t dtype, void* stream) {
     APAD_CHECK(w && out && N > 0 && Cin > 0 && Cin % 64 == 0, "apad_conv_halo_pack: needs Cin %% 64 == 0");
@@ -622,6 +758,33 @@
     if (d->Hup == 0 && (d->Hin != H || d->Win != W)) return 1;
     if (d->Hup != 0 && (d->Hup != H || d->Wup != W)) return 1;
     if (d->M % ((int64_t)H * W) != 0 || d->M >= (1LL << 30)) return 1;
+    if (d->halo_up2) {
+        APAD_CHECK(d->halo_up2 == 1 && hconv_up2_geometry(d->Hin, d->Win, d->Hup, d->Wup) && d->N % 128 == 0,
+                   "apad_gemm: halo_up2 needs an exact nearest-x2 geometry (source width 2, 4 or 8) and N %% 128 == 0");
+        if (d->ldo % 8 != 0 || (d->residual && d->ldr % 8 != 0) || (d->rowgroup_bias && d->rows_per_group <= 0)) return 1;
+        const int Hs = d->Hin, Ws = d->Win, cfg = d->N % 256 == 0 ? 0 : 1;
+        const int64_t Btot = d->M / ((int64_t)H * W);
+        const int64_t a_bytes = Btot * Hs * Ws * (int64_t)d->Cin * 2, w_bytes = apad_conv_halo_up2_packed_bytes(d->N, d->Cin);
+        if (a_bytes >= (1LL << 31) || w_bytes >= (1LL << 31)) return 1;
+        HcP p;
+        p.a = (const uint8_t*)d->a; p.wp = (const uint8_t*)d->w_halo; p.out = (uint8_t*)d->out; p.bias = (const uint8_t*)d->bias;
+        p.residual = (const uint8_t*)d->residual; p.rg = (const uint8_t*)d->rowgroup_bias; p.step_ptr = d->step_ptr;
+        p.ldo = d->ldo; p.ldr = d->ldr; p.ld_rg = d->ld_rg; p.rows_per_group = d->rows_per_group;
+        p.M = (int32_t)d->M; p.N = (int32_t)d->N; p.Cin = d->Cin;
+        p.H = Hs; p.W = Ws; p.Wlog = __builtin_ctz((unsigned)Ws); p.Hs = Hs; p.Ws = Ws; p.Btot = (int32_t)Btot;
+        p.Ho = H; p.Wo = W;
+        const bool odd = H == 2 * Hs - 1;
+        p.Hb = Hs < 2 ? Hs : 2;
+        p.Rn = hconv_up2_tile_rows(Ws, Hs, true, HcA::NPX);
+        p.Rb = hconv_up2_tile_rows(Ws, p.Hb, p.Hb < 2, HcA::NPX);
+        p.mt_n = (int32_t)((Btot * Hs + p.Rn - 1) / p.Rn);
+        p.mt_b = odd ? (int32_t)((Btot * p.Hb + p.Rb - 1) / p.Rb) : 0;
+        p.m_tiles = 4 * p.mt_n + 2 * p.mt_b; p.n_tiles = (int32_t)(d->N / (cfg == 0 ? HcA::BN : HcB::BN)); p.nchunks = d->Cin / 64;
+        p.ksplit = 1; p.partial = nullptr;
+        p.a_bytes = (uint32_t)a_bytes; p.w_bytes = (uint32_t)w_bytes;
+        if (d->dtype == APAD_BF16) return cfg == 0 ? hc_launch<APAD_BF16, HcA, true>(p, s) : hc_launch<APAD_BF16, HcB, true>(p, s);
+        return cfg == 0 ? hc_launch<APAD_F16, HcA, true>(p, s) : hc_launch<APAD_F16, HcB, true>(p, s);
+    }
     if (d->N <= 16) {
         if (d->N % 8 != 0 || (d->Cin != 64 && d->Cin != 128) || W < 4 || d->residual || d->rowgroup_bias || d->ldo % 8 != 0) return 1;
         const int R = 256 / W, S = (R - 1) / H + 1;
@@ -656,6 +819,7 @@
     p.m_tiles = (int32_t)((d->M + BM - 1) / BM); p.n_tiles = (int32_t)(d->N / BNc); p.nchunks = d->Cin / 64;
     p.ksplit = ksplit; p.partial = (float*)d->workspace;
     p.a_bytes = (uint32_t)a_bytes; p.w_bytes = (uint32_t)w_bytes;
+    p.Ho = H; p.Wo = W; p.mt_n = p.mt_b = 0; p.Rn = p.Rb = R; p.Hb = 0;
     if (d->dtype == APAD_BF16) return cfg == 0 ? hc_launch<APAD_BF16, HcA>(p, s) : hc_launch<APAD_BF16, HcB>(p, s);
     return cfg == 0 ? hc_launch<APAD_F16, HcA>(p, s) : hc_launch<APAD_F16, HcB>(p, s);
 }
diff --git a/ap-adapter_amd/ops.py b/ap-adapter_amd/ops.py
--- a/ap-adapter_amd/ops.py
+++ b/ap-adapter_amd/ops.py
@@ -109,7 +109,7 @@
 def gemm(a, w, *, M, N, K, lda, out, ldo, bias=None, residual=None, ldr=0, act=None, rowgroup_bias=None, ld_rg=0,
          rows_per_group=0, step_ptr=None, a_mode=L.A_PLAIN, out_mode=L.OUT_ROWMAJOR, conv=None, vt=None, ldw=None,
          residual_row_mod=0, asym_pad=False, rowstat_out=None, ln_fold=None, a2=None, lda2=0, k_split=0, a_row_mod=0, a2_row_mod=0,
-         w_halo=None, workspace=None, exact=False):
+         w_halo=None, workspace=None, exact=False, halo_up2=False):
     d = L.GemmDesc()
     if rowstat_out is not None:
         d.rowstat_out = rowstat_out.data_ptr()
@@ -132,6 +132,7 @@
         d.a2, d.lda2, d.k_split = a2.data_ptr(), lda2, k_split
     d.a_row_mod, d.a2_row_mod = a_row_mod, a2_row_mod
     d.w_halo = _ptr(w_halo)
+    d.halo_up2 = 1 if halo_up2 else 0
     if workspace is not None:
         d.workspace, d.workspace_bytes = workspace.data_ptr(), workspace.numel() * workspace.element_size()
     L.check(L.lib().apad_gemm(C.byref(d), _stream()), "apad_gemm")
@@ -729,6 +730,23 @@
     return derived(w_packed, "halo", make)
 
 
+HCONV_UP_FOLD = True
+
+
+def conv_halo_up2_eligible(Hin, Win, up):
+    return HCONV_UP_FOLD and up is not None and Win in (2, 4, 8) and up[1] == 2 * Win and up[0] in (2 * Hin, 2 * Hin - 1)
+
+
+def conv_halo_up2_weight(w_packed):
+    def make():
+        wc = w_packed.detach().contiguous()
+        Cout, K = wc.shape
+        out = torch.empty(L.lib().apad_conv_halo_up2_packed_bytes(Cout, K // 9) // 2, dtype=wc.dtype, device=wc.device)
+        L.check(L.lib().apad_conv_halo_pack_up2(wc.data_ptr(), out.data_ptr(), Cout, K // 9, _DT[wc.dtype], _stream()), "apad_conv_halo_pack_up2")
+        return out
+    return derived(w_packed, "halo_up2", make)
+
+
 def conv3x3_pack(w):
     return w.detach().permute(0, 2, 3, 1).reshape(w.shape[0], -1).contiguous()
 
@@ -738,7 +756,7 @@
 
 
 def conv3x3(x, w_packed, bias, B, Hin, Win, stride=1, up=None, residual=None, rowgroup_bias=None, rows_per_group=0,
-            step_ptr=None, src_batch_mod=0, out=None, asym_pad=False):
+            step_ptr=None, src_batch_mod=0, out=None, asym_pad=False, up_fold=True):
     _req(x, "conv3x3.x", w_packed.dtype)
     Cin = x.shape[-1]
     Cout = w_packed.shape[0]
@@ -749,12 +767,17 @@
     if out is None:
         out = torch.empty(B, Hout * Wout, Cout, dtype=x.dtype, device=x.device)
     wh = ws = None
+    fold = False
     if conv_halo_eligible(Cin, Cout, Wout, stride, w_packed.dtype, src_batch_mod, asym_pad):
-        wh = conv_halo_weight(w_packed)
-        nws = L.lib().apad_conv_halo_workspace_bytes(M, Cout, Cin, Wout)
-        if nws:
-            ws = torch.empty(nws // 4, dtype=torch.float32, device=x.device)
-    gemm(x, w_packed, M=M, N=Cout, K=9 * Cin, lda=0, out=out, ldo=Cout, bias=bias, w_halo=wh, workspace=ws,
+        fold = up_fold and Cout % 128 == 0 and conv_halo_up2_eligible(Hin, Win, up)
+        if fold:
+            wh = conv_halo_up2_weight(w_packed)
+        else:
+            wh = conv_halo_weight(w_packed)
+            nws = L.lib().apad_conv_halo_workspace_bytes(M, Cout, Cin, Wout)
+            if nws:
+                ws = torch.empty(nws // 4, dtype=torch.float32, device=x.device)
+    gemm(x, w_packed, M=M, N=Cout, K=9 * Cin, lda=0, out=out, ldo=Cout, bias=bias, w_halo=wh, workspace=ws, halo_up2=fold,
          residual=residual, ldr=Cout, rowgroup_bias=rowgroup_bias,
          ld_rg=(rowgroup_bias.stride(0) if rowgroup_bias is not None else 0), rows_per_group=rows_per_group,
          step_ptr=step_ptr, a_mode=L.A_CONV3X3, asym_pad=asym_pad,
diff --git a/include/apadapter_hip.h b/include/apadapter_hip.h
--- a/include/apadapter_hip.h
+++ b/include/apadapter_hip.h
@@ -56,7 +56,7 @@
     int32_t a_pre_act;
     float a_pre_slope;
     int32_t conv_asym_pad;
-    int32_t reserved_conv;
+    int32_t halo_up2;
     float* rowstat_out;
     const float* rowstat_in;
     const float* ln_colsum;
@@ -241,6 +241,8 @@
 int apad_gemm(const apad_gemm_desc* d, void* stream);
 int apad_conv_halo_pack(const void* w, void* out, int64_t N, int64_t Cin, int32_t dtype, void* stream);
 int64_t apad_conv_halo_packed_bytes(int64_t N, int64_t Cin);
+int apad_conv_halo_pack_up2(const void* w, void* out, int64_t N, int64_t Cin, int32_t dtype, void* stream);
+int64_t apad_conv_halo_up2_packed_bytes(int64_t N, int64_t Cin);
 int64_t apad_conv_halo_workspace_bytes(int64_t M, int64_t N, int64_t Cin, int32_t Wout);
 int apad_probe_mfma(void* sink, int32_t mode, int32_t iters, double* flops, void* stream);
 int64_t apad_hconv_launch_count(void);
```
